# xiexh20/VisTracker

Hardware: AMD Instinct MI355X
Metric: frames/sec joint SMPL+object fit (higher is better)
Workload: dtype f32 (decoder GEMMs: 22-bit split-f16 operands x3 MFMA, fp32 accumulate)

## Files before the change

### include/vistracker.h

```cpp
#ifndef VISTRACKER_H
#define VISTRACKER_H

#include <stddef.h>

#ifdef __cplusplus
extern "C" {
#endif

#define VT_OK 0
#define VT_ERR_ARG -1
#define VT_ERR_HIP -2
#define VT_ERR_BUSY -3

#define VT_SMPL_V 6890
#define VT_SMPL_J 52
#define VT_SMPL_NB 10
#define VT_SMPL_NP 459
#define VT_FEAT 611
#define VT_HID 128

const char *vt_last_error(void);
int vt_version(void);

typedef struct vt_smplh vt_smplh;

int vt_smplh_create(vt_smplh **out, const float *v_template, const float *shapedirs, const float *posedirs,
                    const float *J_regressor, const float *weights, const int *parents, void *stream);
void vt_smplh_destroy(vt_smplh *h);

long vt_smplh_workspace_floats(int B);

int vt_smplh_forward(const vt_smplh *h, const float *pose, const float *betas, const float *trans, int B,
                     float *verts, float *jtr, float *v_posed, float *ws, void *stream);

long vt_smplh_bwd_scratch_floats(int B);
int vt_smplh_backward(const vt_smplh *h, const float *pose, const float *betas, int B, const float *dverts,
                      const float *djtr, const float *v_posed, const float *ws, float *scratch,
                      float *dpose, float *dbetas, float *dtrans, void *stream);

long vt_smplh_prefix_floats(int B);
int vt_smplh_prefix(const vt_smplh *h, const float *pose, int B, float *ws, float *prefix, void *stream);
int vt_smplh_forward_prefixed(const vt_smplh *h, const float *pose, const float *betas, const float *trans, int B, const float *prefix,
                              float *verts, float *jtr, float *v_posed, float *ws, void *stream);
int vt_smplh_backward_free(const vt_smplh *h, const float *pose, int B, const float *dverts, const float *djtr, const float *v_posed,
                           const float *ws, float *scratch, int n_free_pose_cols, float *dpose, float *dbetas, float *dtrans, void *stream);

int vt_rodrigues_forward(const float *aa, int n, float *R, void *stream);
int vt_rodrigues_backward(const float *aa, int n, const float *dR, float *daa, void *stream);

typedef struct vt_landmarks vt_landmarks;
int vt_landmarks_create(vt_landmarks **out, const int *indptr, const int *indices, const float *data, int K, int V,
                        void *stream);
void vt_landmarks_destroy(vt_landmarks *h);
int vt_landmarks_forward(const vt_landmarks *h, const float *verts, int B, float *out, void *stream);
int vt_landmarks_backward(const vt_landmarks *h, const float *dout, int B, float *dverts, int accumulate, void *stream);

int vt_mahalanobis(const float *x, int B, int stride, int off, int n, const float *mean, const float *prec,
                   float *value, float *dx, float gscale, void *stream);

int vt_fill_f64(double *p, long n, double value, void *stream);
int vt_sum_to_term(const float *value, int n, float scale, double *term, void *stream);

typedef struct vt_sifnet vt_sifnet;
int vt_sifnet_create(vt_sifnet **out, const float *const *w, const float *const *b, const float *cam, void *stream);
void vt_sifnet_destroy(vt_sifnet *h);

int vt_nchw_to_nhwc(const float *src, int B, int C, int H, int W, float *dst, void *stream);

typedef struct {
    const float *maps[8];
    int res[8];
    const float *proj;
    int proj_cols;
    int act_level;
    int proj_level;
    int force_fp32;
} vt_maps;

int vt_query_forward(const vt_sifnet *h, const vt_maps *maps, const float *pts, const float *crop_center,
                     const float *body_center, int B, int N,
                     float *df, float *pca, float *parts, float *centers, float *vis, void *stream);
int vt_query_backward(const vt_sifnet *h, const vt_maps *maps, const float *pts, const float *crop_center,
                      const float *body_center, int B, int N,
                      const float *d_df, const float *d_pca, const float *d_parts, const float *d_centers,
                      const float *d_vis, float *dpts, void *stream);

long vt_query_projection_floats(const vt_maps *maps, int B);
int vt_query_build_projection(const vt_sifnet *h, const vt_maps *maps, int B, float *proj, void *stream);

int vt_query_human_loss(const vt_sifnet *h, const vt_maps *maps, const float *pts, const float *crop_center,
                        const float *body_center, int B, int N, const int *labels, const int *order, float w_dfh, float w_part,
                        float *dpts, double *terms, void *stream);
int vt_query_object_loss(const vt_sifnet *h, const vt_maps *maps, const float *pts, const float *crop_center,
                         const float *body_center, int B, int N, const float *occ, float w_obj,
                         float *dpts, double *terms, void *stream);

typedef struct vt_conv3x3 vt_conv3x3;
int vt_conv3x3_create(vt_conv3x3 **out, const float *weight, int cout, int cin, void *stream);
void vt_conv3x3_destroy(vt_conv3x3 *h);
int vt_conv3x3_forward(const vt_conv3x3 *h, const float *in, int B, int H, int W, float *out, int out_cstride, int out_coff, void *stream);
int vt_conv3x3_forward_gn(const vt_conv3x3 *h, const float *in, int in_cstride, int in_coff, const float *gn_stats, const float *gamma,
                          const float *beta, int groups, int B, int H, int W, float *out, int out_cstride, int out_coff, void *stream);
int vt_conv3x3_forward_gn_stats(const vt_conv3x3 *h, const float *in, int in_cstride, int in_coff, const float *gn_stats, const float *gamma,
                                const float *beta, int groups, int B, int H, int W, float *out, int out_cstride, int out_coff, double *stats_ws,
                                int stats_groups, void *stream);
int vt_conv3x3_forward_block(const vt_conv3x3 *h, const float *in, int in_cstride, int in_coff, const float *gn_stats, const float *gamma,
                             const float *beta, int groups, int B, int H, int W, float *out, int out_cstride, int out_coff,
                             const float *res, int res_cstride, int res_coff, float *fin, int fin_cstride, int fin_coff,
                             double *stats_ws, int stats_groups, void *stream);
int vt_conv3x3_tiles(int H, int W);
typedef struct vt_stem7x7 vt_stem7x7;
int vt_stem7x7_create(vt_stem7x7 **out, const float *weight, const float *bias, int cout, int cin, void *stream);
void vt_stem7x7_destroy(vt_stem7x7 *h);
int vt_stem7x7_forward(const vt_stem7x7 *h, const float *in, int in_cstride, int in_coff, int B, int H, int W, float *out, int out_cstride, int out_coff, void *stream);
typedef struct vt_conv1x1 vt_conv1x1;
int vt_conv1x1_create(vt_conv1x1 **out, const float *weight, const float *bias, int cout, int cin, void *stream);
void vt_conv1x1_destroy(vt_conv1x1 *h);
int vt_conv1x1_forward(const vt_conv1x1 *h, const float *in, int in_cstride, int in_coff, const float *gn_stats, const float *gamma, const float *beta, int groups,
                       int B, int H, int W, float *out, int out_cstride, int out_coff, const float *res, int res_cstride, int res_coff,
                       double *stats_ws, int stats_groups, void *stream);
int vt_groupnorm_finalize(double *ws, int nblk, int B, int HW, int C, int groups, float eps, void *stream);
int vt_conv3x3_forward_block_stats(const vt_conv3x3 *h, const float *in, int in_cstride, int in_coff, const float *gn_stats, const float *gamma,
                                   const float *beta, int groups, int B, int H, int W, float *out, int out_cstride, int out_coff,
                                   const float *res, int res_cstride, int res_coff, float *fin, int fin_cstride, int fin_coff,
                                   double *stats_ws, int stats_groups, double *fin_stats_ws, int fin_stats_groups, void *stream);
int vt_avgpool2x2_stats(const float *x, int B, int H, int W, int C, float *out, double *stats_ws, int stats_groups, void *stream);
int vt_sweep_blocks(int HW);
int vt_groupnorm_stats(const float *x, int cstride, int coff, int B, int HW, int C, int groups, float eps, double *ws, void *stream);

#define VT_PRECISION_SPLIT_F16 0
#define VT_PRECISION_FP32 1
int vt_sifnet_set_precision(vt_sifnet *h, int mode);
int vt_sifnet_get_precision(const vt_sifnet *h);

int vt_query_set_human_kernel(int threads);

int vt_query_project_step(const vt_sifnet *h, const vt_maps *maps, const float *pts, const float *crop_center,
                          const float *body_center, int B, int N, int df_idx, float threshold, float *pts_out,
                          float *df_target, void *stream);

int vt_kpts_step(const vt_landmarks *h, const float *verts, const float *kpts, const float *crop_center, int B, int mode, const float *cam, float net_size,
                 float gscale, double *term, float *J, float *dverts, int accumulate, void *stream);
int vt_query_human_step(const vt_sifnet *h, const vt_maps *maps, const float *pts, const float *crop_center, const float *body_center,
                        int B, int N, const int *labels, const int *order, float w_dfh, float w_part, int accumulate, float w_accel,
                        double *term_accel, float *dpts, double *terms, void *stream);
int vt_objstep_head(const float *M0, const float *noise, const float *t, const float *s, int B, const float *X0_points, int N, float *X_points,
                    const float *X0_verts, int NV, float *X_verts, float *R, double *terms, int nzero, float *svd_ws, void *stream);
int vt_temporal_loss2(const float *v, int B, int D, float gscale_accel, double *term_accel, float gscale_velocity, double *term_velocity, float *dv,
                      int init_zero, void *stream);
int vt_objstep_tail(const float *X0_verts, int NV, const float *dX_verts, const float *X0_points, int N, const float *dX_points, const float *s, int B,
                    const float *M0, const float *noise, const float *t, const float *t_init, float w_trans, double *term_trans,
                    float *dR, float *dt, float *dM,
                    float *pR, float *mR, float *vR, float lrR, float *pT, float *mT, float *vT, float lrT, int adam_step, float beta1, float beta2, float eps,
                    double *terms, const float *w, int nterms, float tol, int armed, float *state, int *stop_flag, float *history, int slot, int *ticket, int nzero,
                    float *svd_ws, void *stream);
int vt_objstep_tail_temporal(const float *X_points, float gscale_accel, double *term_accel, float gscale_velocity, double *term_velocity, int init_zero,
                             const float *X0_verts, int NV, const float *dX_verts, const float *X0_points, int N, const float *dX_points, const float *s, int B,
                             const float *M0, const float *noise, const float *t, const float *t_init, float w_trans, double *term_trans,
                             float *dR, float *dt, float *dM,
                             float *pR, float *mR, float *vR, float lrR, float *pT, float *mT, float *vT, float lrT, int adam_step, float beta1, float beta2, float eps,
                             double *terms, const float *w, int nterms, float tol, int armed, float *state, int *stop_flag, float *history, int slot, int *ticket, int nzero,
                             float *svd_ws, void *stream);
int vt_smplstep_tail(float *pose, const float *pose_init, float *dpose, int B, const float *prior_mean, const float *prior_prec, float gscale_prior,
                     double *term_prior, float w_pinit, double *term_pinit,
                     float *p0, int ps0, const float *g0, int gs0, float *m0, float *v0, int n0, float lr0,
                     float *p1, int ps1, const float *g1, int gs1, float *m1, float *v1, int n1, float lr1,
                     float *p2, int ps2, const float *g2, int gs2, float *m2, float *v2, int n2, float lr2,
                     int adam_step, float beta1, float beta2, float eps,
                     double *terms, const float *w, int nterms, float tol, int armed, float *state, int *stop_flag, float *history, int slot, int *ticket, int nzero,
                     void *stream);

int vt_so3_project_forward(const float *M0, const float *noise, int B, float *R, void *stream);
int vt_so3_project_backward(const float *M0, const float *noise, int B, const float *dR, float *dM, void *stream);

int vt_rigid_forward(const float *X0, int shared_x0, const float *R, const float *t, const float *s, int B, int N,
                     float *X, void *stream);
int vt_rigid_backward(const float *X0, int shared_x0, const float *s, int B, int N, const float *dX,
                      float *dR, float *dt, int accumulate, void *stream);

int vt_accel_loss(const float *v, int B, int D, const float *elem_w, float gscale, double *term, float *dv, void *stream);
int vt_accel_loss_strided(const float *v, int B, int D, int stride, const float *elem_w, float gscale, double *term,
                          float *dv, void *stream);
int vt_velocity_loss(const float *v, int B, int D, float gscale, double *term, float *dv, void *stream);

int vt_kpts_loss(const float *J, const float *kpts, const float *crop_center, int B, int K, int mode,
                 const float *cam, float net_size, float gscale, double *term, float *dJ, void *stream);

int vt_sqdiff_loss(const float *a, int a_stride, const float *b, int b_stride, int rows, int cols, float denom,
                   float gscale, double *term, float *da, void *stream);

long vt_collision_workspace_bytes(int B, int n_smpl_faces);
int vt_collision_loss(const float *smpl_verts, int n_smpl_verts, const int *smpl_faces, int n_smpl_faces, const float *obj_verts, int n_obj_verts,
                      const int *obj_faces, int n_obj_faces, int B, float sigma, int max_collisions, float gscale, double *term,
                      float *d_obj_t, int *pairs_per_frame, void *workspace, void *stream);

int vt_chamfer_ragged(const float *x, const int *offx, const float *y, const int *offy, int P, float gscale,
                      double *term, float *dx, float *dy, void *stream);
long vt_chamfer_ws_bytes(long total_x, long total_y, int P);
int vt_chamfer_ragged_ws(const float *x, const int *offx, long total_x, const float *y, const int *offy, long total_y, int P, float gscale,
                         double *term, float *dx, float *dy, void *ws, void *stream);

int vt_chamfer_ragged_idx(const float *x, const int *offx, long total_x, const float *y_base, const int *idx_y, const int *offy, long total_y, int P,
                          float gscale, double *term, float *dy_base, void *ws, int run_plan, void *stream);

int vt_nn_distance(const float *query, int nq, const float *search, int ns, int P, float *dist, void *stream);

long vt_sil_workspace_floats(int B, int NV, int NF, int size);
int vt_sil_forward(const float *verts, int B, int NV, const int *faces, int NF, const float *K, int size,
                   float *image, int *face_index, float *ws, void *stream);
int vt_sil_backward(const float *verts, int B, int NV, const int *faces, int NF, const float *K, int size,
                    const int *face_index, const float *d_image, float eps, float *ws, float *dverts, void *stream);
int vt_sil_setup(const float *mask_h, const float *mask_o, int B, int H, int W, const float *crop_centers, double expansion, int out, double crop_size,
                 double net_size, const double *cam_norm, double image_width, float *image_ref, float *keep_mask, float *K, double *boxes_ws, void *stream);

int vt_sil_mask_loss(const float *image, const float *keep, const float *ref, const float *occ, int B, int size,
                     float gscale, double *term, float *per_frame, float *d_image, void *stream);

int vt_sil_step(const float *verts, int B, int NV, const int *faces, int NF, const float *K, int size, const float *keep, const float *ref,
                const float *occ, float gscale, float eps, double *term, int *face_index, float *d_image, float *ws, float *dverts, void *stream);

int vt_triplane_render(const float *verts, const float *center, int B, int NV, const int *faces, int NF, int size,
                       float *masks, int *face_index, float *ws, void *stream);

int vt_upsample2x_bicubic_add(const float *low, const float *skip, int B, int h, int w, int C, float *out, void *stream);
int vt_upsample2x_bicubic_add_stats(const float *low, const float *skip, int B, int h, int w, int C, float *out, double *stats_ws, int stats_groups,
                                    void *stream);

long vt_groupnorm_workspace_doubles(int B, int HW, int C, int groups);
int vt_groupnorm_nhwc(const float *x, const float *gamma, const float *beta, int B, int HW, int C, int groups, float eps,
                      int relu, double *ws, float *y, void *stream);

int vt_adam_step(float *p, const float *g, float *m, float *v, long n, int step, float lr, float beta1, float beta2,
                 float eps, const int *stop_flag, void *stream);

int vt_adam_step_2d(float *p, long p_stride, const float *g, long g_stride, float *m, float *v, int rows, int cols,
                    int step, float lr, float beta1, float beta2, float eps, const int *stop_flag, void *stream);

int vt_loss_reduce_and_stop(const double *terms, const float *w, int nterms, float tol, int armed, float *state,
                            int *stop_flag, float *history, int slot, void *stream);

int vt_fill(float *p, long n, float value, void *stream);

int vt_stream_set_skip_flag(void *stream, const int *flag);

int vt_gen_round_compact(const float *surface, const float *df_target, const float *pre, const unsigned char *active, int B, int S, float filter_val,
                         float zmin, const long long *fill, int cap, int write, float *buf_points, int *order, float *kept_pre, long long *cnt,
                         long long *fill_out, void *stream);
int vt_gen_scatter_heads(const float *pred, int B, int C, int kmax, const long long *fill_old, const long long *cnt, int cap, float *buf, void *stream);
int vt_gen_resample(const float *samples, const int *order, const long long *cnt, const float *init, int B, int S, int S0, const float *u,
                    const float *pert, int M, float near_scale, float *out, void *stream);

long vt_render_workspace_bytes(int B, int NF, int size, int anti_aliasing, long list_entries);
int vt_render_static_create(void **layer, const float *verts, int NV, const int *faces, int NS, const float *face_colors, const float *K, float orig_size,
                            const float *light, int size, int anti_aliasing, void *stream);
void vt_render_static_destroy(void *layer);
int vt_render_rgb(const float *verts, int B, int NV, const int *faces, int NF, const float *face_colors, const float *K, int k_per_view, float orig_size,
                  const float *light, const float *background, const void *static_layer, int size, int anti_aliasing, float *rgb, float *alpha, float *depth,
                  int *face_index, void *ws, long ws_bytes, long *list_entries, void *stream);
int vt_render_panel_u8(const float *rgb, int B, int size, int row0, int nrows, int col0, int ncols, unsigned char *out, const long long *view_off,
                       long long out_row_stride, void *stream);
int vt_render_rgb_pv(const float *verts, int B, int NV, const int *faces, int NF, const float *face_colors, int colors_per_view, const float *K, int k_per_view,
                     float orig_size, const float *light, const float *background, const void *static_layer, int size, int anti_aliasing, float *rgb,
                     float *alpha, float *depth, int *face_index, void *ws, long ws_bytes, long *list_entries, void *stream);

int vt_contact_regions(const float *smpl_verts, const int *labels, const float *obj_verts, int B, int NVs, int NVo, int P, float thres, int *nn_idx,
                       float *nn_dist, int *part, int *count, float *centre, void *stream);
int vt_contact_spheres(const float *centre, const int *count, int B, int P, const float *unit_verts, int NSV, float radius, float *out, void *stream);
int vt_contact_face_colors(const int *part, int B, int NVo, const int *obj_faces, int NFo, int face_off, const float *base_colors, int NF, const float *palette,
                           int P, float *out, void *stream);

long vt_jpeg_workspace_bytes(int n, int H, int W, int subsampling, long long *max_out_bytes);
int vt_jpeg_encode(const unsigned char *rgb, int n, int H, int W, long long frame_stride, long long row_stride, int quality, int subsampling, void *ws,
                   long ws_bytes, unsigned char *out, long long out_cap, long long *offsets, void *stream);

int vt_mask_bbox(const unsigned char *pm, const unsigned char *om, int B, int H, int W, int thres, int *box, void *stream);
int vt_crop_resize_compose(const unsigned char *rgb, const unsigned char *pm, const unsigned char *om, int B, int H, int W, const int *corners, int crop_size,
                           int out_size, const float *table, float *out, long long frame_stride, void *stream);
int vt_resize_panel_u8(const unsigned char *src, long long src_bytes, const long long *frames, int n, int H, int size, int col0, int pw, unsigned char *out,
                       const long long *out_off, long long out_row_stride, void *stream);

int vt_overlay_panel_u8(const float *rgb, const float *alpha, int B, int size, int row0, int nrows, int col0, int ncols, unsigned char *out,
                        const long long *src_off, const long long *dst_off, long long out_row_stride, float opacity, void *stream);
int vt_mask_score(const int *fidx, int B, int is, int rows, int F, int nf_body, int nf_obj, const unsigned char *pm, long long pm_bytes, const unsigned char *om,
                  long long om_bytes, const long long *frames, int thres, int *count, void *stream);

long vt_point_mesh_workspace_bytes(int B, int n_faces);
int vt_point_mesh_distance(const float *points, int n_points, const float *verts, int n_verts, const int *faces, int n_faces, int B, float *dist, float *closest,
                           int *face_id, void *workspace, void *stream);
int vt_point_mesh_distance_ex(const float *points, int n_points, const float *verts, int n_verts, const int *faces, int n_faces, int B, float *dist,
                              float *closest, int *face_id, void *workspace, int flags, unsigned long long *n_tests, void *stream);
int vt_nearest_vertex(const float *points, int n_points, const float *verts, int n_verts, int B, int *vert_id, float *vert_dist, void *stream);

long vt_sifnet_loss_head_ws_bytes(int B, int n_points);
int vt_sifnet_loss_head(const float *df, const float *pca, const float *parts, const float *centers, const float *vis, int S, int B, int n_points,
                        const float *df_h, const float *df_o, const int *parts_gt, const float *pca_gt, const float *obj_center, const float *visibility,
                        int per_frame, float max_dist, const double *weights, int vis_loss, float gscale, double *terms, float *d_df, float *d_pca,
                        float *d_parts, float *d_centers, float *d_vis, void *workspace, void *stream);

long vt_decoder_param_floats(void);
long vt_decoder_param_offset(int head, int layer, int is_bias);
int vt_decoder_train_forward(const float *params, const float *cam, const vt_maps *maps, const float *pts, const float *crop_center, const float *body_center,
                             int B, int N, float *df, float *pca, float *parts, float *centers, float *vis, void *stream);
long vt_decoder_weight_grads_ws_bytes(int B, int N, int chunk_points);
int vt_decoder_weight_grads(const float *params, const float *cam, const vt_maps *maps, const float *pts, const float *crop_center, const float *body_center,
                            int B, int N, const float *d_df, const float *d_pca, const float *d_parts, const float *d_centers, const float *d_vis,
                            float *dparams, int accumulate, int chunk_points, void *workspace, void *stream);

long vt_decoder_grads_ws_bytes(int B, int N, int chunk_points, int want_maps);
int vt_decoder_grads(const float *params, const float *cam, const vt_maps *maps, const float *pts, const float *crop_center, const float *body_center,
                     int B, int N, const float *d_df, const float *d_pca, const float *d_parts, const float *d_centers, const float *d_vis,
                     float *dparams, int accumulate, const vt_maps *d_maps, int accumulate_maps, int chunk_points, void *workspace, void *stream);

long vt_conv_dgrad_workspace_bytes(int cout, int cin, int taps);
long vt_conv_wgrad_workspace_bytes(int B, int H, int W, int cout, int cin, int taps);
long vt_gn_relu_backward_workspace_bytes(int B, int HW, int C, int groups);
int vt_conv3x3_dgrad(const float *weight, int cout, int cin, const float *d_out, int do_cstride, int do_coff, int B, int H, int W,
                     float *d_in, int di_cstride, int di_coff, void *workspace, void *stream);
int vt_conv1x1_dgrad(const float *weight, int cout, int cin, const float *d_out, int do_cstride, int do_coff, int B, int H, int W,
                     float *d_in, int di_cstride, int di_coff, void *workspace, void *stream);
int vt_conv3x3_wgrad(const float *d_out, int do_cstride, int do_coff, const float *x_in, int xi_cstride, int xi_coff, const float *gn_stats, const float *gamma,
                     const float *beta, int groups, int B, int H, int W, int cin, int cout, float *dW, int accumulate, void *workspace, void *stream);
int vt_conv1x1_wgrad(const float *d_out, int do_cstride, int do_coff, const float *x_in, int xi_cstride, int xi_coff, const float *gn_stats, const float *gamma,
                     const float *beta, int groups, int B, int H, int W, int cin, int cout, float *dW, int accumulate, void *workspace, void *stream);
int vt_gn_relu_backward(const float *g, int g_cstride, int g_coff, const float *x_in, int x_cstride, int x_coff, const float *gn_stats, const float *gamma,
                        const float *beta, int groups, int B, int HW, int C, const float *base, int base_cstride, int base_coff,
                        float *d_x, int dx_cstride, int dx_coff, float *dgamma, float *dbeta, int accumulate, void *workspace, void *stream);
long vt_conv_block_backward_workspace(int B, int H, int W, int cin, int c1, int c2, int c3);
int vt_conv_block_backward(const float *dy, const float *x, const float *raw, const float *stats1, const float *stats2, const float *stats3,
                           const float *w1, const float *w2, const float *w3, const float *gamma1, const float *gamma2, const float *gamma3,
                           const float *beta1, const float *beta2, const float *beta3, const float *wproj, const float *gamma4, const float *beta4,
                           int B, int H, int W, int cin, int c1, int c2, int c3,
                           float *d_x, float *dW1, float *dW2, float *dW3, float *dgamma1, float *dbeta1, float *dgamma2, float *dbeta2, float *dgamma3, float *dbeta3,
                           float *dgamma4, float *dbeta4, float *dWproj, void *workspace, int accumulate, void *stream);

int vt_avgpool2x2_backward(const float *d_out, int B, int H, int W, int C, float *d_x, void *stream);
int vt_upsample2x_bicubic_backward(const float *d_out, int B, int h, int w, int C, float *d_low, void *stream);

long vt_bias_grad_workspace_bytes(int B, int HW, int C);
int vt_bias_grad(const float *d_out, int do_cstride, int do_coff, int B, int HW, int C, float *db, int accumulate, void *workspace, void *stream);
long vt_stem7x7_wgrad_workspace_bytes(int B, int H, int W, int cin, int cout);
int vt_stem7x7_wgrad(const float *d_y, int dy_cstride, int dy_coff, const float *x, int x_cstride, int x_coff, int B, int H, int W, int cin, int cout,
                     float *dW, int accumulate, void *workspace, void *stream);
int vt_gn_relu_backward_y(const float *g, int g_cstride, int g_coff, const float *x_in, int x_cstride, int x_coff, const float *y, int y_cstride, int y_coff,
                          const float *gn_stats, const float *gamma, int groups, int B, int HW, int C, const float *base, int base_cstride, int base_coff,
                          float *d_x, int dx_cstride, int dx_coff, float *dgamma, float *dbeta, int accumulate, void *workspace, void *stream);
long vt_stack_tail_backward_workspace(int B, int H, int W, int C, int Co);
int vt_stack_tail_backward(const float *d_out, const float *d_prev, const float *ll, const float *raw, const float *out, const float *stats,
                           const float *wcl, const float *gamma, const float *beta, const float *wl, const float *wbl, const float *wal,
                           int B, int H, int W, int C, int Co,
                           float *d_ll, float *dWcl, float *dbcl, float *dgamma, float *dbeta, float *dWl, float *dbl, float *dWbl, float *dbbl, float *dWal, float *dbal,
                           void *workspace, int accumulate, void *stream);

#define VT_REPACK_CONV3X3 0
#define VT_REPACK_CONV1X1 1
#define VT_REPACK_STEM7X7 2
typedef struct vt_repack_plan vt_repack_plan;
long vt_conv3x3_packed_bytes(int cout, int cin);
long vt_conv1x1_packed_bytes(int cout, int cin);
int vt_conv1x1_parts(int cout);
long vt_stem7x7_packed_bytes(int cout, int cin);
long vt_repack_workspace_bytes(void);
int vt_conv3x3_pack(const float *w_dev, int cout, int cin, void *packed_dev, float *scale_dev, void *ws_dev, void *stream);
int vt_conv1x1_pack(const float *w_dev, const float *bias_dev, int cout, int cin, void *packed_dev, float *bias_out_dev, float *scale_dev, void *ws_dev,
                    void *stream);
int vt_stem7x7_pack(const float *w_dev, const float *bias_dev, int cout, int cin, void *packed_dev, void *stream);
int vt_conv3x3_create_device(vt_conv3x3 **out, const float *w_dev, int cout, int cin, void *stream);
int vt_conv1x1_create_device(vt_conv1x1 **out, const float *w_dev, const float *bias_dev, int cout, int cin, void *stream);
int vt_stem7x7_create_device(vt_stem7x7 **out, const float *w_dev, const float *bias_dev, int cout, int cin, void *stream);
int vt_conv3x3_repack(vt_conv3x3 *h, const float *w_dev, void *stream);
int vt_conv1x1_repack(vt_conv1x1 *h, const float *w_dev, const float *bias_dev, void *stream);
int vt_stem7x7_repack(vt_stem7x7 *h, const float *w_dev, const float *bias_dev, void *stream);
int vt_repack_plan_create(vt_repack_plan **out, int n, const int *kinds, void *const *handles, const float *const *weights, const float *const *biases);
int vt_repack_plan_run(const vt_repack_plan *plan, void *stream);
void vt_repack_plan_destroy(vt_repack_plan *plan);
int vt_repack_plan_launches(const vt_repack_plan *plan);
int vt_repack_handle_snapshot(int kind, const void *handle, void *packed_out_dev, float *scale_out_dev, void *stream);

int vt_grad_rank_mean(const float *parts, int W, size_t n, size_t stride, float *out, void *stream);

#define VT_GRAD_STATS_CHUNK 4096
#define VT_GUARD_HEAD 16
#define VT_GUARD_SLOT_HEAD 32
#define VT_GUARD_NORM 0
#define VT_GUARD_ERROR 8
#define VT_GUARD_COEF 16
#define VT_GUARD_SKIP 20
#define VT_GUARD_STEP 24
long vt_grad_stats_workspace_bytes(long n, int n_seg);
int vt_grad_stats(const float *g, long n, const long *seg_off, int n_seg, double *sumsq, float *maxabs, int *nonfinite, void *ws, void *stream);
long vt_grad_guard_record_bytes(int n_seg_total, int ring);
int vt_grad_guard_close(const double *sumsq0, const float *maxabs0, const int *nonfinite0, int n_seg0,
                        const double *sumsq1, const float *maxabs1, const int *nonfinite1, int n_seg1,
                        const double *sumsq2, const float *maxabs2, const int *nonfinite2, int n_seg2,
                        const double *error, double max_norm, void *record, int ring, void *stream);
int vt_grad_scale(float *g, long n, const float *coef, const int *skip, void *stream);

long vt_former_layer_tape_floats(int B, int T, int D, int H, int F);
long vt_former_layer_workspace_floats(int B, int T, int D, int H, int F);
int vt_former_layer_forward(const float *x, const float *pos, const unsigned char *key_padding_mask, const float *const *params, int B, int T, int D, int H,
                            int F, int activation, float p, unsigned long long seed, float *y, float *tape, float *workspace, void *stream);
int vt_former_layer_backward(const float *d_y, const float *tape, const float *x, const float *pos, const unsigned char *key_padding_mask,
                             const float *const *params, int B, int T, int D, int H, int F, int activation, float p, unsigned long long seed,
                             float *d_x, float *const *d_params, int accumulate, float *workspace, void *stream);
long vt_layernorm_backward_workspace_floats(long M, int D);
int vt_layernorm_forward(const float *x, const float *weight, const float *bias, long M, int D, float *y, double *stats, void *stream);
int vt_layernorm_backward(const float *d_y, const float *x, const double *stats, const float *weight, long M, int D, float *d_x, float *d_weight,
                          float *d_bias, int accumulate, float *workspace, void *stream);

int vt_query_set_clock_probe(unsigned long long *counters);
long vt_calibrate_workspace_bytes(void);
int vt_calibrate(void *work, double *out, void *stream);

#ifdef __cplusplus
}
#endif
#endif
```

### vistracker_amd/_lib.py

```python
from __future__ import annotations

import ctypes as C
import os

_HERE = os.path.dirname(os.path.abspath(__file__))
LIB_PATH = os.environ.get("VT_LIB_PATH", os.path.join(_HERE, "libvistracker_hip.so"))

vp = C.c_void_p
fp = C.c_void_p
ci = C.c_int
cl = C.c_long
cf = C.c_float
cd = C.c_double


class VtMaps(C.Structure):
    _fields_ = [("maps", C.c_void_p * 8), ("res", C.c_int * 8), ("proj", C.c_void_p), ("proj_cols", C.c_int),
                ("act_level", C.c_int), ("proj_level", C.c_int), ("force_fp32", C.c_int)]


SIGNATURES = {
    "vt_last_error": (C.c_char_p, []),
    "vt_version": (ci, []),
    "vt_smplh_create": (ci, [C.POINTER(vp), vp, vp, vp, vp, vp, vp, vp]),
    "vt_smplh_destroy": (None, [vp]),
    "vt_smplh_workspace_floats": (cl, [ci]),
    "vt_smplh_bwd_scratch_floats": (cl, [ci]),
    "vt_smplh_forward": (ci, [vp, fp, fp, fp, ci, fp, fp, fp, fp, vp]),
    "vt_smplh_backward": (ci, [vp, fp, fp, ci, fp, fp, fp, fp, fp, fp, fp, fp, vp]),
    "vt_smplh_prefix_floats": (cl, [ci]),
    "vt_smplh_prefix": (ci, [vp, fp, ci, fp, fp, vp]),
    "vt_smplh_forward_prefixed": (ci, [vp, fp, fp, fp, ci, fp, fp, fp, fp, fp, vp]),
    "vt_smplh_backward_free": (ci, [vp, fp, ci, fp, fp, fp, fp, fp, ci, fp, fp, fp, vp]),
    "vt_rodrigues_forward": (ci, [fp, ci, fp, vp]),
    "vt_rodrigues_backward": (ci, [fp, ci, fp, fp, vp]),
    "vt_landmarks_create": (ci, [C.POINTER(vp), vp, vp, vp, ci, ci, vp]),
    "vt_landmarks_destroy": (None, [vp]),
    "vt_landmarks_forward": (ci, [vp, fp, ci, fp, vp]),
    "vt_landmarks_backward": (ci, [vp, fp, ci, fp, ci, vp]),
    "vt_mahalanobis": (ci, [fp, ci, ci, ci, ci, fp, fp, fp, fp, cf, vp]),
    "vt_fill_f64": (ci, [fp, cl, cd, vp]),
    "vt_sum_to_term": (ci, [fp, ci, cf, fp, vp]),
    "vt_sifnet_create": (ci, [C.POINTER(vp), C.POINTER(vp), C.POINTER(vp), vp, vp]),
    "vt_sifnet_destroy": (None, [vp]),
    "vt_nchw_to_nhwc": (ci, [fp, ci, ci, ci, ci, fp, vp]),
    "vt_query_forward": (ci, [vp, C.POINTER(VtMaps), fp, fp, fp, ci, ci, fp, fp, fp, fp, fp, vp]),
    "vt_query_backward": (ci, [vp, C.POINTER(VtMaps), fp, fp, fp, ci, ci, fp, fp, fp, fp, fp, fp, vp]),
    "vt_query_human_loss": (ci, [vp, C.POINTER(VtMaps), fp, fp, fp, ci, ci, fp, fp, cf, cf, fp, fp, vp]),
    "vt_query_object_loss": (ci, [vp, C.POINTER(VtMaps), fp, fp, fp, ci, ci, fp, cf, fp, fp, vp]),
    "vt_query_set_human_kernel": (ci, [ci]),
    "vt_sifnet_set_precision": (ci, [vp, ci]),
    "vt_sifnet_get_precision": (ci, [vp]),
    "vt_groupnorm_nhwc": (ci, [fp, fp, fp, ci, ci, ci, ci, cf, ci, fp, fp, vp]),
    "vt_upsample2x_bicubic_add": (ci, [fp, fp, ci, ci, ci, ci, fp, vp]),
    "vt_conv3x3_create": (ci, [C.POINTER(vp), vp, ci, ci, vp]),
    "vt_conv3x3_destroy": (None, [vp]),
    "vt_conv3x3_forward": (ci, [vp, fp, ci, ci, ci, fp, ci, ci, vp]),
    "vt_conv3x3_forward_gn": (ci, [vp, fp, ci, ci, fp, fp, fp, ci, ci, ci, ci, fp, ci, ci, vp]),
    "vt_groupnorm_stats": (ci, [fp, ci, ci, ci, ci, ci, ci, cf, fp, vp]),
    "vt_groupnorm_workspace_doubles": (C.c_long, [ci, ci, ci, ci]),
    "vt_groupnorm_finalize": (ci, [fp, ci, ci, ci, ci, ci, cf, vp]),
    "vt_conv3x3_tiles": (ci, [ci, ci]),
    "vt_kpts_step": (ci, [vp, fp, fp, fp, ci, ci, vp, cf, cf, fp, fp, fp, ci, vp]),
    "vt_query_human_step": (ci, [vp, C.POINTER(VtMaps), fp, fp, fp, ci, ci, fp, fp, cf, cf, ci, cf, fp, fp, fp, vp]),
    "vt_objstep_head": (ci, [fp, fp, fp, fp, ci, fp, ci, fp, fp, ci, fp, fp, fp, ci, fp, vp]),
    "vt_temporal_loss2": (ci, [fp, ci, ci, cf, fp, cf, fp, fp, ci, vp]),
    "vt_objstep_tail": (ci, [fp, ci, fp, fp, ci, fp, fp, ci, fp, fp, fp, fp, cf, fp, fp, fp, fp,
                             fp, fp, fp, cf, fp, fp, fp, cf, ci, cf, cf, cf,
                             fp, vp, ci, cf, ci, fp, fp, fp, ci, fp, ci, fp, vp]),
    "vt_objstep_tail_temporal": (ci, [fp, cf, fp, cf, fp, ci,
                                      fp, ci, fp, fp, ci, fp, fp, ci, fp, fp, fp, fp, cf, fp, fp, fp, fp,
                                      fp, fp, fp, cf, fp, fp, fp, cf, ci, cf, cf, cf,
                                      fp, vp, ci, cf, ci, fp, fp, fp, ci, fp, ci, fp, vp]),
    "vt_smplstep_tail": (ci, [fp, fp, fp, ci, fp, fp, cf, fp, cf, fp,
                              fp, ci, fp, ci, fp, fp, ci, cf, fp, ci, fp, ci, fp, fp, ci, cf, fp, ci, fp, ci, fp, fp, ci, cf, ci, cf, cf, cf,
                              fp, vp, ci, cf, ci, fp, fp, fp, ci, fp, ci, vp]),
    "vt_stream_set_skip_flag": (ci, [vp, vp]),
    "vt_conv1x1_create": (ci, [C.POINTER(vp), vp, vp, ci, ci, vp]),
    "vt_stem7x7_create": (ci, [C.POINTER(vp), vp, vp, ci, ci, vp]),
    "vt_stem7x7_destroy": (None, [vp]),
    "vt_stem7x7_forward": (ci, [vp, fp, ci, ci, ci, ci, ci, fp, ci, ci, vp]),
    "vt_conv1x1_destroy": (None, [vp]),
    "vt_conv1x1_forward": (ci, [vp, fp, ci, ci, fp, fp, fp, ci, ci, ci, ci, fp, ci, ci, fp, ci, ci, fp, ci, vp]),
    "vt_conv3x3_forward_block": (ci, [vp, fp, ci, ci, fp, fp, fp, ci, ci, ci, ci, fp, ci, ci, fp, ci, ci, fp, ci, ci, fp, ci, vp]),
    "vt_conv3x3_forward_block_stats": (ci, [vp, fp, ci, ci, fp, fp, fp, ci, ci, ci, ci, fp, ci, ci, fp, ci, ci, fp, ci, ci, fp, ci, fp, ci, vp]),
    "vt_avgpool2x2_stats": (ci, [fp, ci, ci, ci, ci, fp, fp, ci, vp]),
    "vt_sweep_blocks": (ci, [ci]),
    "vt_upsample2x_bicubic_add_stats": (ci, [fp, fp, ci, ci, ci, ci, fp, fp, ci, vp]),
    "vt_conv3x3_forward_gn_stats": (ci, [vp, fp, ci, ci, fp, fp, fp, ci, ci, ci, ci, fp, ci, ci, fp, ci, vp]),
    "vt_triplane_render": (ci, [fp, fp, ci, ci, fp, ci, ci, fp, fp, fp, vp]),
    "vt_query_project_step": (ci, [vp, C.POINTER(VtMaps), fp, fp, fp, ci, ci, ci, cf, fp, fp, vp]),
    "vt_query_projection_floats": (C.c_long, [C.POINTER(VtMaps), ci]),
    "vt_query_build_projection": (ci, [vp, C.POINTER(VtMaps), ci, fp, vp]),
    "vt_so3_project_forward": (ci, [fp, fp, ci, fp, vp]),
    "vt_so3_project_backward": (ci, [fp, fp, ci, fp, fp, vp]),
    "vt_rigid_forward": (ci, [fp, ci, fp, fp, fp, ci, ci, fp, vp]),
    "vt_rigid_backward": (ci, [fp, ci, fp, ci, ci, fp, fp, fp, ci, vp]),
    "vt_accel_loss": (ci, [fp, ci, ci, fp, cf, fp, fp, vp]),
    "vt_accel_loss_strided": (ci, [fp, ci, ci, ci, fp, cf, fp, fp, vp]),
    "vt_velocity_loss": (ci, [fp, ci, ci, cf, fp, fp, vp]),
    "vt_kpts_loss": (ci, [fp, fp, fp, ci, ci, ci, vp, cf, cf, fp, fp, vp]),
    "vt_sqdiff_loss": (ci, [fp, ci, fp, ci, ci, ci, cf, cf, fp, fp, vp]),
    "vt_chamfer_ragged": (ci, [fp, fp, fp, fp, ci, cf, fp, fp, fp, vp]),
    "vt_chamfer_ws_bytes": (C.c_long, [C.c_long, C.c_long, ci]),
    "vt_chamfer_ragged_ws": (ci, [fp, fp, C.c_long, fp, fp, C.c_long, ci, cf, fp, fp, fp, fp, vp]),
    "vt_chamfer_ragged_idx": (ci, [fp, fp, C.c_long, fp, fp, fp, C.c_long, ci, cf, fp, fp, fp, ci, vp]),
    "vt_collision_workspace_bytes": (cl, [ci, ci]),
    "vt_collision_loss": (ci, [fp, ci, fp, ci, fp, ci, fp, ci, ci, cf, ci, cf, fp, fp, fp, fp, vp]),
    "vt_nn_distance": (ci, [fp, ci, fp, ci, ci, fp, vp]),
    "vt_sil_workspace_floats": (cl, [ci, ci, ci, ci]),
    "vt_sil_forward": (ci, [fp, ci, ci, fp, ci, fp, ci, fp, fp, fp, vp]),
    "vt_sil_backward": (ci, [fp, ci, ci, fp, ci, fp, ci, fp, fp, cf, fp, fp, vp]),
    "vt_sil_mask_loss": (ci, [fp, fp, fp, fp, ci, ci, cf, fp, fp, fp, vp]),
    "vt_sil_step": (ci, [fp, ci, ci, fp, ci, fp, ci, fp, fp, fp, cf, cf, fp, fp, fp, fp, fp, vp]),
    "vt_gen_round_compact": (ci, [fp, fp, fp, vp, ci, ci, cf, cf, vp, ci, ci, fp, vp, fp, vp, vp, vp]),
    "vt_gen_scatter_heads": (ci, [fp, ci, ci, ci, vp, vp, ci, fp, vp]),
    "vt_gen_resample": (ci, [fp, vp, vp, fp, ci, ci, ci, fp, fp, ci, cf, fp, vp]),
    "vt_sil_setup": (ci, [fp, fp, ci, ci, ci, fp, C.c_double, ci, C.c_double, C.c_double, C.POINTER(C.c_double), C.c_double, fp, fp, fp, fp, vp]),
    "vt_adam_step": (ci, [fp, fp, fp, fp, cl, ci, cf, cf, cf, cf, fp, vp]),
    "vt_adam_step_2d": (ci, [fp, cl, fp, cl, fp, fp, ci, ci, ci, cf, cf, cf, cf, fp, vp]),
    "vt_loss_reduce_and_stop": (ci, [fp, vp, ci, cf, ci, fp, fp, fp, ci, vp]),
    "vt_fill": (ci, [fp, cl, cf, vp]),
    "vt_selftest_mfma": (ci, [fp, fp, fp, vp]),
    "vt_query_set_clock_probe": (ci, [vp]),
    "vt_render_workspace_bytes": (cl, [ci, ci, ci, ci, cl]),
    "vt_render_static_create": (ci, [C.POINTER(vp), fp, ci, fp, ci, fp, fp, cf, C.POINTER(cf), ci, ci, vp]),
    "vt_render_static_destroy": (None, [vp]),
    "vt_render_rgb": (ci, [fp, ci, ci, fp, ci, fp, fp, ci, cf, C.POINTER(cf), C.POINTER(cf), vp, ci, ci, fp, fp, fp, fp, fp, cl,
                           C.POINTER(cl), vp]),
    "vt_render_panel_u8": (ci, [fp, ci, ci, ci, ci, ci, ci, fp, fp, C.c_longlong, vp]),
    "vt_render_rgb_pv": (ci, [fp, ci, ci, fp, ci, fp, ci, fp, ci, cf, C.POINTER(cf), C.POINTER(cf), vp, ci, ci, fp, fp, fp, fp, fp, cl,
                              C.POINTER(cl), vp]),
    "vt_contact_regions": (ci, [fp, fp, fp, ci, ci, ci, ci, cf, fp, fp, fp, fp, fp, vp]),
    "vt_contact_spheres": (ci, [fp, fp, ci, ci, fp, ci, cf, fp, vp]),
    "vt_contact_face_colors": (ci, [fp, ci, ci, fp, ci, ci, fp, ci, fp, ci, fp, vp]),
    "vt_jpeg_workspace_bytes": (cl, [ci, ci, ci, ci, C.POINTER(C.c_longlong)]),
    "vt_jpeg_encode": (ci, [fp, ci, ci, ci, C.c_longlong, C.c_longlong, ci, ci, vp, cl, vp, C.c_longlong,
                            C.POINTER(C.c_longlong), vp]),
    "vt_mask_bbox": (ci, [fp, fp, ci, ci, ci, ci, fp, vp]),
    "vt_crop_resize_compose": (ci, [fp, fp, fp, ci, ci, ci, fp, ci, ci, fp, fp, C.c_longlong, vp]),
    "vt_resize_panel_u8": (ci, [fp, C.c_longlong, vp, ci, ci, ci, ci, ci, fp, fp, C.c_longlong, vp]),
    "vt_overlay_panel_u8": (ci, [fp, fp, ci, ci, ci, ci, ci, ci, fp, fp, fp, C.c_longlong, cf, vp]),
    "vt_mask_score": (ci, [fp, ci, ci, ci, ci, ci, ci, fp, C.c_longlong, fp, C.c_longlong, vp, ci, fp, vp]),
    "vt_point_mesh_workspace_bytes": (cl, [ci, ci]),
    "vt_point_mesh_distance": (ci, [fp, ci, fp, ci, fp, ci, ci, fp, fp, fp, vp, vp]),
    "vt_point_mesh_distance_ex": (ci, [fp, ci, fp, ci, fp, ci, ci, fp, fp, fp, vp, ci, fp, vp]),
    "vt_nearest_vertex": (ci, [fp, ci, fp, ci, ci, fp, fp, vp]),
    "vt_sifnet_loss_head_ws_bytes": (cl, [ci, ci]),
    "vt_sifnet_loss_head": (ci, [fp, fp, fp, fp, fp, ci, ci, ci, fp, fp, fp, fp, fp, fp, ci, cf, C.POINTER(cd), ci, cf, fp, fp, fp, fp, fp, fp, vp, vp]),
    "vt_decoder_param_floats": (cl, []),
    "vt_decoder_param_offset": (cl, [ci, ci, ci]),
    "vt_decoder_train_forward": (ci, [fp, vp, C.POINTER(VtMaps), fp, fp, fp, ci, ci, fp, fp, fp, fp, fp, vp]),
    "vt_decoder_weight_grads_ws_bytes": (cl, [ci, ci, ci]),
    "vt_decoder_weight_grads": (ci, [fp, vp, C.POINTER(VtMaps), fp, fp, fp, ci, ci, fp, fp, fp, fp, fp, fp, ci, ci, vp, vp]),
    "vt_decoder_grads_ws_bytes": (cl, [ci, ci, ci, ci]),
    "vt_decoder_grads": (ci, [fp, vp, C.POINTER(VtMaps), fp, fp, fp, ci, ci, fp, fp, fp, fp, fp, fp, ci, C.POINTER(VtMaps), ci, ci, vp, vp]),
    "vt_conv_dgrad_workspace_bytes": (cl, [ci, ci, ci]),
    "vt_conv_wgrad_workspace_bytes": (cl, [ci, ci, ci, ci, ci, ci]),
    "vt_gn_relu_backward_workspace_bytes": (cl, [ci, ci, ci, ci]),
    "vt_conv3x3_dgrad": (ci, [fp, ci, ci, fp, ci, ci, ci, ci, ci, fp, ci, ci, vp, vp]),
    "vt_conv1x1_dgrad": (ci, [fp, ci, ci, fp, ci, ci, ci, ci, ci, fp, ci, ci, vp, vp]),
    "vt_conv3x3_wgrad": (ci, [fp, ci, ci, fp, ci, ci, fp, fp, fp, ci, ci, ci, ci, ci, ci, fp, ci, vp, vp]),
    "vt_conv1x1_wgrad": (ci, [fp, ci, ci, fp, ci, ci, fp, fp, fp, ci, ci, ci, ci, ci, ci, fp, ci, vp, vp]),
    "vt_gn_relu_backward": (ci, [fp, ci, ci, fp, ci, ci, fp, fp, fp, ci, ci, ci, ci, fp, ci, ci, fp, ci, ci, fp, fp, ci, vp, vp]),
    "vt_conv_block_backward_workspace": (cl, [ci, ci, ci, ci, ci, ci, ci]),
    "vt_conv_block_backward": (ci, [fp] * 6 + [fp] * 9 + [fp] * 3 + [ci] * 7 + [fp] * 13 + [vp, ci, vp]),
    "vt_avgpool2x2_backward": (ci, [fp, ci, ci, ci, ci, fp, vp]),
    "vt_upsample2x_bicubic_backward": (ci, [fp, ci, ci, ci, ci, fp, vp]),
    "vt_bias_grad_workspace_bytes": (cl, [ci, ci, ci]),
    "vt_bias_grad": (ci, [fp, ci, ci, ci, ci, ci, fp, ci, vp, vp]),
    "vt_stem7x7_wgrad_workspace_bytes": (cl, [ci, ci, ci, ci, ci]),
    "vt_stem7x7_wgrad": (ci, [fp, ci, ci, fp, ci, ci, ci, ci, ci, ci, ci, fp, ci, vp, vp]),
    "vt_gn_relu_backward_y": (ci, [fp, ci, ci, fp, ci, ci, fp, ci, ci, fp, fp, ci, ci, ci, ci, fp, ci, ci, fp, ci, ci, fp, fp, ci, vp, vp]),
    "vt_stack_tail_backward_workspace": (cl, [ci, ci, ci, ci, ci]),
    "vt_stack_tail_backward": (ci, [fp] * 6 + [fp] * 6 + [ci] * 5 + [fp] * 11 + [vp, ci, vp]),
    "vt_conv3x3_packed_bytes": (cl, [ci, ci]),
    "vt_conv1x1_packed_bytes": (cl, [ci, ci]),
    "vt_conv1x1_parts": (ci, [ci]),
    "vt_stem7x7_packed_bytes": (cl, [ci, ci]),
    "vt_repack_workspace_bytes": (cl, []),
    "vt_conv3x3_pack": (ci, [fp, ci, ci, fp, fp, fp, vp]),
    "vt_conv1x1_pack": (ci, [fp, fp, ci, ci, fp, fp, fp, fp, vp]),
    "vt_stem7x7_pack": (ci, [fp, fp, ci, ci, fp, vp]),
    "vt_conv3x3_create_device": (ci, [C.POINTER(vp), fp, ci, ci, vp]),
    "vt_conv1x1_create_device": (ci, [C.POINTER(vp), fp, fp, ci, ci, vp]),
    "vt_stem7x7_create_device": (ci, [C.POINTER(vp), fp, fp, ci, ci, vp]),
    "vt_conv3x3_repack": (ci, [vp, fp, vp]),
    "vt_conv1x1_repack": (ci, [vp, fp, fp, vp]),
    "vt_stem7x7_repack": (ci, [vp, fp, fp, vp]),
    "vt_repack_plan_create": (ci, [C.POINTER(vp), ci, C.POINTER(ci), C.POINTER(vp), C.POINTER(vp), C.POINTER(vp)]),
    "vt_repack_plan_launches": (ci, [vp]),
    "vt_repack_plan_run": (ci, [vp, vp]),
    "vt_repack_plan_destroy": (None, [vp]),
    "vt_repack_handle_snapshot": (ci, [ci, vp, fp, fp, vp]),
    "vt_grad_rank_mean": (ci, [fp, ci, C.c_size_t, C.c_size_t, fp, vp]),
    "vt_grad_stats_workspace_bytes": (cl, [cl, ci]),
    "vt_grad_stats": (ci, [fp, cl, fp, ci, fp, fp, fp, fp, vp]),
    "vt_grad_guard_record_bytes": (cl, [ci, ci]),
    "vt_grad_guard_close": (ci, [fp, fp, fp, ci] * 3 + [fp, cd, fp, ci, vp]),
    "vt_grad_scale": (ci, [fp, cl, fp, fp, vp]),
    "vt_calibrate_workspace_bytes": (cl, []),
    "vt_calibrate": (ci, [vp, C.POINTER(C.c_double), vp]),
    "vt_former_layer_tape_floats": (cl, [ci, ci, ci, ci, ci]),
    "vt_former_layer_workspace_floats": (cl, [ci, ci, ci, ci, ci]),
    "vt_former_layer_forward": (ci, [fp, fp, fp, vp, ci, ci, ci, ci, ci, ci, cf, C.c_ulonglong, fp, fp, fp, vp]),
    "vt_former_layer_backward": (ci, [fp, fp, fp, fp, fp, vp, ci, ci, ci, ci, ci, ci, cf, C.c_ulonglong, fp, vp, ci, fp, vp]),
    "vt_layernorm_backward_workspace_floats": (cl, [cl, ci]),
    "vt_layernorm_forward": (ci, [fp, fp, fp, cl, ci, fp, fp, vp]),
    "vt_layernorm_backward": (ci, [fp, fp, fp, fp, cl, ci, fp, fp, fp, ci, fp, vp]),
}

_lib = None


class VtError(RuntimeError):
    pass


def lib():
    global _lib
    if _lib is None:
        if not os.path.exists(LIB_PATH):
            raise VtError(f"{LIB_PATH} is missing: build it with `make -C vistracker_amd/csrc` "
                          f"(or `python -c 'import __graft_entry__ as g; g.build()'`); there is no CPU fallback")
        import torch
        l = C.CDLL(LIB_PATH)
        for name, (res, args) in SIGNATURES.items():
            fn = getattr(l, name)
            fn.restype = res
            fn.argtypes = args
        _lib = l
        _host_tuning()
    return _lib


def _host_tuning():
    if os.environ.get("VT_HOST_THP", "keep") != "off":
        return
    try:
        C.CDLL(None, use_errno=True).prctl(41, 1, 0, 0, 0)
    except Exception:
        pass


VT_OK, VT_ERR_ARG, VT_ERR_HIP, VT_ERR_BUSY = 0, -1, -2, -3


def check(rc: int):
    if rc != 0:
        raise VtError(f"libvistracker_hip error {rc}: {lib().vt_last_error().decode()}")


def stream_ptr():
    import torch
    return torch.cuda.current_stream().cuda_stream


def dptr(t):
    if t is None:
        return None
    if not t.is_cuda:
        raise VtError("libvistracker_hip ops need CUDA (HIP) tensors; there is no CPU fallback in the product path")
    if not t.is_contiguous():
        raise VtError("libvistracker_hip ops need contiguous tensors")
    import torch
    if t.device.index != torch.cuda.current_device():
        raise VtError(f"tensor on cuda:{t.device.index} but the current device is cuda:{torch.cuda.current_device()}: "
                      "wrap the call in `with torch.cuda.device(tensor.device):`")
    return t.data_ptr()
```

### vistracker_amd/csrc/smplh.hip

```cpp
#include "common.h"
#include <cstring>

#define V_ VT_SMPL_V
#define J_ VT_SMPL_J
#define NB_ VT_SMPL_NB
#define NP_ VT_SMPL_NP
#define VP_ 6912
#define NVT_ 27
#define KQ_ 472
#define NQ_ 480
#define J_LIVE_ 22
#define NP_LIVE_ ((J_LIVE_ - 1) * 9)
#define KF_ 272
#define NT_LIVE_ 13
#define NQ_HAND_ (NT_LIVE_ * 16)
#define NP_NUM_ (J_ * 3)
__host__ __device__ constexpr int kq_of_posemap(int p) { return p < NP_LIVE_ ? KF_ + p : p - NP_LIVE_; }
__host__ __device__ constexpr int nq_of_posemap(int p) { return p < NP_LIVE_ ? p : NQ_HAND_ + (p - NP_LIVE_); }
#define KQ_BETA0 (KF_ + NP_LIVE_)
#define KQ_TEMPLATE (KQ_ - 1)
#define NQ_BETA0 NP_LIVE_
static_assert(KF_ % 8 == 0 && KF_ >= NP_ - NP_LIVE_ && KQ_BETA0 + NB_ <= KQ_TEMPLATE && (KQ_ - KF_) % 8 == 0, "K order of Q_kcv");
static_assert(NQ_BETA0 + NB_ <= NQ_HAND_ && NQ_HAND_ + (NP_ - NP_LIVE_) <= NQ_, "N order of Q_t");
typedef float f32x4 __attribute__((ext_vector_type(4)));
#define MFMA16(a, b, c) __builtin_amdgcn_mfma_f32_16x16x4f32((a), (b), (c), 0, 0, 0)

#define WS_R 0
#define WS_J (52 * 9)
#define WS_G (WS_J + 52 * 3)
#define WS_A (WS_G + 52 * 12)
#define WS_FRAME (WS_A + 52 * 12)
#define PT_DA 0
#define PT_DTR 624
#define PT_N 627
#define KTOT_ (VP_ * 3)
#define KG_SLAB 24
#define NKS_ (KTOT_ / 16 / KG_SLAB)

#define SCHED_STEPS 32
#define SCHED_WIDTH 10
struct SmplParents { int p[J_]; int nsteps; short sched[SCHED_STEPS][SCHED_WIDTH]; };

#define SP_K 8
struct vt_smplh {
    float *Q_kcv, *Q_t, *W_jv, *W_v64, *J_t, *J_s;
    float *W_sp;
    int nnz;
    SmplParents par;
};

struct RodCtx { float n, ax, ay, az, c, s, qn, w, x, y, z; };

__device__ __forceinline__ void rodrigues_fwd(const float *t, float *R, RodCtx *k)
{
    const float xe = t[0] + 1e-8f, ye = t[1] + 1e-8f, ze = t[2] + 1e-8f;
    const float n = sqrtf(xe * xe + ye * ye + ze * ze);
    const float ax = t[0] / n, ay = t[1] / n, az = t[2] / n;
    const float h = n * 0.5f;
    const float c = cosf(h), s = sinf(h);
    const float q0 = c, q1 = s * ax, q2 = s * ay, q3 = s * az;
    const float qn = sqrtf(q0 * q0 + q1 * q1 + q2 * q2 + q3 * q3);
    const float w = q0 / qn, x = q1 / qn, y = q2 / qn, z = q3 / qn;
    const float w2 = w * w, x2 = x * x, y2 = y * y, z2 = z * z;
    const float wx = w * x, wy = w * y, wz = w * z, xy = x * y, xz = x * z, yz = y * z;
    R[0] = w2 + x2 - y2 - z2; R[1] = 2 * xy - 2 * wz;   R[2] = 2 * wy + 2 * xz;
    R[3] = 2 * wz + 2 * xy;   R[4] = w2 - x2 + y2 - z2; R[5] = 2 * yz - 2 * wx;
    R[6] = 2 * xz - 2 * wy;   R[7] = 2 * wx + 2 * yz;   R[8] = w2 - x2 - y2 + z2;
    if (k) { k->n = n; k->ax = ax; k->ay = ay; k->az = az; k->c = c; k->s = s; k->qn = qn; k->w = w; k->x = x; k->y = y; k->z = z; }
}

__device__ __forceinline__ void rodrigues_bwd(const float *t, const float *dR, float *dt)
{
    float R[9]; RodCtx k; rodrigues_fwd(t, R, &k);
    const float w = k.w, x = k.x, y = k.y, z = k.z;
    const float dw = 2 * w * (dR[0] + dR[4] + dR[8]) + 2 * (-z * dR[1] + y * dR[2] + z * dR[3] - x * dR[5] - y * dR[6] + x * dR[7]);
    const float dx = 2 * x * (dR[0] - dR[4] - dR[8]) + 2 * (y * dR[1] + z * dR[2] + y * dR[3] - w * dR[5] + z * dR[6] + w * dR[7]);
    const float dy = 2 * y * (-dR[0] + dR[4] - dR[8]) + 2 * (x * dR[1] + w * dR[2] + x * dR[3] + z * dR[5] - w * dR[6] + z * dR[7]);
    const float dz = 2 * z * (-dR[0] - dR[4] + dR[8]) + 2 * (-w * dR[1] + x * dR[2] + w * dR[3] + y * dR[5] + x * dR[6] + y * dR[7]);
    const float dot = w * dw + x * dx + y * dy + z * dz;
    const float dq0 = (dw - w * dot) / k.qn, dq1 = (dx - x * dot) / k.qn, dq2 = (dy - y * dot) / k.qn, dq3 = (dz - z * dot) / k.qn;
    const float dh = -k.s * dq0 + k.c * (k.ax * dq1 + k.ay * dq2 + k.az * dq3);
    const float dax = k.s * dq1, day = k.s * dq2, daz = k.s * dq3;
    const float dn = 0.5f * dh - (t[0] * dax + t[1] * day + t[2] * daz) / (k.n * k.n);
    dt[0] = dax / k.n + dn * (t[0] + 1e-8f) / k.n;
    dt[1] = day / k.n + dn * (t[1] + 1e-8f) / k.n;
    dt[2] = daz / k.n + dn * (t[2] + 1e-8f) / k.n;
}

__global__ void rodrigues_fwd_kernel(const float *aa, int n, float *R)
{
    const int i = blockIdx.x * blockDim.x + threadIdx.x;
    if (i >= n) return;
    float t[3] = {aa[3 * i], aa[3 * i + 1], aa[3 * i + 2]}, r[9];
    rodrigues_fwd(t, r, nullptr);
#pragma unroll
    for (int e = 0; e < 9; e++) R[9 * i + e] = r[e];
}

__global__ void rodrigues_bwd_kernel(const float *aa, int n, const float *dR, float *daa)
{
    const int i = blockIdx.x * blockDim.x + threadIdx.x;
    if (i >= n) return;
    float t[3] = {aa[3 * i], aa[3 * i + 1], aa[3 * i + 2]}, g[9], d[3];
#pragma unroll
    for (int e = 0; e < 9; e++) g[e] = dR[9 * i + e];
    rodrigues_bwd(t, g, d);
    daa[3 * i] = d[0]; daa[3 * i + 1] = d[1]; daa[3 * i + 2] = d[2];
}

__global__ __launch_bounds__(64) void smplh_pose_kernel(const float *__restrict__ pose, const float *__restrict__ betas,
                                                        const float *__restrict__ trans, const float *__restrict__ J_t,
                                                        const float *__restrict__ J_s, SmplParents par,
                                                        float *__restrict__ ws, float *__restrict__ jtr, int rod_lo, int rod_hi, int chain,
                                                        const int *skip)
{
    VT_SKIP_RETURN(skip);
    __shared__ float sR[J_ * 9], sJ[J_ * 3], sG[J_ * 12];
    const int b = blockIdx.x, j = threadIdx.x;
    float *w = ws + (size_t)b * WS_FRAME;
    if (j < J_) {
        float R[9];
        if (j >= rod_lo && j < rod_hi) {
            float t[3] = {pose[(b * J_ + j) * 3], pose[(b * J_ + j) * 3 + 1], pose[(b * J_ + j) * 3 + 2]};
            rodrigues_fwd(t, R, nullptr);
#pragma unroll
            for (int e = 0; e < 9; e++) w[WS_R + j * 9 + e] = R[e];
        } else if (chain) {
#pragma unroll
            for (int e = 0; e < 9; e++) R[e] = w[WS_R + j * 9 + e];
        }
        if (chain) {
#pragma unroll
            for (int e = 0; e < 9; e++) sR[j * 9 + e] = R[e];
        }
    }
    if (!chain) return;
    if (j < J_) {
#pragma unroll
        for (int c = 0; c < 3; c++) {
            float a = J_t[j * 3 + c];
#pragma unroll
            for (int l = 0; l < NB_; l++) a += J_s[(j * 3 + c) * NB_ + l] * betas[b * NB_ + l];
            sJ[j * 3 + c] = a; w[WS_J + j * 3 + c] = a;
        }
    }
    __shared__ int sPar[J_];
    if (j < J_) sPar[j] = par.p[j];
    __syncthreads();
    int lvl = 0, maxl = 0;
    if (j < J_) { for (int q = j; q != 0; q = sPar[q]) lvl++; }
    maxl = lvl;
    for (int o = 32; o > 0; o >>= 1) maxl = max(maxl, __shfl_xor(maxl, o, 64));
    maxl = __builtin_amdgcn_readfirstlane(maxl);
    if (j == 0) { for (int r = 0; r < 3; r++) { for (int c = 0; c < 3; c++) sG[r * 4 + c] = sR[r * 3 + c]; sG[r * 4 + 3] = sJ[r]; } }
    __syncthreads();
    for (int l = 1; l <= maxl; l++) {
        if (j < J_ && lvl == l) {
            const int i = j, p = sPar[i];
            const float *Gp = sG + 12 * p, *Ri = sR + 9 * i;
            const float d0 = sJ[3 * i] - sJ[3 * p], d1 = sJ[3 * i + 1] - sJ[3 * p + 1], d2 = sJ[3 * i + 2] - sJ[3 * p + 2];
            float *Gi = sG + 12 * i;
            for (int r = 0; r < 3; r++) {
                const float g0 = Gp[r * 4], g1 = Gp[r * 4 + 1], g2 = Gp[r * 4 + 2];
                Gi[r * 4 + 0] = g0 * Ri[0] + g1 * Ri[3] + g2 * Ri[6];
                Gi[r * 4 + 1] = g0 * Ri[1] + g1 * Ri[4] + g2 * Ri[7];
                Gi[r * 4 + 2] = g0 * Ri[2] + g1 * Ri[5] + g2 * Ri[8];
                Gi[r * 4 + 3] = g0 * d0 + g1 * d1 + g2 * d2 + Gp[r * 4 + 3];
            }
        }
        __syncthreads();
    }
    if (j < J_) {
        const float *G = sG + 12 * j;
#pragma unroll
        for (int r = 0; r < 3; r++) {
            const float gt = G[r * 4 + 3];
            w[WS_G + j * 12 + r * 4 + 0] = G[r * 4]; w[WS_G + j * 12 + r * 4 + 1] = G[r * 4 + 1];
            w[WS_G + j * 12 + r * 4 + 2] = G[r * 4 + 2]; w[WS_G + j * 12 + r * 4 + 3] = gt;
            w[WS_A + j * 12 + r * 4 + 0] = G[r * 4]; w[WS_A + j * 12 + r * 4 + 1] = G[r * 4 + 1]; w[WS_A + j * 12 + r * 4 + 2] = G[r * 4 + 2];
            w[WS_A + j * 12 + r * 4 + 3] = gt - (G[r * 4] * sJ[3 * j] + G[r * 4 + 1] * sJ[3 * j + 1] + G[r * 4 + 2] * sJ[3 * j + 2]);
            if (jtr) jtr[(b * J_ + j) * 3 + r] = gt + trans[3 * b + r];
        }
    }
}

#define FWD_FB 16
#ifndef FWD_PF
#define FWD_PF 6
#endif
#define AXS 516
#define SAS 628
#define FWD_R0 (FWD_FB * AXS > 8 * SAS ? FWD_FB * AXS : 8 * SAS)
template <int MODE>
__global__ __launch_bounds__(256) void smplh_verts_kernel(const float *__restrict__ Q_kcv, const float *__restrict__ W_jv,
                                                          const float *__restrict__ betas, const float *__restrict__ trans,
                                                          const float *__restrict__ ws, int B,
                                                          float *__restrict__ verts, float *__restrict__ v_posed, const float *__restrict__ W_sp, int nnz,
                                                          float *prefix, const int *skip)
{
    VT_SKIP_RETURN(skip);
    constexpr int K0 = MODE == 2 ? KF_ : 0, K1 = MODE == 1 ? KF_ : KQ_;
    extern __shared__ __attribute__((aligned(16))) float lds[];
    float *sAx = lds;
    float *sA = lds;
    float *sVp = lds + FWD_R0;
    float *sW = sVp + FWD_FB * 64 * 3;
    float *sTr = sW + (nnz > 0 ? 2 * SP_K * 64 : J_ * 64);
    const int tid = threadIdx.x, wave = tid >> 6, lane = tid & 63, q = lane >> 4, j = lane & 15;
    const int b0 = blockIdx.y * FWD_FB, v = blockIdx.x * 64 + wave * 16 + j;
    for (int k = K0 + tid; k < K1; k += 256) {
        int p = -1, l = -1;
        if (k < NP_ - NP_LIVE_) p = NP_LIVE_ + k;
        else if (k >= KF_ && k < KQ_BETA0) p = k - KF_;
        else if (k >= KQ_BETA0 && k < KQ_BETA0 + NB_) l = k - KQ_BETA0;
        const int e9 = p % 9;
        const float sub = (p >= 0 && (e9 == 0 || e9 == 4 || e9 == 8)) ? 1.f : 0.f;
        float val[FWD_FB];
#pragma unroll
        for (int f = 0; f < FWD_FB; f++) {
            const int b = min(b0 + f, B - 1);
            if (p >= 0) val[f] = ws[(size_t)b * WS_FRAME + WS_R + 9 + p];
            else if (l >= 0) val[f] = betas[b * NB_ + l];
            else val[f] = (k == KQ_TEMPLATE) ? 1.f : 0.f;
        }
#pragma unroll
        for (int f = 0; f < FWD_FB; f++) sAx[f * AXS + k] = val[f] - sub;
    }
    if (MODE == 1) {
    } else if (nnz > 0) {
        for (int i = tid; i < nnz * 64; i += 256) {
            sW[i] = W_sp[(size_t)(i >> 6) * VP_ + blockIdx.x * 64 + (i & 63)];
            sW[SP_K * 64 + i] = W_sp[(size_t)(SP_K + (i >> 6)) * VP_ + blockIdx.x * 64 + (i & 63)];
        }
    } else
        for (int i = tid; i < J_ * 64; i += 256) sW[i] = W_jv[(i >> 6) * VP_ + blockIdx.x * 64 + (i & 63)];
    if (MODE != 1 && tid < FWD_FB * 3) { const int f = tid / 3, b = min(b0 + f, B - 1); sTr[tid] = trans[b * 3 + tid % 3]; }
    __syncthreads();

    f32x4 acc[3];
    f32x4 *pre4 = reinterpret_cast<f32x4 *>(prefix) + ((size_t)blockIdx.y * gridDim.x + blockIdx.x) * 3 * 256 + tid;
#pragma unroll
    for (int c = 0; c < 3; c++) acc[c] = MODE == 2 ? pre4[c * 256] : (f32x4){0.f, 0.f, 0.f, 0.f};
    constexpr int S0 = K0 / 8, NS = K1 / 8;
    float bq[FWD_PF][2][3];
#define FWD_LOADQ(slot_, s_)                                                                     \
    {                                                                                            \
        const float *qk = Q_kcv + (size_t)(8 * (s_) + 2 * q) * 3 * VP_ + v;                      \
        _Pragma("unroll") for (int e = 0; e < 2; e++)                                            \
            _Pragma("unroll") for (int c = 0; c < 3; c++) bq[slot_][e][c] = qk[(size_t)(e * 3 + c) * VP_]; \
    }
#pragma unroll
    for (int s = 0; s < FWD_PF; s++) FWD_LOADQ(s, S0 + s)
#pragma unroll
    for (int s = S0; s < NS; s++) {
        const float2 av = *reinterpret_cast<const float2 *>(sAx + j * AXS + 8 * s + 2 * q);
#pragma unroll
        for (int c = 0; c < 3; c++) acc[c] = MFMA16(av.x, bq[(s - S0) % FWD_PF][0][c], acc[c]);
#pragma unroll
        for (int c = 0; c < 3; c++) acc[c] = MFMA16(av.y, bq[(s - S0) % FWD_PF][1][c], acc[c]);
        if (s + FWD_PF < NS) FWD_LOADQ((s - S0) % FWD_PF, s + FWD_PF)
        __builtin_amdgcn_sched_barrier(0);
    }
#undef FWD_LOADQ
    if (MODE == 1) {
#pragma unroll
        for (int c = 0; c < 3; c++) pre4[c * 256] = acc[c];
        return;
    }
    __syncthreads();
#pragma unroll
    for (int r = 0; r < 4; r++)
#pragma unroll
        for (int c = 0; c < 3; c++) sVp[((4 * q + r) * 64 + wave * 16 + j) * 3 + c] = acc[c][r];
    const int vv = tid & 63, vg = blockIdx.x * 64 + vv;
#pragma unroll 1
    for (int r = 0; r < 4; r++) {
        if ((r & 1) == 0) {
            if (r) __syncthreads();
            for (int i = tid; i < 8 * 624; i += 256) {
                const int sl = i / 624, f = 4 * (sl >> 1) + r + (sl & 1), b = min(b0 + f, B - 1);
                sA[sl * SAS + (i % 624)] = ws[(size_t)b * WS_FRAME + WS_A + (i % 624)];
            }
            __syncthreads();
        }
        const int f = 4 * wave + r, b = b0 + f;
        float T[12];
#pragma unroll
        for (int e = 0; e < 12; e++) T[e] = 0.f;
        const float4 *Af = reinterpret_cast<const float4 *>(sA + (2 * wave + (r & 1)) * SAS);
        if (nnz > 0) {
            for (int k = 0; k < nnz; k++) {
                const int jj = __float_as_int(sW[k * 64 + vv]);
                const float wj = sW[(SP_K + k) * 64 + vv];
                const float4 a0 = Af[jj * 3], a1 = Af[jj * 3 + 1], a2 = Af[jj * 3 + 2];
                T[0] += wj * a0.x; T[1] += wj * a0.y; T[2] += wj * a0.z; T[3] += wj * a0.w;
                T[4] += wj * a1.x; T[5] += wj * a1.y; T[6] += wj * a1.z; T[7] += wj * a1.w;
                T[8] += wj * a2.x; T[9] += wj * a2.y; T[10] += wj * a2.z; T[11] += wj * a2.w;
            }
        } else {
#pragma unroll 4
            for (int jj = 0; jj < J_; jj++) {
                const float wj = sW[jj * 64 + vv];
                const float4 a0 = Af[jj * 3], a1 = Af[jj * 3 + 1], a2 = Af[jj * 3 + 2];
                T[0] += wj * a0.x; T[1] += wj * a0.y; T[2] += wj * a0.z; T[3] += wj * a0.w;
                T[4] += wj * a1.x; T[5] += wj * a1.y; T[6] += wj * a1.z; T[7] += wj * a1.w;
                T[8] += wj * a2.x; T[9] += wj * a2.y; T[10] += wj * a2.z; T[11] += wj * a2.w;
            }
        }
        if (b < B && vg < V_) {
            const float p0 = sVp[(f * 64 + vv) * 3], p1 = sVp[(f * 64 + vv) * 3 + 1], p2 = sVp[(f * 64 + vv) * 3 + 2];
            const size_t o = ((size_t)b * V_ + vg) * 3;
#pragma unroll
            for (int rr = 0; rr < 3; rr++) verts[o + rr] = T[rr * 4] * p0 + T[rr * 4 + 1] * p1 + T[rr * 4 + 2] * p2 + T[rr * 4 + 3] + sTr[f * 3 + rr];
            v_posed[o] = p0; v_posed[o + 1] = p1; v_posed[o + 2] = p2;
        }
    }
}

template <int FB>
__global__ __launch_bounds__(256) void smplh_bwd_tile_kernel(const float *__restrict__ W_v64, const float *__restrict__ ws,
                                                             const float *__restrict__ v_posed, const float *__restrict__ dverts,
                                                             int B, float *__restrict__ part, float *__restrict__ dvp_g, const int *skip)
{
    VT_SKIP_RETURN(skip);
    extern __shared__ __attribute__((aligned(16))) float lds[];
    float *sdT = lds;
    float *sA = sdT + 256 * 13;
    const int tid = threadIdx.x, tile = blockIdx.x, b0 = blockIdx.y * FB, v0 = tile * 256, v = v0 + tid;
    const int wave = tid >> 6, lane = tid & 63, q = lane >> 4, j = lane & 15;
    for (int i = tid; i < FB * 624; i += 256) { const int f = i / 624, b = min(b0 + f, B - 1); sA[i] = ws[(size_t)b * WS_FRAME + WS_A + (i % 624)]; }
    float w1[4][13], w2[64];
#pragma unroll
    for (int mt = 0; mt < 4; mt++)
#pragma unroll
        for (int ks = 0; ks < 13; ks++) w1[mt][ks] = W_v64[(size_t)(v0 + 64 * wave + 16 * mt + j) * 64 + 4 * ks + q];
#pragma unroll
    for (int ks = 0; ks < 64; ks++) w2[ks] = W_v64[(size_t)(v0 + 4 * ks + q) * 64 + wave * 16 + j];
    __syncthreads();
    float dvn[3] = {0.f, 0.f, 0.f}, vpn[3] = {0.f, 0.f, 0.f};
    auto fetch = [&](int b) {
#pragma unroll
        for (int r = 0; r < 3; r++) { dvn[r] = 0.f; vpn[r] = 0.f; }
        if (b < B && v < V_) {
            const size_t o = ((size_t)b * V_ + v) * 3;
            dvn[0] = dverts[o]; dvn[1] = dverts[o + 1]; dvn[2] = dverts[o + 2];
            vpn[0] = v_posed[o]; vpn[1] = v_posed[o + 1]; vpn[2] = v_posed[o + 2];
        }
    };
    fetch(b0);
#pragma unroll 1
    for (int f = 0; f < FB; f++) {
        const int b = b0 + f;
        const float dv[3] = {dvn[0], dvn[1], dvn[2]}, vp[3] = {vpn[0], vpn[1], vpn[2]};
        if (f + 1 < FB) fetch(b + 1);
#pragma unroll
        for (int r = 0; r < 3; r++) {
            sdT[tid * 13 + r * 4 + 0] = dv[r] * vp[0]; sdT[tid * 13 + r * 4 + 1] = dv[r] * vp[1];
            sdT[tid * 13 + r * 4 + 2] = dv[r] * vp[2]; sdT[tid * 13 + r * 4 + 3] = dv[r];
        }
        __syncthreads();
        {
            f32x4 t[4];
#pragma unroll
            for (int mt = 0; mt < 4; mt++) t[mt] = (f32x4){0.f, 0.f, 0.f, 0.f};
#pragma unroll
            for (int ks = 0; ks < 13; ks++) {
                const float bv = j < 12 ? sA[f * 624 + (4 * ks + q) * 12 + j] : 0.f;
#pragma unroll
                for (int mt = 0; mt < 4; mt++) t[mt] = MFMA16(w1[mt][ks], bv, t[mt]);
            }
            const int r4 = (j < 12 ? (j >> 2) : 0) * 4 + 3;
#pragma unroll
            for (int mt = 0; mt < 4; mt++) {
#pragma unroll
                for (int r = 0; r < 4; r++) {
                    const int vl = 64 * wave + 16 * mt + 4 * q + r;
                    float x = t[mt][r] * sdT[vl * 13 + r4];
                    x += __shfl_down(x, 4, 16) + __shfl_down(x, 8, 16);
                    if (j < 3 && b < B) dvp_g[(size_t)b * KTOT_ + (size_t)(v0 + vl) * 3 + j] = x;
                }
            }
        }
        {
            f32x4 acc = (f32x4){0.f, 0.f, 0.f, 0.f}, acc2 = (f32x4){0.f, 0.f, 0.f, 0.f};
#pragma unroll
            for (int ks = 0; ks < 64; ks += 2) {
                const int va = 4 * ks + q, vb = va + 4;
                const float a0 = j < 12 ? sdT[va * 13 + j] : 0.f, a1 = j < 12 ? sdT[vb * 13 + j] : 0.f;
                acc = MFMA16(a0, w2[ks], acc);
                acc2 = MFMA16(a1, w2[ks + 1], acc2);
            }
            acc += acc2;
            if (b < B) {
                float *dst = part + ((size_t)tile * B + b) * PT_N;
                const int jn = wave * 16 + j;
#pragma unroll
                for (int r = 0; r < 4; r++) {
                    const int e = 4 * q + r;
                    if (e < 12) {
                        if (jn < J_) dst[PT_DA + jn * 12 + e] = acc[r];
                        else if (jn == J_ && (e & 3) == 3) dst[PT_DTR + (e >> 2)] = acc[r];
                    }
                }
            }
        }
        __syncthreads();
    }
}

#define BL_M 96
#ifndef BL_NW
#define BL_NW 1
#endif
#define BL_AS 132
__global__ __launch_bounds__(256) void smplh_bwd_blend_kernel(const float *__restrict__ Q_p, const float *__restrict__ dvp_g, int B, int ntiles,
                                                              float *__restrict__ part3, const int *skip)
{
    VT_SKIP_RETURN(skip);
    __shared__ __attribute__((aligned(16))) float sA[BL_M * BL_AS];
    const int tid = threadIdx.x, wave = tid >> 6, lane = tid & 63, q = lane >> 4, j = lane & 15;
    const int ks = blockIdx.x, m0 = blockIdx.z * BL_M, nt0 = blockIdx.y * (4 * BL_NW) + wave * BL_NW;
    const bool has_tile = nt0 < ntiles;
    f32x4 acc[6][BL_NW];
#pragma unroll
    for (int mt = 0; mt < 6; mt++)
#pragma unroll
        for (int n = 0; n < BL_NW; n++) acc[mt][n] = (f32x4){0.f, 0.f, 0.f, 0.f};
    const float4 *Q4 = reinterpret_cast<const float4 *>(Q_p);
#pragma unroll 1
    for (int c = 0; c < KG_SLAB / 8; c++) {
        __syncthreads();
        for (int i = tid; i < BL_M * 32; i += 256) {
            const int row = i >> 5, c4 = i & 31, b = m0 + row;
            float4 v = make_float4(0.f, 0.f, 0.f, 0.f);
            if (b < B) v = *reinterpret_cast<const float4 *>(dvp_g + (size_t)b * KTOT_ + (size_t)(ks * KG_SLAB + c * 8) * 16 + c4 * 4);
            *reinterpret_cast<float4 *>(sA + row * BL_AS + c4 * 4) = v;
        }
        __syncthreads();
        if (!has_tile) continue;
#pragma unroll
        for (int g = 0; g < 8; g++) {
            const size_t kg = (size_t)ks * KG_SLAB + c * 8 + g;
            float bq[BL_NW][4];
#pragma unroll
            for (int n = 0; n < BL_NW; n++) {
                const float4 fq = Q4[(kg * (NQ_ / 16) + min(nt0 + n, ntiles - 1)) * 64 + lane];
                bq[n][0] = fq.x; bq[n][1] = fq.y; bq[n][2] = fq.z; bq[n][3] = fq.w;
            }
#pragma unroll
            for (int mt = 0; mt < 6; mt++) {
                const float4 a4 = *reinterpret_cast<const float4 *>(sA + (mt * 16 + j) * BL_AS + g * 16 + q * 4);
                const float av[4] = {a4.x, a4.y, a4.z, a4.w};
#pragma unroll
                for (int s = 0; s < 4; s++)
#pragma unroll
                    for (int n = 0; n < BL_NW; n++) acc[mt][n] = MFMA16(av[s], bq[n][s], acc[mt][n]);
            }
        }
    }
#pragma unroll
    for (int mt = 0; mt < 6; mt++) {
#pragma unroll
        for (int r = 0; r < 4; r++) {
            const int b = m0 + mt * 16 + 4 * q + r;
            if (b < B) {
                float *dst = part3 + ((size_t)ks * B + b) * NQ_;
#pragma unroll
                for (int n = 0; n < BL_NW; n++)
                    if (nt0 + n < ntiles) dst[(nt0 + n) * 16 + j] = acc[mt][n][r];
            }
        }
    }
}

__global__ __launch_bounds__(256) void smplh_bwd_frame_kernel(const float *__restrict__ pose, const float *__restrict__ J_s,
                                                              SmplParents par, const float *__restrict__ ws,
                                                              const float *__restrict__ part, const float *__restrict__ part3,
                                                              const float *__restrict__ djtr, int B, int n_free, float *__restrict__ dpose,
                                                              float *__restrict__ dbetas, float *__restrict__ dtrans, const int *skip)
{
    VT_SKIP_RETURN(skip);
    __shared__ float red[PT_N], red3[NQ_];
    __shared__ float sdG[J_ * 12], sdJ[J_ * 3], sdR[J_ * 9];
    __shared__ float sG[J_ * 12], sRm[J_ * 9], sJr[J_ * 3];
    const int b = blockIdx.x, tid = threadIdx.x;
    const float *w = ws + (size_t)b * WS_FRAME;
    for (int i = tid; i < J_ * 12; i += 256) sG[i] = w[WS_G + i];
    for (int i = tid; i < J_ * 9; i += 256) sRm[i] = w[WS_R + i];
    for (int i = tid; i < J_ * 3; i += 256) sJr[i] = w[WS_J + i];
    for (int i = tid; i < PT_N; i += 256) {
        float s = 0.f;
#pragma unroll 9
        for (int t = 0; t < NVT_; t++) s += part[((size_t)t * B + b) * PT_N + i];
        red[i] = s;
    }
    const int ncol = n_free < NP_NUM_ ? NQ_HAND_ : NQ_, jfree = n_free / 3;
    for (int i = tid; i < ncol; i += 256) {
        float s = 0.f;
#pragma unroll 9
        for (int t = 0; t < NKS_; t++) s += part3[((size_t)t * B + b) * NQ_ + i];
        red3[i] = s;
    }
    __syncthreads();
    if (tid < J_) {
        const int j = tid;
        const float *G = sG + 12 * j; const float *Jr = sJr;
        float dj[3] = {0.f, 0.f, 0.f};
#pragma unroll
        for (int r = 0; r < 3; r++) {
            const float dat = red[PT_DA + 12 * j + r * 4 + 3];
#pragma unroll
            for (int c = 0; c < 3; c++) { sdG[12 * j + r * 4 + c] = red[PT_DA + 12 * j + r * 4 + c] - dat * Jr[3 * j + c]; dj[c] -= G[r * 4 + c] * dat; }
            sdG[12 * j + r * 4 + 3] = dat + (djtr ? djtr[(b * J_ + j) * 3 + r] : 0.f);
        }
        sdJ[3 * j] = dj[0]; sdJ[3 * j + 1] = dj[1]; sdJ[3 * j + 2] = dj[2];
#pragma unroll
        for (int e = 0; e < 9; e++) sdR[9 * j + e] = 0.f;
    }
    __syncthreads();
    const int jloc = tid / 24, el = tid - 24 * jloc;
    const int nsteps = par.nsteps > 0 ? par.nsteps : J_ - 1;
    for (int step = 0; step < nsteps; step++) {
        const int j = par.nsteps > 0 ? (jloc < SCHED_WIDTH ? (int)par.sched[step][jloc < SCHED_WIDTH ? jloc : 0] : -1) : (jloc == 0 ? J_ - 1 - step : -1);
        if (j >= 1) {
            const int p = par.p[j];
            const float *Gp = sG + 12 * p, *Rj = sRm + 9 * j, *dGj = sdG + 12 * j;
            float upd = 0.f; float *dst = nullptr; float upd2 = 0.f; float *dst2 = nullptr;
            if (el < 12) {
                const int r = el >> 2, c = el & 3;
                dst = sdG + 12 * p + el;
                if (c < 3) upd = dGj[r * 4] * Rj[3 * c] + dGj[r * 4 + 1] * Rj[3 * c + 1] + dGj[r * 4 + 2] * Rj[3 * c + 2] + dGj[r * 4 + 3] * (sJr[3 * j + c] - sJr[3 * p + c]);
                else upd = dGj[r * 4 + 3];
            } else if (el < 21) {
                const int e = el - 12, r = e / 3, c = e - 3 * r;
                dst = sdR + 9 * j + e;
                upd = Gp[r] * dGj[c] + Gp[4 + r] * dGj[4 + c] + Gp[8 + r] * dGj[8 + c];
            } else {
                const int c = el - 21;
                upd = Gp[c] * dGj[3] + Gp[4 + c] * dGj[7] + Gp[8 + c] * dGj[11];
                dst = sdJ + 3 * j + c; dst2 = sdJ + 3 * p + c; upd2 = -upd;
            }
            if (dst) *dst += upd;
            if (dst2) *dst2 += upd2;
        }
        __syncthreads();
    }
    if (tid < 3) { for (int c = 0; c < 3; c++) sdR[3 * tid + c] += sdG[tid * 4 + c]; sdJ[tid] += sdG[tid * 4 + 3]; }
    __syncthreads();
    if (tid < jfree) {
        const int j = tid;
        float g[9], t[3] = {pose[(b * J_ + j) * 3], pose[(b * J_ + j) * 3 + 1], pose[(b * J_ + j) * 3 + 2]}, d[3];
#pragma unroll
        for (int e = 0; e < 9; e++) g[e] = sdR[9 * j + e] + (j >= 1 ? red3[nq_of_posemap((j - 1) * 9 + e)] : 0.f);
        rodrigues_bwd(t, g, d);
        dpose[(b * J_ + j) * 3] = d[0]; dpose[(b * J_ + j) * 3 + 1] = d[1]; dpose[(b * J_ + j) * 3 + 2] = d[2];
    } else if (tid >= 64 && tid < 64 + NB_) {
        const int l = tid - 64;
        float s = red3[NQ_BETA0 + l];
        for (int i = 0; i < J_ * 3; i++) s += J_s[i * NB_ + l] * sdJ[i];
        dbetas[b * NB_ + l] = s;
    } else if (tid >= 128 && tid < 131) {
        const int c = tid - 128;
        float s = red[PT_DTR + c];
        if (djtr) for (int j = 0; j < J_; j++) s += djtr[(b * J_ + j) * 3 + c];
        dtrans[b * 3 + c] = s;
    }
}

extern "C" int vt_smplh_create(vt_smplh **out, const float *v_template, const float *shapedirs, const float *posedirs,
                               const float *J_regressor, const float *weights, const int *parents, void *stream)
{
    VT_REQUIRE(out && v_template && shapedirs && posedirs && J_regressor && weights && parents, "vt_smplh_create: null argument");
    hipStream_t st = vt_stream(stream);
    vt_smplh *h = new vt_smplh();
    for (int j = 0; j < J_; j++) h->par.p[j] = (j == 0) ? 0 : parents[j];
    for (int j = 1; j < J_; j++) VT_REQUIRE(h->par.p[j] >= 0 && h->par.p[j] < j, "vt_smplh_create: parents[%d]=%d must be in [0,%d)", j, parents[j], j);
    {
        int lvl[J_], rank[J_], maxl = 0;
        lvl[0] = 0; rank[0] = 0;
        for (int j = 1; j < J_; j++) { lvl[j] = lvl[h->par.p[j]] + 1; maxl = std::max(maxl, lvl[j]); rank[j] = 0; for (int k = j + 1; k < J_; k++) rank[j] += (h->par.p[k] == h->par.p[j]); }
        int n = 0; bool ok = true;
        for (int t = 0; t < SCHED_STEPS; t++) for (int i = 0; i < SCHED_WIDTH; i++) h->par.sched[t][i] = -1;
        for (int l = maxl; l >= 1 && ok; l--)
            for (int r = 0; r < J_ && ok; r++) {
                int cnt = 0;
                for (int j = J_ - 1; j >= 1; j--) if (lvl[j] == l && rank[j] == r) { if (n >= SCHED_STEPS || cnt >= SCHED_WIDTH) { ok = false; break; } h->par.sched[n][cnt++] = (short)j; }
                if (cnt) n++;
            }
        h->par.nsteps = ok ? n : 0;
    }
    float *Q_kcv = new float[(size_t)KQ_ * 3 * VP_](), *Q_t = new float[(size_t)VP_ * 3 * NQ_](), *W_jv = new float[(size_t)J_ * VP_](),
          *J_t = new float[J_ * 3], *J_s = new float[J_ * 3 * NB_];
    for (int v = 0; v < V_; v++) for (int c = 0; c < 3; c++) {
        for (int k = 0; k < NP_ + NB_ + 1; k++) {
            const float val = k < NP_ ? posedirs[((size_t)v * 3 + c) * NP_ + k]
                            : (k < NP_ + NB_ ? shapedirs[((size_t)v * 3 + c) * NB_ + (k - NP_)] : v_template[v * 3 + c]);
            const int kq = k < NP_ ? kq_of_posemap(k) : (k < NP_ + NB_ ? KQ_BETA0 + (k - NP_) : KQ_TEMPLATE);
            Q_kcv[(size_t)(kq * 3 + c) * VP_ + v] = val;
            if (k < NP_ + NB_) {
                const int nq = k < NP_ ? nq_of_posemap(k) : NQ_BETA0 + (k - NP_);
                const size_t kr = (size_t)v * 3 + c, g = kr >> 4, qq = (kr & 15) >> 2, ss = kr & 3;
                Q_t[((g * (NQ_ / 16) + (nq >> 4)) * 64 + qq * 16 + (nq & 15)) * 4 + ss] = val;
            }
        }
    }
    float *W_v64 = new float[(size_t)VP_ * 64]();
    for (int v = 0; v < V_; v++) { for (int j = 0; j < J_; j++) { W_jv[(size_t)j * VP_ + v] = weights[(size_t)v * J_ + j]; W_v64[(size_t)v * 64 + j] = weights[(size_t)v * J_ + j]; } W_v64[(size_t)v * 64 + J_] = 1.0f; }
    float *W_sp = new float[(size_t)2 * SP_K * VP_]();
    int nnz = 0;
    for (int v = 0; v < V_; v++) {
        int k = 0;
        for (int j = 0; j < J_; j++) {
            const float w = weights[(size_t)v * J_ + j];
            if (w == 0.0f) continue;
            if (k < SP_K) { const int jj = j; memcpy(&W_sp[(size_t)k * VP_ + v], &jj, 4); W_sp[(size_t)(SP_K + k) * VP_ + v] = w; }
            k++;
        }
        nnz = k > nnz ? k : nnz;
    }
    h->nnz = nnz <= SP_K ? (nnz > 0 ? nnz : 1) : 0;
    for (int j = 0; j < J_; j++) for (int c = 0; c < 3; c++) {
        double a = 0; double sb[NB_] = {0};
        for (int v = 0; v < V_; v++) {
            const double r = J_regressor[(size_t)j * V_ + v];
            if (r == 0.0) continue;
            a += r * v_template[v * 3 + c];
            for (int l = 0; l < NB_; l++) sb[l] += r * shapedirs[((size_t)v * 3 + c) * NB_ + l];
        }
        J_t[j * 3 + c] = (float)a;
        for (int l = 0; l < NB_; l++) J_s[(j * 3 + c) * NB_ + l] = (float)sb[l];
    }
    int rc = VT_OK;
    if ((rc = vt_upload(&h->Q_kcv, Q_kcv, (size_t)KQ_ * 3 * VP_, st)) || (rc = vt_upload(&h->Q_t, Q_t, (size_t)VP_ * 3 * NQ_, st)) ||
        (rc = vt_upload(&h->W_jv, W_jv, (size_t)J_ * VP_, st)) || (rc = vt_upload(&h->W_v64, W_v64, (size_t)VP_ * 64, st)) ||
        (rc = vt_upload(&h->J_t, J_t, (size_t)J_ * 3, st)) || (rc = vt_upload(&h->J_s, J_s, (size_t)J_ * 3 * NB_, st)) ||
        (rc = vt_upload(&h->W_sp, W_sp, (size_t)2 * SP_K * VP_, st))) {
        return rc;
    }
    VT_HIP(hipStreamSynchronize(st));
    delete[] Q_kcv; delete[] Q_t; delete[] W_jv; delete[] W_v64; delete[] J_t; delete[] J_s; delete[] W_sp;
    *out = h;
    return VT_OK;
}

extern "C" void vt_smplh_destroy(vt_smplh *h)
{
    if (!h) return;
    hipFree(h->Q_kcv); hipFree(h->Q_t); hipFree(h->W_jv); hipFree(h->W_v64); hipFree(h->J_t); hipFree(h->J_s); hipFree(h->W_sp);
    delete h;
}

extern "C" long vt_smplh_workspace_floats(int B) { return (long)B * WS_FRAME; }
extern "C" long vt_smplh_bwd_scratch_floats(int B) { return (long)NVT_ * B * PT_N + (long)B * KTOT_ + (long)NKS_ * B * NQ_; }

#define BWD_FB 6

extern "C" long vt_smplh_prefix_floats(int B) { return (long)((B + FWD_FB - 1) / FWD_FB) * (VP_ / 64) * 3 * 256 * 4; }

#define FWD_LDS_FLOATS(w_) (FWD_R0 + FWD_FB * 64 * 3 + (w_) + FWD_FB * 3)
static int smplh_forward_launch(int mode, const vt_smplh *h, const float *pose, const float *betas, const float *trans, int B, float *verts, float *jtr,
                                float *v_posed, float *ws, float *prefix, hipStream_t st)
{
    const int *skip = mode == 1 ? nullptr : vt_skip_flag_of(st);
    hipLaunchKernelGGL(smplh_pose_kernel, dim3(B), dim3(64), 0, st, pose, betas, trans, h->J_t, h->J_s, h->par, ws, jtr, mode == 1 ? J_LIVE_ : 0,
                       mode == 2 ? J_LIVE_ : J_, mode == 1 ? 0 : 1, skip);
    VT_LAUNCH_CHECK();
    const size_t lds_f = sizeof(float) * FWD_LDS_FLOATS(h->nnz > 0 ? 2 * SP_K * 64 : J_ * 64), lds_max = sizeof(float) * FWD_LDS_FLOATS(J_ * 64);
    const dim3 grid(VP_ / 64, (B + FWD_FB - 1) / FWD_FB);
    if (mode == 0) {
        VT_LDS_LIMIT(smplh_verts_kernel<0>, lds_max);
        hipLaunchKernelGGL(smplh_verts_kernel<0>, grid, dim3(256), lds_f, st, h->Q_kcv, h->W_jv, betas, trans, ws, B, verts, v_posed, h->W_sp, h->nnz, prefix, skip);
    } else if (mode == 1) {
        VT_LDS_LIMIT(smplh_verts_kernel<1>, sizeof(float) * FWD_R0);
        hipLaunchKernelGGL(smplh_verts_kernel<1>, grid, dim3(256), sizeof(float) * FWD_R0, st, h->Q_kcv, h->W_jv, betas, trans, ws, B, verts, v_posed, h->W_sp,
                           h->nnz, prefix, skip);
    } else {
        VT_LDS_LIMIT(smplh_verts_kernel<2>, lds_max);
        hipLaunchKernelGGL(smplh_verts_kernel<2>, grid, dim3(256), lds_f, st, h->Q_kcv, h->W_jv, betas, trans, ws, B, verts, v_posed, h->W_sp, h->nnz, prefix, skip);
    }
    VT_LAUNCH_CHECK();
    return VT_OK;
}

extern "C" int vt_smplh_forward(const vt_smplh *h, const float *pose, const float *betas, const float *trans, int B,
                                float *verts, float *jtr, float *v_posed, float *ws, void *stream)
{
    VT_REQUIRE(h && pose && betas && trans && verts && v_posed && ws && B > 0, "vt_smplh_forward: null argument or B <= 0");
    return smplh_forward_launch(0, h, pose, betas, trans, B, verts, jtr, v_posed, ws, nullptr, vt_stream(stream));
}

extern "C" int vt_smplh_prefix(const vt_smplh *h, const float *pose, int B, float *ws, float *prefix, void *stream)
{
    VT_REQUIRE(h && pose && ws && prefix && B > 0, "vt_smplh_prefix: null argument or B <= 0");
    return smplh_forward_launch(1, h, pose, nullptr, nullptr, B, nullptr, nullptr, nullptr, ws, prefix, vt_stream(stream));
}

extern "C" int vt_smplh_forward_prefixed(const vt_smplh *h, const float *pose, const float *betas, const float *trans, int B, const float *prefix,
                                         float *verts, float *jtr, float *v_posed, float *ws, void *stream)
{
    VT_REQUIRE(h && pose && betas && trans && prefix && verts && v_posed && ws && B > 0, "vt_smplh_forward_prefixed: null argument or B <= 0");
    return smplh_forward_launch(2, h, pose, betas, trans, B, verts, jtr, v_posed, ws, const_cast<float *>(prefix), vt_stream(stream));
}

static int smplh_backward_launch(const vt_smplh *h, const float *pose, int B, const float *dverts, const float *djtr, const float *v_posed, const float *ws,
                                 float *scratch, int n_free, float *dpose, float *dbetas, float *dtrans, hipStream_t st)
{
    const int *skip = vt_skip_flag_of(st);
    const size_t lds = sizeof(float) * (256 * 13 + BWD_FB * 624);
    float *dvp_g = scratch + (size_t)NVT_ * B * PT_N, *part3 = dvp_g + (size_t)B * KTOT_;
    const int ntiles = n_free < NP_NUM_ ? NT_LIVE_ : NQ_ / 16;
    VT_LDS_LIMIT(smplh_bwd_tile_kernel<BWD_FB>, lds);
    hipLaunchKernelGGL(smplh_bwd_tile_kernel<BWD_FB>, dim3(NVT_, (B + BWD_FB - 1) / BWD_FB), dim3(256), lds, st, h->W_v64, ws, v_posed, dverts, B, scratch, dvp_g, skip);
    VT_LAUNCH_CHECK();
    hipLaunchKernelGGL(smplh_bwd_blend_kernel, dim3(NKS_, (ntiles + 4 * BL_NW - 1) / (4 * BL_NW), (B + BL_M - 1) / BL_M), dim3(256), 0, st, h->Q_t, dvp_g, B, ntiles,
                       part3, skip);
    VT_LAUNCH_CHECK();
    hipLaunchKernelGGL(smplh_bwd_frame_kernel, dim3(B), dim3(256), 0, st, pose, h->J_s, h->par, ws, scratch, part3, djtr, B, n_free, dpose, dbetas, dtrans, skip);
    VT_LAUNCH_CHECK();
    return VT_OK;
}

extern "C" int vt_smplh_backward(const vt_smplh *h, const float *pose, const float *betas, int B, const float *dverts,
                                 const float *djtr, const float *v_posed, const float *ws, float *scratch,
                                 float *dpose, float *dbetas, float *dtrans, void *stream)
{
    (void)betas;
    VT_REQUIRE(h && pose && dverts && v_posed && ws && scratch && dpose && dbetas && dtrans && B > 0, "vt_smplh_backward: null argument or B <= 0");
    return smplh_backward_launch(h, pose, B, dverts, djtr, v_posed, ws, scratch, NP_NUM_, dpose, dbetas, dtrans, vt_stream(stream));
}

extern "C" int vt_smplh_backward_free(const vt_smplh *h, const float *pose, int B, const float *dverts, const float *djtr, const float *v_posed,
                                      const float *ws, float *scratch, int n_free_pose_cols, float *dpose, float *dbetas, float *dtrans, void *stream)
{
    VT_REQUIRE(h && pose && dverts && v_posed && ws && scratch && dpose && dbetas && dtrans && B > 0, "vt_smplh_backward_free: null argument or B <= 0");
    VT_REQUIRE(n_free_pose_cols > 0 && n_free_pose_cols <= 3 * J_LIVE_ && n_free_pose_cols % 3 == 0,
               "vt_smplh_backward_free: n_free_pose_cols=%d must be a multiple of 3 in (0, %d] (the joints from %d on are the frozen ones of the layout)",
               n_free_pose_cols, 3 * J_LIVE_, J_LIVE_);
    return smplh_backward_launch(h, pose, B, dverts, djtr, v_posed, ws, scratch, n_free_pose_cols, dpose, dbetas, dtrans, vt_stream(stream));
}

extern "C" int vt_rodrigues_forward(const float *aa, int n, float *R, void *stream)
{
    VT_REQUIRE(aa && R && n > 0, "vt_rodrigues_forward: bad argument");
    hipLaunchKernelGGL(rodrigues_fwd_kernel, dim3((n + 255) / 256), dim3(256), 0, vt_stream(stream), aa, n, R);
    VT_LAUNCH_CHECK();
    return VT_OK;
}

extern "C" int vt_rodrigues_backward(const float *aa, int n, const float *dR, float *daa, void *stream)
{
    VT_REQUIRE(aa && dR && daa && n > 0, "vt_rodrigues_backward: bad argument");
    hipLaunchKernelGGL(rodrigues_bwd_kernel, dim3((n + 255) / 256), dim3(256), 0, vt_stream(stream), aa, n, dR, daa);
    VT_LAUNCH_CHECK();
    return VT_OK;
}
```

### vistracker_amd/csrc/step.hip

```cpp
#include "step_ops.h"
#include <vector>

__global__ __launch_bounds__(1024) void objstep_head_kernel(const float *__restrict__ M0, const float *__restrict__ noise, const float *__restrict__ t,
                                                           const float *__restrict__ s, const float *__restrict__ X0p, int N, float *__restrict__ Xp,
                                                           const float *__restrict__ X0v, int NV, float *__restrict__ Xv, float *__restrict__ Rout,
                                                           double *terms, int nzero, float *__restrict__ svd_ws)
{
    __shared__ float sR[9];
    const int b = blockIdx.y;
    if (threadIdx.x == 0) {
        float M[9]; Svd3 sv;
        so3_input(M0, noise, b, M);
        svd3(M, sv);
        so3_rotation(sv, sR);
        if (blockIdx.x == 0) {
#pragma unroll
            for (int e = 0; e < 9; e++) Rout[9 * b + e] = sR[e];
            if (svd_ws) svd_ws_store(sv, svd_ws + SVD_WS * b);
        }
    }
    if (blockIdx.x == 0 && b == 0 && terms && (int)threadIdx.x < nzero) terms[threadIdx.x] = 0.0;
    __syncthreads();
    const float sc = s[b], t0 = t[3 * b], t1 = t[3 * b + 1], t2 = t[3 * b + 2];
    const float tt[3] = {t0, t1, t2};
    float r[9];
#pragma unroll
    for (int e = 0; e < 9; e++) r[e] = sR[e];
    for (int n = blockIdx.x * blockDim.x + threadIdx.x; n < N; n += gridDim.x * blockDim.x) rigid_point(X0p + (size_t)n * 3, r, tt, sc, Xp + ((size_t)b * N + n) * 3);
    if (Xv)
        for (int n = blockIdx.x * blockDim.x + threadIdx.x; n < NV; n += gridDim.x * blockDim.x) rigid_point(X0v + (size_t)n * 3, r, tt, sc, Xv + ((size_t)b * NV + n) * 3);
}
extern "C" int vt_objstep_head(const float *M0, const float *noise, const float *t, const float *s, int B, const float *X0_points, int N, float *X_points,
                               const float *X0_verts, int NV, float *X_verts, float *R, double *terms, int nzero, float *svd_ws, void *stream)
{
    VT_REQUIRE(M0 && t && s && X0_points && X_points && R && B > 0 && N > 0 && (!X_verts || (X0_verts && NV > 0)) && nzero >= 0 && nzero <= 16, "vt_objstep_head: bad argument");
    hipLaunchKernelGGL(objstep_head_kernel, dim3(1, B), dim3(1024), 0, vt_stream(stream), M0, noise, t, s, X0_points, N, X_points, X0_verts, NV, X_verts,
                       R, terms, nzero, svd_ws);
    VT_LAUNCH_CHECK();
    return VT_OK;
}

__device__ __forceinline__ float temporal2_elem(const float *v, int f, int B, int D, int i, float gs_a, float gs_v, float g, double &acc_a, double &acc_v)
{
    float taps[5], ga, gv;
    stencil_taps(v, f, B, D, i, taps);
    acc_a += (double)accel_stencil(taps, f, B, 1.f, gs_a, ga);
    g += ga;
    acc_v += (double)velocity_stencil(taps[1], taps[2], taps[3], f, B, gs_v, gv);
    return g + gv;
}
__global__ __launch_bounds__(256) void temporal2_kernel(const float *__restrict__ v, int B, int D, float gs_a, double *term_a, float gs_v, double *term_v,
                                                        float *__restrict__ dv, int init_zero)
{
    __shared__ double red[4];
    double acc_a = 0, acc_v = 0;
    for (int t = blockIdx.x * 256 + threadIdx.x; t < B * D; t += gridDim.x * 256) {
        const int f = t / D, i = t - f * D;
        dv[(size_t)f * D + i] = temporal2_elem(v, f, B, D, i, gs_a, gs_v, init_zero ? 0.f : dv[(size_t)f * D + i], acc_a, acc_v);
    }
    term_add(acc_a / ((double)(B - 2) * D), term_a, red);
    term_add(acc_v / ((double)(B - 1) * D), term_v, red);
}
extern "C" int vt_temporal_loss2(const float *v, int B, int D, float gscale_accel, double *term_accel, float gscale_velocity, double *term_velocity, float *dv,
                                 int init_zero, void *stream)
{
    VT_REQUIRE(v && dv && B >= 3 && D > 0, "vt_temporal_loss2: bad argument (B >= 3)");
    const float gs_a = 2.f * gscale_accel / ((float)(B - 2) * (float)D), gs_v = 2.f * gscale_velocity / ((float)(B - 1) * (float)D);
    hipLaunchKernelGGL(temporal2_kernel, dim3(min((B * D + 255) / 256, 512)), dim3(256), 0, vt_stream(stream), v, B, D, gs_a, term_accel, gs_v, term_velocity, dv, init_zero);
    VT_LAUNCH_CHECK();
    return VT_OK;
}

struct StepEnd {
    const double *terms_r; double *terms_w; TermW tw; int nterms; float tol; int armed; float *state; int *stop_flag; float *history; int slot;
    int *ticket; int nzero;
};
#ifndef STEP_END_FENCE
#if defined(__HIP_DEVICE_COMPILE__) && !defined(__gfx942__) && !defined(__gfx950__)
#define STEP_END_FENCE 1
#else
#define STEP_END_FENCE 0
#endif
#endif
__device__ __forceinline__ void step_end(const StepEnd &e, int nblocks, bool stopped)
{
    __shared__ int last;
#if STEP_END_FENCE
    __threadfence();
#else
    asm volatile("s_waitcnt vmcnt(0) lgkmcnt(0)" ::: "memory");
#endif
    __syncthreads();
    if (threadIdx.x == 0) last = (atomicAdd(e.ticket, 1) == nblocks - 1);
    __syncthreads();
    if (!last) return;
#if STEP_END_FENCE
    __threadfence();
#endif
    if (threadIdx.x == 0) {
        *e.ticket = 0;
        close_loss<true>(e.terms_r, e.tw, e.nterms, e.tol, e.armed, e.state, e.stop_flag, e.history, e.slot, stopped);
        for (int k = 0; k < e.nzero; k++) e.terms_w[k] = 0.0;
    }
}

struct TemporalIn { const float *X; float gs_a, gs_v; double *term_a, *term_v; int mode; };
__global__ __launch_bounds__(256) void objstep_tail_kernel(TemporalIn tin, const float *__restrict__ X0v, int NV, const float *__restrict__ dXv, const float *__restrict__ X0p, int N,
                                                           const float *__restrict__ dXp, const float *__restrict__ s, const float *__restrict__ M0,
                                                           const float *__restrict__ noise, const float *__restrict__ tpar, const float *__restrict__ t_init,
                                                           float w_trans, double *term_trans, float *__restrict__ dR, float *__restrict__ dt, float *__restrict__ dM,
                                                           AdamSlice aR, AdamSlice aT, float bc2s, float beta1, float beta2, float eps, StepEnd end,
                                                           const float *__restrict__ svd_ws)
{
    __shared__ float red12[4][12];
    __shared__ double redt[4];
    const int b = blockIdx.x, B = gridDim.x;
    const bool stopped = end.stop_flag && *end.stop_flag;
    double acc_a = 0, acc_v = 0;
    const bool rot = aR.p != nullptr;
    const float sc = s[b];
    float svw[SVD_WS];
    if (svd_ws && rot && threadIdx.x == 0) {
#pragma unroll
        for (int e = 0; e < SVD_WS; e++) svw[e] = svd_ws[SVD_WS * b + e];
    }
    const float inv_denom = 1.f / (float)(3 * B);
    float tot[12];
#pragma unroll
    for (int e = 0; e < 12; e++) tot[e] = 0.f;
#pragma unroll
    for (int pass = 0; pass < 2; pass++) {
        const float *X0 = pass == 0 ? X0v : X0p; const float *dX = pass == 0 ? dXv : dXp; const int n_ = pass == 0 ? NV : N;
        if (!dX) continue;
        float a[12];
#pragma unroll
        for (int e = 0; e < 12; e++) a[e] = 0.f;
        for (int n = threadIdx.x; n < n_; n += 256) {
            const float *x = X0 + (size_t)n * 3; const float *g = dX + ((size_t)b * n_ + n) * 3;
            float gt[3];
            if (pass == 1 && tin.mode) {
#pragma unroll
                for (int c = 0; c < 3; c++) gt[c] = temporal2_elem(tin.X, b, B, N * 3, n * 3 + c, tin.gs_a, tin.gs_v, tin.mode == 2 ? 0.f : g[c], acc_a, acc_v);
                g = gt;
            }
            if (rot) rigid_vjp_point<true>(x, g, sc, a); else rigid_vjp_point<false>(x, g, sc, a);
        }
#pragma unroll
        for (int e = 0; e < 12; e++) a[e] = wave_sum(a[e]);
        __syncthreads();
        if ((threadIdx.x & 63) == 0) {
#pragma unroll
            for (int e = 0; e < 12; e++) red12[threadIdx.x >> 6][e] = a[e];
        }
        __syncthreads();
#pragma unroll
        for (int e = 0; e < 12; e++) {
            float v = 0.f;
#pragma unroll
            for (int i = 0; i < 4; i++) v += red12[i][e];
            tot[e] = (pass == 0 || !dXv) ? v : tot[e] + v;
        }
        if (pass == 0 && t_init) {
#pragma unroll
            for (int c = 0; c < 3; c++) { float gr; sqdiff_elem(tpar[3 * b + c], t_init[3 * b + c], inv_denom, w_trans, gr); tot[9 + c] += gr; }
        }
    }
    if (tin.mode) {
        term_add(acc_a / ((double)(B - 2) * (N * 3)), tin.term_a, redt);
        term_add(acc_v / ((double)(B - 1) * (N * 3)), tin.term_v, redt);
    }
    if (threadIdx.x == 0) {
        float g[12];
#pragma unroll
        for (int e = 0; e < 12; e++) g[e] = tot[e];
        if (t_init) {
            double acc = 0;
#pragma unroll
            for (int c = 0; c < 3; c++) { float gr; acc += (double)sqdiff_elem(tpar[3 * b + c], t_init[3 * b + c], inv_denom, w_trans, gr); }
            atomicAdd(term_trans, acc * (double)inv_denom);
        }
#pragma unroll
        for (int c = 0; c < 3; c++) dt[3 * b + c] = g[9 + c];
        if (rot) {
            float M[9]; Svd3 sv;
            if (svd_ws) svd_ws_load(svw, sv);
            else { so3_input(M0, noise, b, M); svd3(M, sv); }
            so3_vjp(sv, g, dM + 9 * b);
#pragma unroll
            for (int e = 0; e < 9; e++) dR[9 * b + e] = g[e];
        }
    }
    __syncthreads();
    if (!stopped) {
        if (aR.p && threadIdx.x < 9) adam_one(aR, b, threadIdx.x, bc2s, beta1, beta2, eps);
        if (aT.p && threadIdx.x >= 64 && threadIdx.x < 67) adam_one(aT, b, threadIdx.x - 64, bc2s, beta1, beta2, eps);
    }
    step_end(end, B, stopped);
}
static StepEnd make_end(double *terms, const float *w, int nterms, float tol, int armed, float *state, int *stop_flag, float *history, int slot, int *ticket, int nzero)
{
    StepEnd e; e.terms_r = terms; e.terms_w = terms; e.nterms = nterms; e.tol = tol; e.armed = armed; e.state = state; e.stop_flag = stop_flag; e.history = history; e.slot = slot;
    e.ticket = ticket; e.nzero = nzero;
    for (int k = 0; k < 16; k++) e.tw.w[k] = k < nterms ? w[k] : 0.f;
    return e;
}
static int objstep_tail_launch(const char *who, const TemporalIn &tin, const float *X0_verts, int NV, const float *dX_verts, const float *X0_points, int N, const float *dX_points,
                               const float *s, int B, const float *M0, const float *noise, const float *t, const float *t_init, float w_trans, double *term_trans,
                               float *dR, float *dt, float *dM,
                               float *pR, float *mR, float *vR, float lrR, float *pT, float *mT, float *vT, float lrT, int adam_step, float beta1, float beta2, float eps,
                               double *terms, const float *w, int nterms, float tol, int armed, float *state, int *stop_flag, float *history, int slot, int *ticket, int nzero,
                               const float *svd_ws, void *stream)
{
    VT_REQUIRE(X0_points && dX_points && s && M0 && t && dR && dt && dM && B > 0 && N > 0 && (!dX_verts || (X0_verts && NV > 0)) && (!t_init || term_trans), "%s: bad argument", who);
    VT_REQUIRE(terms && w && state && ticket && nterms > 0 && nterms <= 16 && nzero >= 0 && nzero <= nterms && adam_step >= 1 && (!pR || (mR && vR)) && (!pT || (mT && vT)),
               "%s: bad optimiser / loss arguments", who);
    double bc1; const float bc2s = adam_bias(beta1, beta2, adam_step, &bc1);
    AdamSlice aR = {pR, 9, dM, 9, mR, vR, 9, (float)(lrR / bc1)}, aT = {pT, 3, dt, 3, mT, vT, 3, (float)(lrT / bc1)};
    hipLaunchKernelGGL(objstep_tail_kernel, dim3(B), dim3(256), 0, vt_stream(stream), tin, X0_verts, NV, dX_verts, X0_points, N, dX_points, s, M0, noise, t, t_init, w_trans, term_trans,
                       dR, dt, dM, aR, aT, bc2s, beta1, beta2, eps, make_end(terms, w, nterms, tol, armed, state, stop_flag, history, slot, ticket, nzero), svd_ws);
    VT_LAUNCH_CHECK();
    return VT_OK;
}
extern "C" int vt_objstep_tail(const float *X0_verts, int NV, const float *dX_verts, const float *X0_points, int N, const float *dX_points, const float *s, int B,
                               const float *M0, const float *noise, const float *t, const float *t_init, float w_trans, double *term_trans,
                               float *dR, float *dt, float *dM,
                               float *pR, float *mR, float *vR, float lrR, float *pT, float *mT, float *vT, float lrT, int adam_step, float beta1, float beta2, float eps,
                               double *terms, const float *w, int nterms, float tol, int armed, float *state, int *stop_flag, float *history, int slot, int *ticket, int nzero,
                               float *svd_ws, void *stream)
{
    return objstep_tail_launch("vt_objstep_tail", TemporalIn{nullptr, 0.f, 0.f, nullptr, nullptr, 0}, X0_verts, NV, dX_verts, X0_points, N, dX_points, s, B, M0, noise, t, t_init, w_trans,
                               term_trans, dR, dt, dM, pR, mR, vR, lrR, pT, mT, vT, lrT, adam_step, beta1, beta2, eps, terms, w, nterms, tol, armed, state, stop_flag, history, slot,
                               ticket, nzero, svd_ws, stream);
}
extern "C" int vt_objstep_tail_temporal(const float *X_points, float gscale_accel, double *term_accel, float gscale_velocity, double *term_velocity, int init_zero,
                                        const float *X0_verts, int NV, const float *dX_verts, const float *X0_points, int N, const float *dX_points, const float *s, int B,
                                        const float *M0, const float *noise, const float *t, const float *t_init, float w_trans, double *term_trans,
                                        float *dR, float *dt, float *dM,
                                        float *pR, float *mR, float *vR, float lrR, float *pT, float *mT, float *vT, float lrT, int adam_step, float beta1, float beta2, float eps,
                                        double *terms, const float *w, int nterms, float tol, int armed, float *state, int *stop_flag, float *history, int slot, int *ticket, int nzero,
                                        float *svd_ws, void *stream)
{
    VT_REQUIRE(X_points && term_accel && term_velocity && B >= 3, "vt_objstep_tail_temporal: bad argument (B >= 3)");
    const int D = N * 3;
    const TemporalIn tin = {X_points, 2.f * gscale_accel / ((float)(B - 2) * (float)D), 2.f * gscale_velocity / ((float)(B - 1) * (float)D), term_accel, term_velocity, init_zero ? 2 : 1};
    return objstep_tail_launch("vt_objstep_tail_temporal", tin, X0_verts, NV, dX_verts, X0_points, N, dX_points, s, B, M0, noise, t, t_init, w_trans, term_trans, dR, dt, dM,
                               pR, mR, vR, lrR, pT, mT, vT, lrT, adam_step, beta1, beta2, eps, terms, w, nterms, tol, armed, state, stop_flag, history, slot, ticket, nzero, svd_ws, stream);
}

__global__ __launch_bounds__(64) void smplstep_tail_kernel(float *__restrict__ pose, const float *__restrict__ pose_init, float *__restrict__ dpose,
                                                           const float *__restrict__ mean, const float *__restrict__ prec, float gscale, double *term_prior,
                                                           float w_pinit, double *term_pinit, AdamSlice a0, AdamSlice a1, AdamSlice a2, float bc2s, float beta1,
                                                           float beta2, float eps, StepEnd end)
{
    __shared__ float d[64], t2[64];
    const int b = blockIdx.x, B = gridDim.x, j = threadIdx.x, n = 63, off = 3, stride = 156;
    const bool stopped = end.stop_flag && *end.stop_flag;
    const float val = mahalanobis_value(pose + (size_t)b * stride + off, n, mean, prec, d, t2);
    __syncthreads();
    mahalanobis_grad(t2, n, prec, dpose + (size_t)b * stride + off, gscale);
    double acc = 0;
    const float inv_denom = 1.f / (float)B;
    for (int c = j; c < 69; c += 64) {
        float g;
        acc += (double)sqdiff_elem(pose[(size_t)b * stride + 3 + c], pose_init[(size_t)b * stride + 3 + c], inv_denom, w_pinit, g);
        dpose[(size_t)b * stride + 3 + c] += g;
    }
    for (int o = 32; o > 0; o >>= 1) acc += __shfl_xor(acc, o, 64);
    if (j == 0) { atomicAdd(term_pinit, acc * (double)inv_denom); atomicAdd(term_prior, (double)val / (double)B); }
    __syncthreads();
    if (!stopped) {
        const AdamSlice *sl[3] = {&a0, &a1, &a2};
#pragma unroll
        for (int k = 0; k < 3; k++)
            if (sl[k]->p) for (int c = j; c < sl[k]->ncols; c += 64) adam_one(*sl[k], b, c, bc2s, beta1, beta2, eps);
    }
    step_end(end, B, stopped);
}
extern "C" int vt_smplstep_tail(float *pose, const float *pose_init, float *dpose, int B, const float *prior_mean, const float *prior_prec, float gscale_prior,
                                double *term_prior, float w_pinit, double *term_pinit,
                                float *p0, int ps0, const float *g0, int gs0, float *m0, float *v0, int n0, float lr0,
                                float *p1, int ps1, const float *g1, int gs1, float *m1, float *v1, int n1, float lr1,
                                float *p2, int ps2, const float *g2, int gs2, float *m2, float *v2, int n2, float lr2,
                                int adam_step, float beta1, float beta2, float eps,
                                double *terms, const float *w, int nterms, float tol, int armed, float *state, int *stop_flag, float *history, int slot, int *ticket, int nzero,
                                void *stream)
{
    VT_REQUIRE(pose && pose_init && dpose && prior_mean && prior_prec && term_prior && term_pinit && B > 0 && adam_step >= 1, "vt_smplstep_tail: bad argument");
    VT_REQUIRE(terms && w && state && ticket && nterms > 0 && nterms <= 16 && nzero >= 0 && nzero <= nterms, "vt_smplstep_tail: bad loss arguments");
    VT_REQUIRE((!p0 || (g0 && m0 && v0 && n0 > 0 && ps0 >= n0 && gs0 >= n0)) && (!p1 || (g1 && m1 && v1 && n1 > 0 && ps1 >= n1 && gs1 >= n1)) &&
               (!p2 || (g2 && m2 && v2 && n2 > 0 && ps2 >= n2 && gs2 >= n2)), "vt_smplstep_tail: a parameter group without its gradient / moments, or a stride below its column count");
    double bc1; const float bc2s = adam_bias(beta1, beta2, adam_step, &bc1);
    AdamSlice a0 = {p0, ps0, g0, gs0, m0, v0, n0, (float)(lr0 / bc1)}, a1 = {p1, ps1, g1, gs1, m1, v1, n1, (float)(lr1 / bc1)}, a2 = {p2, ps2, g2, gs2, m2, v2, n2, (float)(lr2 / bc1)};
    hipLaunchKernelGGL(smplstep_tail_kernel, dim3(B), dim3(64), 0, vt_stream(stream), pose, pose_init, dpose, prior_mean, prior_prec, gscale_prior, term_prior, w_pinit, term_pinit,
                       a0, a1, a2, bc2s, beta1, beta2, eps, make_end(terms, w, nterms, tol, armed, state, stop_flag, history, slot, ticket, nzero));
    VT_LAUNCH_CHECK();
    return VT_OK;
}

__global__ __launch_bounds__(1024) void kpts_step_kernel(const int *__restrict__ indptr, const int *__restrict__ indices, const float *__restrict__ data,
                                                        const int *__restrict__ colptr, const int *__restrict__ rowidx, const float *__restrict__ cdata,
                                                        const float *__restrict__ verts, int V, int K, const float *__restrict__ kpts, const float *__restrict__ cc,
                                                        int mode, Cam5 cam, float net_size, float gscale, float inv_cnt, double *term, float *__restrict__ Jout,
                                                        float *__restrict__ dverts, int accumulate)
{
    __shared__ float sJ[64 * 3], sdJ[64 * 3];
    __shared__ double red[16];
    const int b = blockIdx.x, wave = threadIdx.x >> 6, lane = threadIdx.x & 63, nw = blockDim.x >> 6;
    for (int k = wave; k < K; k += nw) {
        float a[3];
        landmark_row(indptr, indices, data, verts, b, V, k, lane, a);
        if (lane == 0) {
            sJ[3 * k] = a[0]; sJ[3 * k + 1] = a[1]; sJ[3 * k + 2] = a[2];
            if (Jout) { float *o = Jout + ((size_t)b * K + k) * 3; o[0] = a[0]; o[1] = a[1]; o[2] = a[2]; }
        }
    }
    __syncthreads();
    double acc = 0;
    if ((int)threadIdx.x < K) {
        const int k = threadIdx.x;
        acc = (double)kpts_term(sJ + 3 * k, kpts + 3 * (b * K + k), cc, b, mode, cam, net_size, gscale, inv_cnt, sdJ + 3 * k);
    }
    term_add(acc * (double)inv_cnt, term, red);
    for (int v = threadIdx.x; v < V; v += blockDim.x) landmark_col(colptr, rowidx, cdata, sdJ, 0, v, accumulate, dverts + ((size_t)b * V + v) * 3);
}
extern "C" int vt_kpts_step(const vt_landmarks *h, const float *verts, const float *kpts, const float *crop_center, int B, int mode, const float *cam, float net_size,
                            float gscale, double *term, float *J, float *dverts, int accumulate, void *stream)
{
    VT_REQUIRE(h && verts && kpts && cam && dverts && B > 0 && h->K <= 64 && (mode == 0 || (mode == 1 && crop_center)), "vt_kpts_step: bad argument (at most 64 landmarks)");
    Cam5 c{cam[0], cam[1], cam[2], cam[3], cam[4]};
    const float inv_cnt = 1.f / (mode == 0 ? (float)(B * h->K * 2) : (float)(B * h->K));
    hipLaunchKernelGGL(kpts_step_kernel, dim3(B), dim3(1024), 0, vt_stream(stream), h->indptr, h->indices, h->data, h->colptr, h->rowidx, h->cdata, verts, h->V, h->K,
                       kpts, crop_center, mode, c, net_size, gscale, inv_cnt, term, J, dverts, accumulate);
    VT_LAUNCH_CHECK();
    return VT_OK;
}

struct SkipEntry { int dev; hipStream_t st; const int *flag; };
static thread_local std::vector<SkipEntry> t_skip_tab;
static int skip_device() { int d = 0; (void)hipGetDevice(&d); return d; }
const int *vt_skip_flag_of(hipStream_t st)
{
    if (t_skip_tab.empty()) return nullptr;
    const int dev = skip_device();
    for (const auto &e : t_skip_tab) if (e.st == st && e.dev == dev) return e.flag;
    return nullptr;
}
extern "C" int vt_stream_set_skip_flag(void *stream, const int *flag)
{
    const hipStream_t st = vt_stream(stream); const int dev = skip_device();
    for (size_t i = 0; i < t_skip_tab.size(); i++)
        if (t_skip_tab[i].st == st && t_skip_tab[i].dev == dev) {
            if (flag && t_skip_tab[i].flag != flag) VT_FAIL(VT_ERR_BUSY, "vt_stream_set_skip_flag: another stop flag is already registered for this stream by this thread");
            if (!flag) { t_skip_tab[i] = t_skip_tab.back(); t_skip_tab.pop_back(); }
            return VT_OK;
        }
    if (flag) t_skip_tab.push_back({dev, st, flag});
    return VT_OK;
}
```

### vistracker_amd/csrc/step_ops.h

```cpp
#pragma once
#include "common.h"

__device__ __forceinline__ void term_add(double s, double *term, double *red )
{
    for (int o = 32; o > 0; o >>= 1) s += __shfl_xor(s, o, 64);
    const int nw = (blockDim.x + 63) >> 6;
    __syncthreads();
    if ((threadIdx.x & 63) == 0) red[threadIdx.x >> 6] = s;
    __syncthreads();
    if (threadIdx.x == 0) { double t = 0; for (int i = 0; i < nw; i++) t += red[i]; if (term) atomicAdd(term, t); }
}

__device__ __forceinline__ void landmark_row(const int *indptr, const int *indices, const float *data, const float *verts, int b, int V, int k, int lane, float *a)
{
    float a0 = 0.f, a1 = 0.f, a2 = 0.f;
    for (int e = indptr[k] + lane; e < indptr[k + 1]; e += 64) {
        const float w = data[e]; const float *v = verts + ((size_t)b * V + indices[e]) * 3;
        a0 += w * v[0]; a1 += w * v[1]; a2 += w * v[2];
    }
    a[0] = wave_sum(a0); a[1] = wave_sum(a1); a[2] = wave_sum(a2);
}

__device__ __forceinline__ void landmark_col(const int *colptr, const int *rowidx, const float *cdata, const float *dJ, size_t row0, int v, int accumulate, float *o)
{
    const int s = colptr[v], e = colptr[v + 1];
    if (s == e && accumulate) return;
    float a0 = 0.f, a1 = 0.f, a2 = 0.f;
    for (int i = s; i < e; i++) { const float w = cdata[i]; const float *g = dJ + (row0 + rowidx[i]) * 3; a0 += w * g[0]; a1 += w * g[1]; a2 += w * g[2]; }
    if (accumulate) { o[0] += a0; o[1] += a1; o[2] += a2; } else { o[0] = a0; o[1] = a1; o[2] = a2; }
}

__device__ __forceinline__ float mahalanobis_value(const float *x, int n, const float *mean, const float *prec, float *d, float *t2)
{
    const int j = threadIdx.x;
    d[j] = (j < n) ? x[j] - mean[j] : 0.f;
    __syncthreads();
    float a = 0.f;
    if (j < n) for (int i = 0; i < n; i++) a += d[i] * prec[i * n + j];
    t2[j] = a;
    return wave_sum(a * a);
}
__device__ __forceinline__ void mahalanobis_grad(const float *t2, int n, const float *prec, float *dx, float gscale)
{
    const int j = threadIdx.x;
    if (j >= n) return;
    float g = 0.f;
    for (int k = 0; k < n; k++) g += t2[k] * prec[j * n + k];
    dx[j] += 2.f * g * gscale;
}

struct Svd3 { float U[9], V[9], s[3], d; };
#define SVD_WS 22

__device__ __forceinline__ void jacobi_pair(float *A, float *V, const int p, const int q)
{
    float a = 0.f, b = 0.f, g = 0.f;
#pragma unroll
    for (int r = 0; r < 3; r++) { a += A[3 * r + p] * A[3 * r + p]; b += A[3 * r + q] * A[3 * r + q]; g += A[3 * r + p] * A[3 * r + q]; }
    if (fabsf(g) <= 1e-30f) return;
    const float zeta = (b - a) / (2.f * g);
    const float t = (zeta >= 0.f ? 1.f : -1.f) / (fabsf(zeta) + sqrtf(1.f + zeta * zeta));
    const float c = 1.f / sqrtf(1.f + t * t), sn = c * t;
#pragma unroll
    for (int r = 0; r < 3; r++) {
        float x = A[3 * r + p], y = A[3 * r + q]; A[3 * r + p] = c * x - sn * y; A[3 * r + q] = sn * x + c * y;
        x = V[3 * r + p]; y = V[3 * r + q]; V[3 * r + p] = c * x - sn * y; V[3 * r + q] = sn * x + c * y;
    }
}

__device__ __forceinline__ void svd3(const float *M, Svd3 &o)
{
    float A[9], V[9] = {1, 0, 0, 0, 1, 0, 0, 0, 1};
#pragma unroll
    for (int e = 0; e < 9; e++) A[e] = M[e];
    for (int sweep = 0; sweep < 8; sweep++) { jacobi_pair(A, V, 0, 1); jacobi_pair(A, V, 0, 2); jacobi_pair(A, V, 1, 2); }
    float sv[3];
#pragma unroll
    for (int c = 0; c < 3; c++) sv[c] = sqrtf(A[c] * A[c] + A[3 + c] * A[3 + c] + A[6 + c] * A[6 + c]);
#define SWAPC(i, j)                                                                                          \
    if (sv[j] > sv[i]) {                                                                                     \
        float t_ = sv[i]; sv[i] = sv[j]; sv[j] = t_;                                                         \
        for (int r = 0; r < 3; r++) { t_ = A[3 * r + i]; A[3 * r + i] = A[3 * r + j]; A[3 * r + j] = t_;     \
                                      t_ = V[3 * r + i]; V[3 * r + i] = V[3 * r + j]; V[3 * r + j] = t_; }   \
    }
    SWAPC(0, 1) SWAPC(0, 2) SWAPC(1, 2)
#undef SWAPC
#pragma unroll
    for (int c = 0; c < 3; c++) {
        o.s[c] = sv[c];
        const float inv = sv[c] > 0.f ? 1.f / sv[c] : 0.f;
#pragma unroll
        for (int r = 0; r < 3; r++) { o.U[3 * r + c] = A[3 * r + c] * inv; o.V[3 * r + c] = V[3 * r + c]; }
    }
    const float *U = o.U, *W = o.V;
    const float dU = U[0] * (U[4] * U[8] - U[5] * U[7]) - U[1] * (U[3] * U[8] - U[5] * U[6]) + U[2] * (U[3] * U[7] - U[4] * U[6]);
    const float dV = W[0] * (W[4] * W[8] - W[5] * W[7]) - W[1] * (W[3] * W[8] - W[5] * W[6]) + W[2] * (W[3] * W[7] - W[4] * W[6]);
    o.d = dU * dV;
}

__device__ __forceinline__ void so3_input(const float *M0, const float *noise, int b, float *M)
{
#pragma unroll
    for (int e = 0; e < 9; e++) M[e] = M0[9 * b + e] + (noise ? 1e-4f * noise[9 * b + e] : 0.f);
}

__device__ __forceinline__ void so3_rotation(const Svd3 &s, float *R)
{
#pragma unroll
    for (int r = 0; r < 3; r++)
#pragma unroll
        for (int c = 0; c < 3; c++) R[3 * r + c] = s.U[3 * r] * s.V[3 * c] + s.U[3 * r + 1] * s.V[3 * c + 1] + s.d * s.U[3 * r + 2] * s.V[3 * c + 2];
}

__device__ __forceinline__ void so3_vjp(const Svd3 &s, const float *G, float *dM)
{
    const float D[3] = {1.f, 1.f, s.d}, h[3] = {s.s[0], s.s[1], s.d * s.s[2]};
    float UtG[9], Q[9], Z[9], UDZ[9];
#pragma unroll
    for (int r = 0; r < 3; r++)
#pragma unroll
        for (int c = 0; c < 3; c++) UtG[3 * r + c] = s.U[r] * G[c] + s.U[3 + r] * G[3 + c] + s.U[6 + r] * G[6 + c];
#pragma unroll
    for (int r = 0; r < 3; r++)
#pragma unroll
        for (int c = 0; c < 3; c++) Q[3 * r + c] = D[r] * (UtG[3 * r] * s.V[c] + UtG[3 * r + 1] * s.V[3 + c] + UtG[3 * r + 2] * s.V[6 + c]);
#pragma unroll
    for (int r = 0; r < 3; r++)
#pragma unroll
        for (int c = 0; c < 3; c++) Z[3 * r + c] = (r == c) ? 0.f : (Q[3 * r + c] - Q[3 * c + r]) / (h[r] + h[c]);
#pragma unroll
    for (int r = 0; r < 3; r++)
#pragma unroll
        for (int c = 0; c < 3; c++) UDZ[3 * r + c] = s.U[3 * r] * D[0] * Z[c] + s.U[3 * r + 1] * D[1] * Z[3 + c] + s.U[3 * r + 2] * D[2] * Z[6 + c];
#pragma unroll
    for (int r = 0; r < 3; r++)
#pragma unroll
        for (int c = 0; c < 3; c++) dM[3 * r + c] = UDZ[3 * r] * s.V[3 * c] + UDZ[3 * r + 1] * s.V[3 * c + 1] + UDZ[3 * r + 2] * s.V[3 * c + 2];
}

__device__ __forceinline__ void svd_ws_store(const Svd3 &s, float *o)
{
#pragma unroll
    for (int e = 0; e < 9; e++) { o[e] = s.U[e]; o[9 + e] = s.V[e]; }
    o[18] = s.s[0]; o[19] = s.s[1]; o[20] = s.s[2]; o[21] = s.d;
}
__device__ __forceinline__ void svd_ws_load(const float *w, Svd3 &s)
{
#pragma unroll
    for (int e = 0; e < 9; e++) { s.U[e] = w[e]; s.V[e] = w[9 + e]; }
    s.s[0] = w[18]; s.s[1] = w[19]; s.s[2] = w[20]; s.d = w[21];
}

__device__ __forceinline__ void rigid_point(const float *x, const float *r, const float *t, float sc, float *o)
{
    const float x0 = x[0], x1 = x[1], x2 = x[2];
#pragma unroll
    for (int c = 0; c < 3; c++) o[c] = (x0 * r[c] + x1 * r[3 + c] + x2 * r[6 + c] + t[c]) * sc;
}
template <bool ROT>
__device__ __forceinline__ void rigid_vjp_point(const float *x, const float *g, float sc, float *a)
{
#pragma unroll
    for (int c = 0; c < 3; c++) {
        const float gc = g[c] * sc; a[9 + c] += gc;
        if (ROT) { a[c] += x[0] * gc; a[3 + c] += x[1] * gc; a[6 + c] += x[2] * gc; }
    }
}

__device__ __forceinline__ void stencil_taps(const float *v, int f, int B, int D, int i, float *o)
{
#pragma unroll
    for (int k = 0; k < 5; k++) o[k] = v[(size_t)min(max(f - 2 + k, 0), B - 1) * D + i];
}
__device__ __forceinline__ float accel_stencil(const float *o, int f, int B, float w, float gs, float &grad)
{
    const float vm2 = o[0], vm1 = o[1], v0 = o[2], vp1 = o[3], vp2 = o[4];
    const float a_m = (f - 1 >= 1 && f - 1 <= B - 2) ? 2.f * vm1 - vm2 - v0 : 0.f;
    const float a_0 = (f >= 1 && f <= B - 2) ? 2.f * v0 - vm1 - vp1 : 0.f;
    const float a_p = (f + 1 >= 1 && f + 1 <= B - 2) ? 2.f * vp1 - v0 - vp2 : 0.f;
    grad = gs * w * (2.f * a_0 - a_m - a_p);
    return w * a_0 * a_0;
}
__device__ __forceinline__ float velocity_stencil(float vm1, float v0, float vp1, int f, int B, float gs, float &grad)
{
    const float d0 = f >= 1 ? v0 - vm1 : 0.f;
    const float d1 = f + 1 < B ? vp1 - v0 : 0.f;
    grad = gs * (d0 - d1);
    return d0 * d0;
}

struct Cam5 { float fx, fy, cx, cy, crop; };
__device__ __forceinline__ float kpts_term(const float *J, const float *kp, const float *cc, int b, int mode, const Cam5 &cam, float net_size, float gscale, float inv_cnt, float *dJ)
{
    const float x = J[0], y = J[1], z = J[2];
    float px = cam.fx * x / z + cam.cx, py = cam.fy * y / z + cam.cy, sc = 1.f;
    if (mode == 1) {
        px = cam.crop / 2 + px - cc[2 * b]; py = cam.crop / 2 + py - cc[2 * b + 1];
        sc = net_size / cam.crop; px *= sc; py *= sc;
    }
    const float ex = px - kp[0], ey = py - kp[1], conf = kp[2];
    const float gpx = 2.f * ex * conf * gscale * inv_cnt * sc, gpy = 2.f * ey * conf * gscale * inv_cnt * sc;
    dJ[0] = gpx * cam.fx / z; dJ[1] = gpy * cam.fy / z;
    dJ[2] = -gpx * cam.fx * x / (z * z) - gpy * cam.fy * y / (z * z);
    return (ex * ex + ey * ey) * conf;
}

__device__ __forceinline__ float sqdiff_elem(float a, float b, float inv_denom, float gscale, float &grad)
{
    const float d = a - b;
    grad = 2.f * d * inv_denom * gscale;
    return d * d;
}

__device__ __forceinline__ void adam_update(float &p, float gi, float &m, float &v, float step_size, float bc2s, float beta1, float beta2, float eps)
{
    const float mi = m * beta1 + (1.f - beta1) * gi;
    const float vi = v * beta2 + (1.f - beta2) * gi * gi;
    m = mi; v = vi;
    const float denom = sqrtf(vi) / bc2s + eps;
    p = p - step_size * (mi / denom);
}
struct AdamSlice { float *p; int pstride; const float *g; int gstride; float *m, *v; int ncols; float step_size; };
__device__ __forceinline__ void adam_one(const AdamSlice &a, int b, int c, float bc2s, float beta1, float beta2, float eps)
{
    const int i = b * a.ncols + c;
    adam_update(a.p[(size_t)b * a.pstride + c], a.g[(size_t)b * a.gstride + c], a.m[i], a.v[i], a.step_size, bc2s, beta1, beta2, eps);
}

struct TermW { float w[16]; };
template <bool ATOMIC>
__device__ __forceinline__ void close_loss(const double *terms, const TermW &tw, int nterms, float tol, int armed, float *state, int *stop_flag, float *history, int slot,
                                           bool stopped)
{
    if (stopped) { if (history) history[slot] = nanf(""); return; }
    double l = 0;
    for (int k = 0; k < nterms; k++) l += (double)tw.w[k] * (ATOMIC ? __hip_atomic_load(terms + k, __ATOMIC_RELAXED, __HIP_MEMORY_SCOPE_AGENT) : terms[k]);
    const float loss = (float)l, prev = state[0];
    if (history) history[slot] = loss;
    if (armed && stop_flag && (fabsf(prev - loss) / prev < prev * tol)) *stop_flag = 1;
    state[0] = loss; state[1] = loss;
}

struct vt_landmarks { int K, V; int *indptr, *indices; float *data; int *colptr, *rowidx; float *cdata; };
static inline float adam_bias(float beta1, float beta2, int step, double *bc1)
{
    *bc1 = 1.0 - pow((double)beta1, step);
    return (float)sqrt(1.0 - pow((double)beta2, step));
}
```

### vistracker_amd/fitting.py

```python
from __future__ import annotations

import contextlib
import ctypes as C
import functools
import os
import threading
import time
from dataclasses import dataclass, field

import numpy as np
import torch

from . import _lib as L
from . import ops

FIT_WEIGHTS = {"pose": 1e-5, "hand": 1e-5, "j2d": 0.09, "object": 900.0, "part": 0.0025, "contact": 900.0, "scale": 100.0,
               "df_h": 100.0, "mask": 0.0009, "ocent": 0.0, "pinit": 25.0, "rot": 100.0, "trans": 100.0,
               "stemp": 10000.0, "otemp": 225.0, "ovtemp": 2500.0, "collide": 9.0}
SMPLT_WEIGHTS = {"pose": 1e-5, "hand": 1e-5, "kpts": 0.09, "temp": 900.0, "ptemp": 25.0, "pinit": 900.0}
JOINT_WEIGHTS_66 = np.repeat(np.array([1, 10, 10, 10, 5, 5, 10, 1, 1, 10, 1, 1, 5, 5, 5, 5, 5, 5, 1, 1, 1, 1], np.float32), 3)
JOINT_WEIGHTS_66[37:39] = 10.0


def _lib():
    return L.lib()


def _chk(rc):
    L.check(rc)


def _ev_begin(prof):
    if prof is None:
        return None
    e = torch.cuda.Event(enable_timing=True); e.record()
    return e


def _flush_events(prof, local, executed):
    if prof is None:
        return
    for k, v in local.items():
        prof[k].extend((a, b, n) for a, b, n, step in v if executed is None or step < executed)


def _ev_end(prof, key, e0, frames, step):
    if prof is None:
        return
    e1 = torch.cuda.Event(enable_timing=True); e1.record()
    prof[key].append((e0, e1, frames, step))


class Terms:

    def __init__(self, names, device):
        self.names = list(names)
        self.buf = torch.zeros(len(self.names), dtype=torch.float64, device=device)
        self.idx = {n: i for i, n in enumerate(self.names)}

    def ptr(self, name):
        return self.buf.data_ptr() + 8 * self.idx[name]

    def zero(self, first=0, count=None):
        count = len(self.names) - first if count is None else count
        _chk(_lib().vt_fill_f64(self.buf.data_ptr() + 8 * first, count, 0.0, L.stream_ptr()))

    def weights(self, table, decay, extra=None):
        w = np.zeros(16, np.float32)
        for n, i in self.idx.items():
            w[i] = table[n] / (1.0 + decay) * (1.0 if extra is None else extra.get(n, 1.0))
        return w


class AdamState:

    def __init__(self, slices, stop_flag):
        self.slices = slices
        self.m = [torch.zeros(p.shape[0], n, device=p.device) for p, n, g, lr in slices]
        self.v = [torch.zeros(p.shape[0], n, device=p.device) for p, n, g, lr in slices]
        self.t = 0
        self.stop_flag = stop_flag

    def tick(self):
        self.t += 1
        return self.t

    def step(self):
        t = self.tick()
        for (p, n, g, lr), m, v in zip(self.slices, self.m, self.v):
            _chk(_lib().vt_adam_step_2d(p.data_ptr(), p.shape[1], g.data_ptr(), g.shape[1], m.data_ptr(), v.data_ptr(), p.shape[0], n,
                                        t, lr, 0.9, 0.999, 1e-8, self.stop_flag.data_ptr(), L.stream_ptr()))

    @functools.cached_property
    def smpl_tail_groups(self):
        out = ()
        for (p, n, g, lr), m, v in zip(self.slices, self.m, self.v):
            out += (p.data_ptr(), p.shape[1], g.data_ptr(), g.shape[1], m.data_ptr(), v.data_ptr(), n, lr)
        return out + (None, 0, None, 0, None, None, 0, 0.0) * (3 - len(self.slices))

    @functools.cached_property
    def object_tail_groups(self):
        rot = trans = (None, None, None, 0.0)
        for (p, n, g, lr), m, v in zip(self.slices, self.m, self.v):
            if n == 9:
                rot = (p.data_ptr(), m.data_ptr(), v.data_ptr(), lr)
            else:
                trans = (p.data_ptr(), m.data_ptr(), v.data_ptr(), lr)
        return rot + trans


def _check_finite(res, what):
    executed = res.losses[:res.steps]
    if executed.size and not np.isfinite(executed).all():
        bad = int(np.flatnonzero(~np.isfinite(executed))[0])
        raise FloatingPointError(f"{what}: non-finite loss at Adam step {bad} (non-finite input or decoder activation out of range)")


def _as_input(t, dev):
    if t is None:
        return None
    return torch.as_tensor(t).to(device=dev, dtype=torch.float32).contiguous()


def _require_params(*ts):
    for t in ts:
        if not (torch.is_tensor(t) and t.is_cuda and t.dtype == torch.float32 and t.is_contiguous()):
            raise L.VtError("fit loops update their parameters in place: pass contiguous float32 CUDA tensors "
                            f"(got {type(t).__name__} {getattr(t, 'dtype', None)} on {getattr(t, 'device', None)})")
        if t.device != ts[0].device:
            raise L.VtError("fit loops: all parameters must live on the same device")


@dataclass
class FitResult:
    steps: int = 0
    outer_iters: int = 0
    stopped_early: bool = False
    losses: np.ndarray = field(default_factory=lambda: np.zeros(0, np.float32))


def morton_order(points) -> np.ndarray:
    p = np.asarray(points, np.float64)
    q = ((p - p.min(0)) / (p.max(0) - p.min(0) + 1e-12) * 1023).astype(np.int64)

    def part(x):
        x = (x | (x << 16)) & 0x030000FF; x = (x | (x << 8)) & 0x0300F00F; x = (x | (x << 4)) & 0x030C30C3
        return (x | (x << 2)) & 0x09249249
    return np.argsort(part(q[:, 0]) | (part(q[:, 1]) << 1) | (part(q[:, 2]) << 2), kind="stable")


def morton_order_device(p: torch.Tensor) -> torch.Tensor:
    p = p.double()
    lo = p.min(0).values; hi = p.max(0).values
    q = ((p - lo) / (hi - lo + 1e-12) * 1023).long()

    def part(x):
        x = (x | (x << 16)) & 0x030000FF; x = (x | (x << 8)) & 0x0300F00F; x = (x | (x << 4)) & 0x030C30C3
        return (x | (x << 2)) & 0x09249249
    key = part(q[:, 0]) | (part(q[:, 1]) << 1)
    if p.shape[1] > 2:
        key = key | (part(q[:, 2]) << 2)
    return torch.argsort(key, stable=True).to(torch.int32)


class _StopWatch:
    _tls = threading.local()

    def __init__(self, ctx, stop, lookahead):
        self.ctx, self.stop, self.look = ctx, stop, lookahead
        self.pending = None; self.n = 0
        if lookahead:
            pool = getattr(self._tls, "pool", None)
            if pool is None or pool[0] != stop.device:
                pool = (stop.device, torch.zeros(2, dtype=torch.int32).pin_memory(), [torch.cuda.Event(), torch.cuda.Event()])
                self._tls.pool = pool
            _, self.host, self.ev = pool

    def _wait(self, k):
        t0 = time.perf_counter()
        self.ev[k].synchronize()
        with self.ctx._counter_lock:
            self.ctx.host_wait_s += time.perf_counter() - t0
        return bool(int(self.host[k]))

    def check(self):
        if not self.look:
            return bool(self.ctx._read_stop(self.stop))
        k = self.n & 1; self.n += 1
        self.host[k:k + 1].copy_(self.stop, non_blocking=True); self.ev[k].record()
        prev, self.pending = self.pending, k
        return prev is not None and self._wait(prev)

    def final(self):
        if not self.look or self.pending is None:
            return False
        k, self.pending = self.pending, None
        return self._wait(k)


class _Fit:

    def __init__(self, dev, names, nsteps, prev_loss, prof):
        self.terms = Terms(names, dev)
        self.stop = torch.zeros(1, dtype=torch.int32, device=dev)
        self.loss_state = torch.full((2,), prev_loss, device=dev)
        self.ticket = torch.zeros(1, dtype=torch.int32, device=dev)
        self.hist = torch.full((nsteps,), float("nan"), device=dev)
        self.lp = {"human": [], "object": []} if prof is not None else None
        self.adam = None


class _SmplFit(_Fit):

    def __init__(self, pose, betas, trans, names, nsteps, prev_loss, prof=None, smpl=None):
        dev = pose.device; B = self.B = pose.shape[0]
        super().__init__(dev, names, nsteps, prev_loss, prof)
        self.pose, self.betas, self.trans = pose, betas, trans
        self.verts = torch.empty(B, 6890, 3, device=dev); self.jtr = torch.empty(B, 52, 3, device=dev); self.vposed = torch.empty_like(self.verts)
        self.ws = torch.empty(_lib().vt_smplh_workspace_floats(B), device=dev); self.scratch = torch.empty(_lib().vt_smplh_bwd_scratch_floats(B), device=dev)
        self.dverts = torch.empty_like(self.verts); self.J = torch.empty(B, 25, 3, device=dev); self.dJ = torch.empty_like(self.J)
        self.dpose = torch.empty(B, 156, device=dev); self.dbetas = torch.empty(B, 10, device=dev); self.dtrans = torch.empty(B, 3, device=dev)
        self.vb = torch.empty(B, device=dev)
        self.pose_init = pose.clone()
        self.prefix, self.n_free = None, 156
        if smpl is not None:
            self.prefix = torch.empty(_lib().vt_smplh_prefix_floats(B), device=dev); self.n_free = 66
            _chk(_lib().vt_smplh_prefix(smpl.h, pose.data_ptr(), B, self.ws.data_ptr(), self.prefix.data_ptr(), L.stream_ptr()))
            self.dpose.zero_()

    @property
    def vert_order_ptr(self):
        return self.vert_order.data_ptr() if self.vert_order is not None else None


class _ObjectFit(_Fit):

    def __init__(self, ctx, obj_R, obj_t, sil, nsteps, prof):
        dev = obj_R.device; B = self.B = obj_R.shape[0]; N = self.N = ctx.obj_points.shape[0]; NV = self.NV = ctx.obj_verts.shape[0]
        super().__init__(dev, ["object", "otemp", "ovtemp", "mask", "trans", "contact", "collide", "scale"], nsteps, 300.0, prof)
        self.obj_R, self.obj_t, self.sil = obj_R, obj_t, sil
        self.R = torch.empty(B, 3, 3, device=dev); self.X = torch.empty(B, N, 3, device=dev); self.dX = torch.empty_like(self.X)
        self.svd_ws = torch.empty(B, 22, device=dev)
        self.dR = torch.empty(B, 3, 3, device=dev); self.dM = torch.empty(B, 3, 3, device=dev); self.dt = torch.empty(B, 3, device=dev)
        if sil is not None:
            self.Vt = torch.empty(B, NV, 3, device=dev); self.dVt = torch.empty_like(self.Vt)
            self.fidx = torch.empty(B, sil.size, sil.size, dtype=torch.int32, device=dev); self.dimg = torch.empty(B, sil.size, sil.size, device=dev)
            self.sws = torch.empty(_lib().vt_sil_workspace_floats(B, NV, ctx.obj_faces.shape[0], sil.size), device=dev)
            if not ctx.fused_steps:
                self.img = torch.empty_like(self.dimg); self.per = torch.empty(B, device=dev)
        self.trans_init = None
        self.Vc = self.cws = None
        self.contact = None


class FitContext:
    use_projection = True
    sort_object_points = True
    sort_query_points = True
    collision_loss = False
    fused_steps = os.environ.get("VT_FUSED_STEPS", "1") != "0"
    fused_smpl_query = os.environ.get("VT_FUSED_SMPL_QUERY", "0") != "0"
    device_skip = os.environ.get("VT_DEVICE_SKIP", "1") != "0"
    frozen_hands = True

    def __init__(self, smpl_model, regressors, priors, decoders=None, part_labels=None, obj_verts=None, obj_faces=None, obj_points=None,
                 cam=ops.DEFAULT_CAM, device="cuda:0"):
        self.device = torch.device(device)
        dev = self.device
        self.smpl = ops.SmplhHandle(smpl_model, dev)
        self.b25 = ops.LandmarkHandle(regressors["body25"], dev)
        self.net = ops.SifNetHandle(decoders, cam, dev) if decoders is not None else None
        self.cam = np.ascontiguousarray(cam, np.float32)
        t = lambda a, dt=torch.float32: None if a is None else torch.as_tensor(np.ascontiguousarray(a), dtype=dt, device=dev)
        self.pri = {k: t(v) for k, v in priors.items()}
        self.labels = t(part_labels, torch.int32)
        self.vert_order = t(morton_order(np.asarray(smpl_model["v_template"])), torch.int32) if self.sort_query_points else None
        if obj_points is not None and self.sort_object_points:
            obj_points = np.asarray(obj_points, np.float32)[morton_order(obj_points)]
        self.obj_verts = t(obj_verts); self.obj_faces = t(obj_faces, torch.int32); self.obj_points = t(obj_points)
        self.smpl_faces = t(np.asarray(smpl_model["f"]).astype(np.int32), torch.int32) if "f" in smpl_model else None
        self.jw66 = t(JOINT_WEIGHTS_66)

    range_retries = 0
    fp32_fallbacks = 0
    _counter_lock = threading.Lock()
    host_wait_s = 0.0

    def _with_range_fallback(self, maps, params, run):
        if self.net is None or maps is None or maps.force_fp32 or self.net.precision == "fp32":
            return run()
        saved = [p.clone() for p in params]
        while True:
            try:
                return run()
            except FloatingPointError as e:
                import warnings
                for p, s0 in zip(params, saved):
                    p.copy_(s0)
                if maps.act_level + 1 < maps.ACT_LEVELS:
                    maps.set_act_level(maps.act_level + 1)
                    warnings.warn(f"{e}; repeating the fit at operand-range level {maps.act_level} of the split-f16 decoders", RuntimeWarning)
                    with self._counter_lock:
                        self.range_retries += 1
                    continue
                if maps.force_fp32:
                    raise
                warnings.warn(f"{e}; repeating the fit on the strict-fp32 decoder kernels (5x slower)", RuntimeWarning)
                maps.set_force_fp32(True)
                with self._counter_lock:
                    self.fp32_fallbacks += 1
                return run()

    def smpl_forward(self, pose, betas, trans, verts, jtr, vposed, ws, prefix=None):
        if prefix is not None:
            _chk(_lib().vt_smplh_forward_prefixed(self.smpl.h, pose.data_ptr(), betas.data_ptr(), trans.data_ptr(), pose.shape[0], prefix.data_ptr(),
                                                  verts.data_ptr(), jtr.data_ptr(), vposed.data_ptr(), ws.data_ptr(), L.stream_ptr()))
            return
        _chk(_lib().vt_smplh_forward(self.smpl.h, pose.data_ptr(), betas.data_ptr(), trans.data_ptr(), pose.shape[0], verts.data_ptr(),
                                     jtr.data_ptr(), vposed.data_ptr(), ws.data_ptr(), L.stream_ptr()))

    def smpl_backward(self, pose, betas, dverts, vposed, ws, scratch, dpose, dbetas, dtrans, n_free=156):
        if n_free < 156:
            _chk(_lib().vt_smplh_backward_free(self.smpl.h, pose.data_ptr(), pose.shape[0], dverts.data_ptr(), None, vposed.data_ptr(), ws.data_ptr(),
                                               scratch.data_ptr(), n_free, dpose.data_ptr(), dbetas.data_ptr(), dtrans.data_ptr(), L.stream_ptr()))
            return
        _chk(_lib().vt_smplh_backward(self.smpl.h, pose.data_ptr(), betas.data_ptr(), pose.shape[0], dverts.data_ptr(), None, vposed.data_ptr(),
                                      ws.data_ptr(), scratch.data_ptr(), dpose.data_ptr(), dbetas.data_ptr(), dtrans.data_ptr(), L.stream_ptr()))

    def hand_prior_value(self, pose, terms, name, scratch_b):
        B = pose.shape[0]
        for off, m, p in ((66, "lhand_mean", "lhand_prec"), (111, "rhand_mean", "rhand_prec")):
            _chk(_lib().vt_mahalanobis(pose.data_ptr(), B, 156, off, 45, self.pri[m].data_ptr(), self.pri[p].data_ptr(), scratch_b.data_ptr(), None, 0.0, L.stream_ptr()))
            _chk(_lib().vt_sum_to_term(scratch_b.data_ptr(), B, 1.0 / 45.0, terms.ptr(name), L.stream_ptr()))

    def body_prior(self, pose, dpose, w, terms, name, scratch_b):
        B = pose.shape[0]
        _chk(_lib().vt_mahalanobis(pose.data_ptr(), B, 156, 3, 63, self.pri["body_mean"].data_ptr(), self.pri["body_prec"].data_ptr(),
                                   scratch_b.data_ptr(), dpose.data_ptr(), w / B, L.stream_ptr()))
        _chk(_lib().vt_sum_to_term(scratch_b.data_ptr(), B, 1.0 / B, terms.ptr(name), L.stream_ptr()))

    def _run_fit(self, f, start, end, check_every, outer, prof=None):
        res = FitResult()
        with self._skip_after_stop(f.stop) as skipping:
            watch = _StopWatch(self, f.stop, skipping)
            for it in range(start, end):
                step, phase, w, armed = outer(it)
                for i in range(10):
                    step(f, phase, (it - start) * 10 + i, w, armed)
                res.steps += 10
                res.outer_iters += 1
                if (it - start) % check_every == check_every - 1 and watch.check():
                    res.stopped_early = True
                    break
            res.stopped_early = res.stopped_early or watch.final()
        res.losses = f.hist.cpu().numpy()
        if res.stopped_early:
            res.steps = int(np.isfinite(res.losses).sum())
            res.outer_iters = -(-res.steps // 10)
        _flush_events(prof, f.lp, res.steps if (res.stopped_early and self.device_skip) else None)
        _check_finite(res, "fit")
        return res

    def fit_smplt(self, pose, betas, trans, kpts, max_iter=100, iter_for_global=8, temporal=True, pinit_w=900.0,
                  lr_global=0.01, lr_all=0.001, it_range=None, check_every=1, weights=None, early_stop=True):
        with torch.cuda.device(pose.device):
            return self._fit_smplt(pose, betas, trans, kpts, max_iter, iter_for_global, temporal, pinit_w, lr_global, lr_all, it_range, check_every, weights, early_stop)

    def _fit_smplt(self, pose, betas, trans, kpts, max_iter, iter_for_global, temporal, pinit_w, lr_global, lr_all, it_range, check_every, weights, early_stop=True):
        _require_params(pose, betas, trans)
        table = dict(SMPLT_WEIGHTS); table["pinit"] = pinit_w
        if weights is not None:
            table.update({k: float(v) for k, v in weights.items() if k in table})
        start, end = it_range if it_range is not None else (0, max_iter)
        f = _SmplFit(pose, betas, trans, ["kpts", "temp", "ptemp", "pose", "pinit", "hand"], (end - start) * 10, 0.0,
                     smpl=self.smpl if self.frozen_hands else None)
        f.kpts = _as_input(kpts, pose.device)
        f.temporal = temporal and f.B >= 3
        self.hand_prior_value(pose, f.terms, "hand", f.vb)

        def outer(it):
            if f.adam is None or it == iter_for_global:
                if it < iter_for_global:
                    f.adam = AdamState([(trans, 3, f.dtrans, lr_global), (pose, 3, f.dpose, lr_global), (betas, 2, f.dbetas, lr_global)], f.stop)
                else:
                    f.adam = AdamState([(trans, 3, f.dtrans, lr_all), (pose, 66, f.dpose, lr_all), (betas, 10, f.dbetas, lr_all)], f.stop)
            return self._smplt_step, None, f.terms.weights(table, it // 3), int(early_stop and it > 0.3 * max_iter)
        return self._run_fit(f, start, end, check_every, outer)

    def optimize_smpl(self, maps, pose, betas, trans, crop_center, body_center, body_kpts, max_iter=100, iter_for_betas=1,
                      iter_for_pose=1, iter_for_kpts=1, it_range=None, net_size=512.0, check_every=1, prof=None, early_stop=True):
        with torch.cuda.device(pose.device):
            return self._with_range_fallback(maps, (pose, betas, trans), lambda: self._optimize_smpl(
                maps, pose, betas, trans, crop_center, body_center, body_kpts, max_iter, iter_for_betas, iter_for_pose, iter_for_kpts, it_range, net_size,
                check_every, prof, early_stop))

    def _optimize_smpl(self, maps, pose, betas, trans, crop_center, body_center, body_kpts, max_iter, iter_for_betas, iter_for_pose, iter_for_kpts,
                       it_range, net_size, check_every, prof, early_stop=True):
        dev = pose.device
        _require_params(pose, betas, trans)
        split_route = self.net.precision != "fp32" and not maps.force_fp32
        if self.use_projection and split_route:
            maps.build_projection(self.net)
        total = iter_for_betas + iter_for_kpts + iter_for_pose + max_iter
        start, end = it_range if it_range is not None else (0, total)
        f = _SmplFit(pose, betas, trans, ["df_h", "part", "pose", "pinit", "j2d", "stemp", "hand"], (end - start) * 10, 300.0, prof,
                     smpl=self.smpl if self.frozen_hands else None)
        f.maps, f.net_size = maps, net_size
        f.crop_center, f.body_center, f.body_kpts = _as_input(crop_center, dev), _as_input(body_center, dev), _as_input(body_kpts, dev)
        f.vert_order = self.vert_order
        if self.sort_query_points:
            self.smpl_forward(pose, betas, trans, f.verts, f.jtr, f.vposed, f.ws, f.prefix)
            v0 = f.verts[f.B // 2]
            f.vert_order = morton_order_device(torch.stack([v0[:, 0] / v0[:, 2], v0[:, 1] / v0[:, 2]], 1))
        self.hand_prior_value(pose, f.terms, "hand", f.vb)
        if not self.fused_steps:
            step = self._smpl_step
        elif split_route and self.fused_smpl_query:
            step = self._smpl_step_fused_query
        else:
            step = self._smpl_step_fused
        arm_after = 0.25 * max_iter + iter_for_betas + iter_for_pose

        def outer(it):
            if it < iter_for_betas:
                phase = "global"
                if f.adam is None:
                    f.adam = AdamState([(betas, 2, f.dbetas, 0.02), (trans, 3, f.dtrans, 0.02)], f.stop)
            else:
                phase = "kpts" if it >= iter_for_betas + iter_for_pose else "smpl all pose"
                if f.adam is None or it == iter_for_betas:
                    f.adam = AdamState([(trans, 3, f.dtrans, 0.006), (pose, 66, f.dpose, 0.006), (betas, 10, f.dbetas, 0.006)], f.stop)
            return step, phase, f.terms.weights(FIT_WEIGHTS, 1 if phase != "kpts" else it / 3), int(early_stop and it > arm_after)
        return self._run_fit(f, start, end, check_every, outer, prof)

    def optimize_smpl_object(self, maps, smpl_verts, obj_R, obj_t, obj_s, crop_center, body_center, occ, sil=None, noise=None,
                             iter_for_obj=15, iter_for_sil=30, joint_iter=10, max_iter=100, it_range=None, seed=0, check_every=1, prof=None, early_stop=True):
        with torch.cuda.device(obj_R.device):
            return self._with_range_fallback(maps, (obj_R, obj_t), lambda: self._optimize_smpl_object(
                maps, smpl_verts, obj_R, obj_t, obj_s, crop_center, body_center, occ, sil, noise, iter_for_obj, iter_for_sil, joint_iter, max_iter, it_range,
                seed, check_every, prof, early_stop))

    def _optimize_smpl_object(self, maps, smpl_verts, obj_R, obj_t, obj_s, crop_center, body_center, occ, sil, noise, iter_for_obj, iter_for_sil,
                              joint_iter, max_iter, it_range, seed, check_every, prof, early_stop=True):
        dev = obj_R.device; B = obj_R.shape[0]
        _require_params(obj_R, obj_t)
        if self.use_projection and self.net.precision != "fp32" and not maps.force_fp32:
            maps.build_projection(self.net, reuse=True)
        total = joint_iter + iter_for_obj + max_iter + iter_for_sil
        start, end = it_range if it_range is not None else (0, total)
        f = _ObjectFit(self, obj_R, obj_t, sil, (end - start) * 10, prof)
        f.maps = maps
        f.smpl_verts, f.obj_s, f.crop_center, f.body_center, f.occ = (_as_input(x, dev) for x in (smpl_verts, obj_s, crop_center, body_center, occ))
        f.obj_s = f.obj_s.reshape(-1)
        if noise is not None:
            f.noise = _as_input(noise, dev)
        else:
            gen = torch.Generator(device=dev); gen.manual_seed(seed)
            f.noise = torch.rand((end - start) * 10, B, 3, 3, device=dev, generator=gen)
        ones = torch.ones_like(f.obj_s)
        _chk(_lib().vt_sqdiff_loss(f.obj_s.data_ptr(), 1, ones.data_ptr(), 1, B, 1, float(B), 0.0, f.terms.ptr("scale"), None, L.stream_ptr()))
        Rv, dMv = obj_R.view(B, 9), f.dM.view(B, 9)

        def outer(it):
            if it < iter_for_obj:
                phase = "object only"
                if f.adam is None:
                    f.adam = AdamState([(Rv, 9, dMv, 0.002), (obj_t, 3, f.dt, 0.006)], f.stop)
            elif it < iter_for_obj + iter_for_sil:
                phase = "sil"
                if sil is None:
                    raise L.VtError("phase 'sil' needs a SilSetup")
                if f.adam is None or it == iter_for_obj:
                    f.adam = AdamState([(Rv, 9, dMv, 0.006), (obj_t, 3, f.dt, 0.006)], f.stop)
                    f.trans_init = obj_t.clone()
            else:
                phase = "joint"
                if f.adam is None or it == iter_for_obj + iter_for_sil:
                    f.adam = AdamState([(obj_t, 3, f.dt, 0.002)], f.stop)
            decay = 1 if phase == "object only" else (it - iter_for_obj + 1 if phase == "sil" else (it - iter_for_obj + 1) / 3)
            tw = 10.0 if phase == "joint" else 1.0
            w = f.terms.weights(FIT_WEIGHTS, decay, {"otemp": tw, "ovtemp": tw})
            fused = self.fused_steps and not (phase == "joint" and self.collision_loss)
            return (self._object_step_fused if fused else self._object_step), phase, w, int(early_stop and phase == "joint" and it > 0.25 * max_iter)
        return self._run_fit(f, start, end, check_every, outer, prof)

    def _read_stop(self, stop):
        t0 = time.perf_counter()
        v = int(stop.item())
        with self._counter_lock:
            self.host_wait_s += time.perf_counter() - t0
        return v

    @contextlib.contextmanager
    def _skip_after_stop(self, stop):
        if not self.device_skip:
            yield False
            return
        sp = L.stream_ptr()
        rc = _lib().vt_stream_set_skip_flag(sp, stop.data_ptr())
        if rc == L.VT_ERR_BUSY:
            yield False
            return
        L.check(rc)
        try:
            yield True
        finally:
            _lib().vt_stream_set_skip_flag(sp, None)

    def _smplt_step(self, f, phase, k, w, armed):
        lib = _lib(); st = L.stream_ptr(); B = f.B; pose = f.pose
        f.terms.zero(0, 5)
        self.smpl_forward(pose, f.betas, f.trans, f.verts, f.jtr, f.vposed, f.ws, f.prefix)
        _chk(lib.vt_landmarks_forward(self.b25.h, f.verts.data_ptr(), B, f.J.data_ptr(), st))
        _chk(lib.vt_kpts_loss(f.J.data_ptr(), f.kpts.data_ptr(), None, B, 25, 0, self.cam.ctypes.data, 0.0, float(w[0]), f.terms.ptr("kpts"), f.dJ.data_ptr(), st))
        _chk(lib.vt_landmarks_backward(self.b25.h, f.dJ.data_ptr(), B, f.dverts.data_ptr(), 0, st))
        if f.temporal:
            _chk(lib.vt_accel_loss(f.verts.data_ptr(), B, 6890 * 3, None, float(w[1]), f.terms.ptr("temp"), f.dverts.data_ptr(), st))
        self.smpl_backward(pose, f.betas, f.dverts, f.vposed, f.ws, f.scratch, f.dpose, f.dbetas, f.dtrans, f.n_free)
        if f.temporal:
            _chk(lib.vt_accel_loss_strided(pose.data_ptr(), B, 66, 156, self.jw66.data_ptr(), float(w[2]), f.terms.ptr("ptemp"), f.dpose.data_ptr(), st))
        self.body_prior(pose, f.dpose, float(w[3]), f.terms, "pose", f.vb)
        _chk(lib.vt_sqdiff_loss(pose.data_ptr() + 12, 156, f.pose_init.data_ptr() + 12, 156, B, 63, float(B * 63), float(w[4]),
                                f.terms.ptr("pinit"), f.dpose.data_ptr() + 12, st))
        f.adam.step()
        _chk(lib.vt_loss_reduce_and_stop(f.terms.buf.data_ptr(), w.ctypes.data, len(f.terms.names), 1e-3, armed, f.loss_state.data_ptr(),
                                         f.stop.data_ptr(), f.hist.data_ptr(), k, st))

    def _human_query(self, f, k, w):
        ev = _ev_begin(f.lp)
        _chk(_lib().vt_query_human_loss(self.net.h, C.byref(f.maps.c), f.verts.data_ptr(), f.crop_center.data_ptr(), f.body_center.data_ptr(), f.B, 6890,
                                        self.labels.data_ptr(), f.vert_order_ptr, float(w[0]), float(w[1]), f.dverts.data_ptr(), f.terms.ptr("df_h"),
                                        L.stream_ptr()))
        _ev_end(f.lp, "human", ev, f.B, k)

    def _smpl_step(self, f, phase, k, w, armed):
        lib = _lib(); st = L.stream_ptr(); B = f.B; pose = f.pose
        f.terms.zero(0, 6)
        self.smpl_forward(pose, f.betas, f.trans, f.verts, f.jtr, f.vposed, f.ws, f.prefix)
        self._human_query(f, k, w)
        if phase == "kpts":
            _chk(lib.vt_landmarks_forward(self.b25.h, f.verts.data_ptr(), B, f.J.data_ptr(), st))
            _chk(lib.vt_kpts_loss(f.J.data_ptr(), f.body_kpts.data_ptr(), f.crop_center.data_ptr(), B, 25, 1, self.cam.ctypes.data, f.net_size,
                                  float(w[4]), f.terms.ptr("j2d"), f.dJ.data_ptr(), st))
            _chk(lib.vt_landmarks_backward(self.b25.h, f.dJ.data_ptr(), B, f.dverts.data_ptr(), 1, st))
        if B >= 4:
            _chk(lib.vt_accel_loss(f.verts.data_ptr(), B, 6890 * 3, None, float(w[5]), f.terms.ptr("stemp"), f.dverts.data_ptr(), st))
        self.smpl_backward(pose, f.betas, f.dverts, f.vposed, f.ws, f.scratch, f.dpose, f.dbetas, f.dtrans, f.n_free)
        self.body_prior(pose, f.dpose, float(w[2]), f.terms, "pose", f.vb)
        _chk(lib.vt_sqdiff_loss(pose.data_ptr() + 12, 156, f.pose_init.data_ptr() + 12, 156, B, 69, float(B), float(w[3]),
                                f.terms.ptr("pinit"), f.dpose.data_ptr() + 12, st))
        f.adam.step()
        _chk(lib.vt_loss_reduce_and_stop(f.terms.buf.data_ptr(), w.ctypes.data, len(f.terms.names), 1e-3, armed, f.loss_state.data_ptr(),
                                         f.stop.data_ptr(), f.hist.data_ptr(), k, st))

    def _smpl_step_fused(self, f, phase, k, w, armed):
        lib = _lib(); st = L.stream_ptr(); B = f.B
        self.smpl_forward(f.pose, f.betas, f.trans, f.verts, f.jtr, f.vposed, f.ws, f.prefix)
        self._human_query(f, k, w)
        if phase == "kpts":
            _chk(lib.vt_kpts_step(self.b25.h, f.verts.data_ptr(), f.body_kpts.data_ptr(), f.crop_center.data_ptr(), B, 1, self.cam.ctypes.data, f.net_size,
                                  float(w[4]), f.terms.ptr("j2d"), f.J.data_ptr(), f.dverts.data_ptr(), 1, st))
        if B >= 4:
            _chk(lib.vt_accel_loss(f.verts.data_ptr(), B, 6890 * 3, None, float(w[5]), f.terms.ptr("stemp"), f.dverts.data_ptr(), st))
        self.smpl_backward(f.pose, f.betas, f.dverts, f.vposed, f.ws, f.scratch, f.dpose, f.dbetas, f.dtrans, f.n_free)
        self._smpl_tail(f, k, w, armed)

    def _smpl_step_fused_query(self, f, phase, k, w, armed):
        lib = _lib(); st = L.stream_ptr(); B = f.B
        self.smpl_forward(f.pose, f.betas, f.trans, f.verts, f.jtr, f.vposed, f.ws, f.prefix)
        if phase == "kpts":
            _chk(lib.vt_kpts_step(self.b25.h, f.verts.data_ptr(), f.body_kpts.data_ptr(), f.crop_center.data_ptr(), B, 1, self.cam.ctypes.data, f.net_size,
                                  float(w[4]), f.terms.ptr("j2d"), f.J.data_ptr(), f.dverts.data_ptr(), 0, st))
        ev = _ev_begin(f.lp)
        _chk(lib.vt_query_human_step(self.net.h, C.byref(f.maps.c), f.verts.data_ptr(), f.crop_center.data_ptr(), f.body_center.data_ptr(), B, 6890,
                                     self.labels.data_ptr(), f.vert_order_ptr, float(w[0]), float(w[1]), int(phase == "kpts"), float(w[5]),
                                     f.terms.ptr("stemp") if B >= 4 else None, f.dverts.data_ptr(), f.terms.ptr("df_h"), st))
        _ev_end(f.lp, "human", ev, B, k)
        self.smpl_backward(f.pose, f.betas, f.dverts, f.vposed, f.ws, f.scratch, f.dpose, f.dbetas, f.dtrans, f.n_free)
        self._smpl_tail(f, k, w, armed)

    def _smpl_tail(self, f, k, w, armed):
        _chk(_lib().vt_smplstep_tail(f.pose.data_ptr(), f.pose_init.data_ptr(), f.dpose.data_ptr(), f.B, self.pri["body_mean"].data_ptr(),
                                     self.pri["body_prec"].data_ptr(), float(w[2]) / f.B, f.terms.ptr("pose"), float(w[3]), f.terms.ptr("pinit"),
                                     *f.adam.smpl_tail_groups, f.adam.tick(), 0.9, 0.999, 1e-8,
                                     f.terms.buf.data_ptr(), w.ctypes.data, len(f.terms.names), 1e-3, armed, f.loss_state.data_ptr(), f.stop.data_ptr(),
                                     f.hist.data_ptr(), k, f.ticket.data_ptr(), 6, L.stream_ptr()))

    def _object_query(self, f, k, w):
        ev = _ev_begin(f.lp)
        _chk(_lib().vt_query_object_loss(self.net.h, C.byref(f.maps.c), f.X.data_ptr(), f.crop_center.data_ptr(), f.body_center.data_ptr(), f.B, f.N,
                                         f.occ.data_ptr(), float(w[0]), f.dX.data_ptr(), f.terms.ptr("object"), L.stream_ptr()))
        _ev_end(f.lp, "object", ev, f.B, k)

    def _contacts(self, f, w):
        if f.contact is None:
            f.contact = self._contacts_once(f.maps, f.smpl_verts, f.X, f.crop_center, f.body_center)
        if f.contact["P"] > 0:
            self._contact_term(f.contact, f.X, f.dX, float(w[5]), f.terms)

    def _object_step(self, f, phase, k, w, armed):
        lib = _lib(); st = L.stream_ptr(); B, N, NV, nz = f.B, f.N, f.NV, f.noise[k]
        obj_R, obj_t, obj_s, X, dX, R, dR, dt = f.obj_R, f.obj_t, f.obj_s, f.X, f.dX, f.R, f.dR, f.dt
        nf = self.obj_faces.shape[0]
        f.terms.zero(0, 7)
        _chk(lib.vt_so3_project_forward(obj_R.data_ptr(), nz.data_ptr(), B, R.data_ptr(), st))
        _chk(lib.vt_rigid_forward(self.obj_points.data_ptr(), 1, R.data_ptr(), obj_t.data_ptr(), obj_s.data_ptr(), B, N, X.data_ptr(), st))
        if phase == "sil":
            _chk(lib.vt_fill(dX.data_ptr(), dX.numel(), 0.0, st))
        else:
            self._object_query(f, k, w)
        if B >= 4:
            _chk(lib.vt_accel_loss(X.data_ptr(), B, N * 3, None, float(w[1]), f.terms.ptr("otemp"), dX.data_ptr(), st))
            _chk(lib.vt_velocity_loss(X.data_ptr(), B, N * 3, float(w[2]), f.terms.ptr("ovtemp"), dX.data_ptr(), st))
        acc = 0
        if phase == "sil":
            sil = f.sil
            _chk(lib.vt_rigid_forward(self.obj_verts.data_ptr(), 1, R.data_ptr(), obj_t.data_ptr(), obj_s.data_ptr(), B, NV, f.Vt.data_ptr(), st))
            _chk(lib.vt_sil_forward(f.Vt.data_ptr(), B, NV, self.obj_faces.data_ptr(), nf, sil.K.data_ptr(), sil.size, f.img.data_ptr(), f.fidx.data_ptr(),
                                    f.sws.data_ptr(), st))
            _chk(lib.vt_sil_mask_loss(f.img.data_ptr(), sil.keep.data_ptr(), sil.ref.data_ptr(), f.occ.data_ptr(), B, sil.size, float(w[3]),
                                      f.terms.ptr("mask"), f.per.data_ptr(), f.dimg.data_ptr(), st))
            _chk(lib.vt_sil_backward(f.Vt.data_ptr(), B, NV, self.obj_faces.data_ptr(), nf, sil.K.data_ptr(), sil.size, f.fidx.data_ptr(), f.dimg.data_ptr(),
                                     1e-4, f.sws.data_ptr(), f.dVt.data_ptr(), st))
            _chk(lib.vt_rigid_backward(self.obj_verts.data_ptr(), 1, obj_s.data_ptr(), B, NV, f.dVt.data_ptr(), dR.data_ptr(), dt.data_ptr(), 0, st))
            _chk(lib.vt_sqdiff_loss(obj_t.data_ptr(), 3, f.trans_init.data_ptr(), 3, B, 3, float(B * 3), float(w[4]), f.terms.ptr("trans"), dt.data_ptr(), st))
            acc = 1
        if phase == "joint":
            self._contacts(f, w)
        _chk(lib.vt_rigid_backward(self.obj_points.data_ptr(), 1, obj_s.data_ptr(), B, N, dX.data_ptr(), dR.data_ptr(), dt.data_ptr(), acc, st))
        if phase == "joint" and self.collision_loss:
            if f.cws is None:
                f.Vc = torch.empty(B, NV, 3, device=X.device)
                f.cws = torch.empty((lib.vt_collision_workspace_bytes(B, self.smpl_faces.shape[0]) + 7) // 8, dtype=torch.int64, device=X.device)
            _chk(lib.vt_rigid_forward(self.obj_verts.data_ptr(), 1, R.data_ptr(), obj_t.data_ptr(), obj_s.data_ptr(), B, NV, f.Vc.data_ptr(), st))
            _chk(lib.vt_collision_loss(f.smpl_verts.data_ptr(), f.smpl_verts.shape[1], self.smpl_faces.data_ptr(), self.smpl_faces.shape[0], f.Vc.data_ptr(), NV,
                                       self.obj_faces.data_ptr(), nf, B, 0.5, 8, float(w[6]), f.terms.ptr("collide"), dt.data_ptr(), None, f.cws.data_ptr(), st))
        _chk(lib.vt_so3_project_backward(obj_R.data_ptr(), nz.data_ptr(), B, dR.data_ptr(), f.dM.data_ptr(), st))
        f.adam.step()
        _chk(lib.vt_loss_reduce_and_stop(f.terms.buf.data_ptr(), w.ctypes.data, len(f.terms.names), 1e-4, armed, f.loss_state.data_ptr(), f.stop.data_ptr(),
                                         f.hist.data_ptr(), k, st))

    def _object_step_fused(self, f, phase, k, w, armed):
        lib = _lib(); st = L.stream_ptr(); B, N, NV, nz = f.B, f.N, f.NV, f.noise[k]
        is_sil = phase == "sil"
        X, dX = f.X.data_ptr(), f.dX.data_ptr()
        obj_verts, Vt, dVt = (self.obj_verts.data_ptr(), f.Vt.data_ptr(), f.dVt.data_ptr()) if is_sil else (None, None, None)
        _chk(lib.vt_objstep_head(f.obj_R.data_ptr(), nz.data_ptr(), f.obj_t.data_ptr(), f.obj_s.data_ptr(), B, self.obj_points.data_ptr(), N, X,
                                 obj_verts, NV, Vt, f.R.data_ptr(), f.terms.buf.data_ptr(), 7, f.svd_ws.data_ptr(), st))
        if not is_sil:
            self._object_query(f, k, w)
        tail_temporal = B >= 4 and phase != "joint"
        if B >= 4 and phase == "joint":
            _chk(lib.vt_temporal_loss2(X, B, N * 3, float(w[1]), f.terms.ptr("otemp"), float(w[2]), f.terms.ptr("ovtemp"), dX, 0, st))
        elif is_sil and B < 4:
            _chk(lib.vt_fill(dX, f.dX.numel(), 0.0, st))
        if is_sil:
            sil = f.sil
            _chk(lib.vt_sil_step(Vt, B, NV, self.obj_faces.data_ptr(), self.obj_faces.shape[0], sil.K.data_ptr(), sil.size, sil.keep.data_ptr(),
                                 sil.ref.data_ptr(), f.occ.data_ptr(), float(w[3]), 1e-4, f.terms.ptr("mask"), f.fidx.data_ptr(), f.dimg.data_ptr(),
                                 f.sws.data_ptr(), dVt, st))
        if phase == "joint":
            self._contacts(f, w)
        tail, pre = lib.vt_objstep_tail, ()
        if tail_temporal:
            tail, pre = lib.vt_objstep_tail_temporal, (X, float(w[1]), f.terms.ptr("otemp"), float(w[2]), f.terms.ptr("ovtemp"), int(is_sil))
        _chk(tail(*pre, obj_verts, NV, dVt, self.obj_points.data_ptr(), N, dX, f.obj_s.data_ptr(), B, f.obj_R.data_ptr(), nz.data_ptr(), f.obj_t.data_ptr(),
                  f.trans_init.data_ptr() if is_sil else None, float(w[4]), f.terms.ptr("trans"), f.dR.data_ptr(), f.dt.data_ptr(), f.dM.data_ptr(),
                  *f.adam.object_tail_groups, f.adam.tick(), 0.9, 0.999, 1e-8, f.terms.buf.data_ptr(), w.ctypes.data, len(f.terms.names), 1e-4, armed,
                  f.loss_state.data_ptr(), f.stop.data_ptr(), f.hist.data_ptr(), k, f.ticket.data_ptr(), 0, f.svd_ws.data_ptr(), st))

    def _contact_term(self, contact, X, dX, w, terms):
        _chk(_lib().vt_chamfer_ragged_idx(contact["x"].data_ptr(), contact["offx"].data_ptr(), contact["x"].shape[0], X.data_ptr(), contact["idx_o32"].data_ptr(),
                                          contact["offy"].data_ptr(), contact["idx_o32"].shape[0], contact["P"], w, terms.ptr("contact"), dX.data_ptr(),
                                          contact["ws"].data_ptr(), int(not contact["planned"]), L.stream_ptr()))
        contact["planned"] = True

    def _contacts_once(self, maps, smpl_verts, X, crop_center, body_center, thres=0.08):
        B, N = X.shape[:2]; V = smpl_verts.shape[1]; dev = X.device
        df_o, _, parts_o, _, _ = ops.sifnet_query(self.net, maps, X, crop_center, body_center, head_mask=0b00101)
        df_h, _, _, _, _ = ops.sifnet_query(self.net, maps, smpl_verts, crop_center, body_center, head_mask=0b00001)
        mask_o = df_o[:, 0] < thres
        mask_h = df_h[:, 1] < thres
        lab_o = parts_o.argmax(1)
        lab_h = self.labels.long().unsqueeze(0).expand(B, V)
        oh = torch.zeros(B, 14, device=dev, dtype=torch.long); oo = torch.zeros_like(oh)
        oh.scatter_add_(1, lab_h, mask_h.long()); oo.scatter_add_(1, lab_o, mask_o.long())
        pair = (oh > 0) & (oo > 0)
        P = int(pair.sum().item())
        if P == 0:
            return {"P": 0}
        sel_h = mask_h & pair.gather(1, lab_h); sel_o = mask_o & pair.gather(1, lab_o)
        bh, vh = sel_h.nonzero(as_tuple=True); bo, no = sel_o.nonzero(as_tuple=True)
        cnt_h = (oh * pair).reshape(-1); cnt_o = (oo * pair).reshape(-1)
        keep = pair.reshape(-1)
        ch, co = cnt_h[keep], cnt_o[keep]
        perm = torch.argsort(ch * co, descending=True, stable=True)
        rank_of_key = torch.zeros(B * 14, dtype=torch.long, device=dev)
        rank_of_key[keep.nonzero(as_tuple=True)[0][perm]] = torch.arange(P, device=dev)
        kh = rank_of_key[bh * 14 + lab_h[bh, vh]]; ko = rank_of_key[bo * 14 + lab_o[bo, no]]
        oh_s = torch.sort(kh, stable=True); oo_s = torch.sort(ko, stable=True)
        idx_h = (bh * V + vh)[oh_s.indices]; idx_o = (bo * N + no)[oo_s.indices]
        offx = torch.zeros(P + 1, dtype=torch.int32, device=dev); offy = torch.zeros(P + 1, dtype=torch.int32, device=dev)
        offx[1:] = torch.cumsum(ch[perm], 0).int(); offy[1:] = torch.cumsum(co[perm], 0).int()
        x = smpl_verts.reshape(-1, 3).index_select(0, idx_h).contiguous()
        ws = torch.empty(int(_lib().vt_chamfer_ws_bytes(x.shape[0], idx_o.shape[0], P)), dtype=torch.uint8, device=dev)
        return {"P": P, "x": x, "offx": offx, "offy": offy, "idx_o": idx_o, "idx_o32": idx_o.int().contiguous(), "ws": ws, "planned": False}


class SilSetup:

    def __init__(self, K, keep, ref, size=256):
        self.K, self.keep, self.ref, self.size = K.contiguous(), keep.contiguous(), ref.contiguous(), size
```

Measured before the change: 152.4.

## Fuse SMPL backward frame, step tail and next pose kernel into one close kernel

```diff
diff --git a/include/vistracker.h b/include/vistracker.h
--- a/include/vistracker.h
+++ b/include/vistracker.h
@@ -44,6 +44,11 @@
                               float *verts, float *jtr, float *v_posed, float *ws, void *stream);
 int vt_smplh_backward_free(const vt_smplh *h, const float *pose, int B, const float *dverts, const float *djtr, const float *v_posed,
                            const float *ws, float *scratch, int n_free_pose_cols, float *dpose, float *dbetas, float *dtrans, void *stream);
+
+int vt_smplh_forward_verts(const vt_smplh *h, const float *betas, const float *trans, int B, const float *prefix, float *verts, float *v_posed,
+                           const float *ws, void *stream);
+int vt_smplh_backward_gemms(const vt_smplh *h, int B, const float *dverts, const float *v_posed, const float *ws, float *scratch, int n_free_pose_cols,
+                            void *stream);
 
 int vt_rodrigues_forward(const float *aa, int n, float *R, void *stream);
 int vt_rodrigues_backward(const float *aa, int n, const float *dR, float *daa, void *stream);
@@ -169,6 +174,16 @@
                      int adam_step, float beta1, float beta2, float eps,
                      double *terms, const float *w, int nterms, float tol, int armed, float *state, int *stop_flag, float *history, int slot, int *ticket, int nzero,
                      void *stream);
+int vt_smplstep_close(const vt_smplh *h, float *pose, float *betas, float *trans, int B, const float *djtr, float *ws, const float *scratch,
+                      int n_free_pose_cols, float *dpose, float *dbetas, float *dtrans, int prefixed, float *jtr,
+                      const float *pose_init, const float *prior_mean, const float *prior_prec, float gscale_prior, double *term_prior, float w_pinit,
+                      double *term_pinit,
+                      float *p0, int ps0, const float *g0, int gs0, float *m0, float *v0, int n0, float lr0,
+                      float *p1, int ps1, const float *g1, int gs1, float *m1, float *v1, int n1, float lr1,
+                      float *p2, int ps2, const float *g2, int gs2, float *m2, float *v2, int n2, float lr2,
+                      int adam_step, float beta1, float beta2, float eps,
+                      double *terms, const float *w, int nterms, float tol, int armed, float *state, int *stop_flag, float *history, int slot, int *ticket, int nzero,
+                      void *stream);
 
 int vt_so3_project_forward(const float *M0, const float *noise, int B, float *R, void *stream);
 int vt_so3_project_backward(const float *M0, const float *noise, int B, const float *dR, float *dM, void *stream);
diff --git a/vistracker_amd/_lib.py b/vistracker_amd/_lib.py
--- a/vistracker_amd/_lib.py
+++ b/vistracker_amd/_lib.py
@@ -32,6 +32,12 @@
     "vt_smplh_prefix": (ci, [vp, fp, ci, fp, fp, vp]),
     "vt_smplh_forward_prefixed": (ci, [vp, fp, fp, fp, ci, fp, fp, fp, fp, fp, vp]),
     "vt_smplh_backward_free": (ci, [vp, fp, ci, fp, fp, fp, fp, fp, ci, fp, fp, fp, vp]),
+    "vt_smplh_forward_verts": (ci, [vp, fp, fp, ci, fp, fp, fp, fp, vp]),
+    "vt_smplh_backward_gemms": (ci, [vp, ci, fp, fp, fp, fp, ci, vp]),
+    "vt_smplstep_close": (ci, [vp, fp, fp, fp, ci, fp, fp, fp, ci, fp, fp, fp, ci, fp,
+                               fp, fp, fp, cf, fp, cf, fp,
+                               fp, ci, fp, ci, fp, fp, ci, cf, fp, ci, fp, ci, fp, fp, ci, cf, fp, ci, fp, ci, fp, fp, ci, cf, ci, cf, cf, cf,
+                               fp, vp, ci, cf, ci, fp, fp, fp, ci, fp, ci, vp]),
     "vt_rodrigues_forward": (ci, [fp, ci, fp, vp]),
     "vt_rodrigues_backward": (ci, [fp, ci, fp, fp, vp]),
     "vt_landmarks_create": (ci, [C.POINTER(vp), vp, vp, vp, ci, ci, vp]),
diff --git a/vistracker_amd/csrc/smplh.hip b/vistracker_amd/csrc/smplh.hip
--- a/vistracker_amd/csrc/smplh.hip
+++ b/vistracker_amd/csrc/smplh.hip
@@ -1,4 +1,4 @@
-#include "common.h"
+#include "step_ops.h"
 #include <cstring>
 
 #define V_ VT_SMPL_V
@@ -108,15 +108,11 @@
     daa[3 * i] = d[0]; daa[3 * i + 1] = d[1]; daa[3 * i + 2] = d[2];
 }
 
-__global__ __launch_bounds__(64) void smplh_pose_kernel(const float *__restrict__ pose, const float *__restrict__ betas,
-                                                        const float *__restrict__ trans, const float *__restrict__ J_t,
-                                                        const float *__restrict__ J_s, SmplParents par,
-                                                        float *__restrict__ ws, float *__restrict__ jtr, int rod_lo, int rod_hi, int chain,
-                                                        const int *skip)
-{
-    VT_SKIP_RETURN(skip);
+__device__ __forceinline__ void smplh_pose_frame(const float *pose, const float *betas, const float *trans, const float *J_t, const float *J_s,
+                                                 const SmplParents &par, float *ws, float *jtr, int rod_lo, int rod_hi, int chain, int b)
+{
     __shared__ float sR[J_ * 9], sJ[J_ * 3], sG[J_ * 12];
-    const int b = blockIdx.x, j = threadIdx.x;
+    const int j = threadIdx.x;
     float *w = ws + (size_t)b * WS_FRAME;
     if (j < J_) {
         float R[9];
@@ -148,7 +144,7 @@
     if (j < J_) sPar[j] = par.p[j];
     __syncthreads();
     int lvl = 0, maxl = 0;
-    if (j < J_) { for (int q = j; q != 0; q = sPar[q]) lvl++; }
+    if ((j & 63) < J_) { for (int q = j & 63; q != 0; q = sPar[q]) lvl++; }
     maxl = lvl;
     for (int o = 32; o > 0; o >>= 1) maxl = max(maxl, __shfl_xor(maxl, o, 64));
     maxl = __builtin_amdgcn_readfirstlane(maxl);
@@ -182,6 +178,15 @@
             if (jtr) jtr[(b * J_ + j) * 3 + r] = gt + trans[3 * b + r];
         }
     }
+}
+__global__ __launch_bounds__(64) void smplh_pose_kernel(const float *__restrict__ pose, const float *__restrict__ betas,
+                                                        const float *__restrict__ trans, const float *__restrict__ J_t,
+                                                        const float *__restrict__ J_s, SmplParents par,
+                                                        float *__restrict__ ws, float *__restrict__ jtr, int rod_lo, int rod_hi, int chain,
+                                                        const int *skip)
+{
+    VT_SKIP_RETURN(skip);
+    smplh_pose_frame(pose, betas, trans, J_t, J_s, par, ws, jtr, rod_lo, rod_hi, chain, blockIdx.x);
 }
 
 #define FWD_FB 16
@@ -473,17 +478,13 @@
     }
 }
 
-__global__ __launch_bounds__(256) void smplh_bwd_frame_kernel(const float *__restrict__ pose, const float *__restrict__ J_s,
-                                                              SmplParents par, const float *__restrict__ ws,
-                                                              const float *__restrict__ part, const float *__restrict__ part3,
-                                                              const float *__restrict__ djtr, int B, int n_free, float *__restrict__ dpose,
-                                                              float *__restrict__ dbetas, float *__restrict__ dtrans, const int *skip)
-{
-    VT_SKIP_RETURN(skip);
+__device__ __forceinline__ void smplh_bwd_frame(const float *pose, const float *J_s, const SmplParents &par, const float *ws, const float *part,
+                                                const float *part3, const float *djtr, int B, int n_free, float *dpose, float *dbetas, float *dtrans, int b)
+{
     __shared__ float red[PT_N], red3[NQ_];
     __shared__ float sdG[J_ * 12], sdJ[J_ * 3], sdR[J_ * 9];
     __shared__ float sG[J_ * 12], sRm[J_ * 9], sJr[J_ * 3];
-    const int b = blockIdx.x, tid = threadIdx.x;
+    const int tid = threadIdx.x;
     const float *w = ws + (size_t)b * WS_FRAME;
     for (int i = tid; i < J_ * 12; i += 256) sG[i] = w[WS_G + i];
     for (int i = tid; i < J_ * 9; i += 256) sRm[i] = w[WS_R + i];
@@ -566,6 +567,33 @@
         dtrans[b * 3 + c] = s;
     }
 }
+__global__ __launch_bounds__(256) void smplh_bwd_frame_kernel(const float *__restrict__ pose, const float *__restrict__ J_s,
+                                                              SmplParents par, const float *__restrict__ ws,
+                                                              const float *__restrict__ part, const float *__restrict__ part3,
+                                                              const float *__restrict__ djtr, int B, int n_free, float *__restrict__ dpose,
+                                                              float *__restrict__ dbetas, float *__restrict__ dtrans, const int *skip)
+{
+    VT_SKIP_RETURN(skip);
+    smplh_bwd_frame(pose, J_s, par, ws, part, part3, djtr, B, n_free, dpose, dbetas, dtrans, blockIdx.x);
+}
+
+struct CloseSmplh { const float *J_t, *J_s, *part, *part3, *djtr; float *ws, *jtr; int n_free, rod_hi; };
+struct CloseTail { const float *pose_init, *mean, *prec; float gscale; double *term_prior; float w_pinit; double *term_pinit; float bc2s, beta1, beta2, eps; };
+__global__ __launch_bounds__(256) void smplstep_close_kernel(float *pose, float *betas, float *trans, float *dpose, float *dbetas, float *dtrans, SmplParents par,
+                                                             CloseSmplh m, CloseTail t, AdamSlice a0, AdamSlice a1, AdamSlice a2, StepEnd end, const int *skip)
+{
+    const int b = blockIdx.x, B = gridDim.x;
+    const bool stopped = end.stop_flag && *end.stop_flag;
+    const bool skipped = skip != nullptr && *(volatile const int *)skip != 0;
+    if (!skipped) smplh_bwd_frame(pose, m.J_s, par, m.ws, m.part, m.part3, m.djtr, B, m.n_free, dpose, dbetas, dtrans, b);
+    __syncthreads();
+    if (threadIdx.x >= 64) return;
+    smplstep_tail_frame<64>(pose, t.pose_init, dpose, t.mean, t.prec, t.gscale, t.term_prior, t.w_pinit, t.term_pinit, a0, a1, a2, t.bc2s, t.beta1, t.beta2, t.eps,
+                             b, B, stopped);
+    __syncthreads();
+    if (!stopped && !skipped) smplh_pose_frame(pose, betas, trans, m.J_t, m.J_s, par, m.ws, m.jtr, 0, m.rod_hi, 1, b);
+    step_end(end, B, stopped);
+}
 
 extern "C" int vt_smplh_create(vt_smplh **out, const float *v_template, const float *shapedirs, const float *posedirs,
                                const float *J_regressor, const float *weights, const int *parents, void *stream)
@@ -659,12 +687,14 @@
 
 #define FWD_LDS_FLOATS(w_) (FWD_R0 + FWD_FB * 64 * 3 + (w_) + FWD_FB * 3)
 static int smplh_forward_launch(int mode, const vt_smplh *h, const float *pose, const float *betas, const float *trans, int B, float *verts, float *jtr,
-                                float *v_posed, float *ws, float *prefix, hipStream_t st)
+                                float *v_posed, float *ws, float *prefix, hipStream_t st, bool pose_launch = true)
 {
     const int *skip = mode == 1 ? nullptr : vt_skip_flag_of(st);
-    hipLaunchKernelGGL(smplh_pose_kernel, dim3(B), dim3(64), 0, st, pose, betas, trans, h->J_t, h->J_s, h->par, ws, jtr, mode == 1 ? J_LIVE_ : 0,
-                       mode == 2 ? J_LIVE_ : J_, mode == 1 ? 0 : 1, skip);
-    VT_LAUNCH_CHECK();
+    if (pose_launch) {
+        hipLaunchKernelGGL(smplh_pose_kernel, dim3(B), dim3(64), 0, st, pose, betas, trans, h->J_t, h->J_s, h->par, ws, jtr, mode == 1 ? J_LIVE_ : 0,
+                           mode == 2 ? J_LIVE_ : J_, mode == 1 ? 0 : 1, skip);
+        VT_LAUNCH_CHECK();
+    }
     const size_t lds_f = sizeof(float) * FWD_LDS_FLOATS(h->nnz > 0 ? 2 * SP_K * 64 : J_ * 64), lds_max = sizeof(float) * FWD_LDS_FLOATS(J_ * 64);
     const dim3 grid(VP_ / 64, (B + FWD_FB - 1) / FWD_FB);
     if (mode == 0) {
@@ -703,7 +733,7 @@
 }
 
 static int smplh_backward_launch(const vt_smplh *h, const float *pose, int B, const float *dverts, const float *djtr, const float *v_posed, const float *ws,
-                                 float *scratch, int n_free, float *dpose, float *dbetas, float *dtrans, hipStream_t st)
+                                 float *scratch, int n_free, float *dpose, float *dbetas, float *dtrans, hipStream_t st, bool frame_launch = true)
 {
     const int *skip = vt_skip_flag_of(st);
     const size_t lds = sizeof(float) * (256 * 13 + BWD_FB * 624);
@@ -715,6 +745,7 @@
     hipLaunchKernelGGL(smplh_bwd_blend_kernel, dim3(NKS_, (ntiles + 4 * BL_NW - 1) / (4 * BL_NW), (B + BL_M - 1) / BL_M), dim3(256), 0, st, h->Q_t, dvp_g, B, ntiles,
                        part3, skip);
     VT_LAUNCH_CHECK();
+    if (!frame_launch) return VT_OK;
     hipLaunchKernelGGL(smplh_bwd_frame_kernel, dim3(B), dim3(256), 0, st, pose, h->J_s, h->par, ws, scratch, part3, djtr, B, n_free, dpose, dbetas, dtrans, skip);
     VT_LAUNCH_CHECK();
     return VT_OK;
@@ -739,6 +770,54 @@
     return smplh_backward_launch(h, pose, B, dverts, djtr, v_posed, ws, scratch, n_free_pose_cols, dpose, dbetas, dtrans, vt_stream(stream));
 }
 
+static bool n_free_ok(int n) { return n == NP_NUM_ || (n > 0 && n <= 3 * J_LIVE_ && n % 3 == 0); }
+
+extern "C" int vt_smplh_forward_verts(const vt_smplh *h, const float *betas, const float *trans, int B, const float *prefix, float *verts, float *v_posed,
+                                      const float *ws, void *stream)
+{
+    VT_REQUIRE(h && betas && trans && verts && v_posed && ws && B > 0, "vt_smplh_forward_verts: null argument or B <= 0");
+    return smplh_forward_launch(prefix ? 2 : 0, h, nullptr, betas, trans, B, verts, nullptr, v_posed, const_cast<float *>(ws), const_cast<float *>(prefix),
+                                vt_stream(stream), false);
+}
+
+extern "C" int vt_smplh_backward_gemms(const vt_smplh *h, int B, const float *dverts, const float *v_posed, const float *ws, float *scratch, int n_free_pose_cols,
+                                       void *stream)
+{
+    VT_REQUIRE(h && dverts && v_posed && ws && scratch && B > 0, "vt_smplh_backward_gemms: null argument or B <= 0");
+    VT_REQUIRE(n_free_ok(n_free_pose_cols), "vt_smplh_backward_gemms: n_free_pose_cols=%d must be 156 or a multiple of 3 in (0, %d]", n_free_pose_cols, 3 * J_LIVE_);
+    return smplh_backward_launch(h, nullptr, B, dverts, nullptr, v_posed, ws, scratch, n_free_pose_cols, nullptr, nullptr, nullptr, vt_stream(stream), false);
+}
+
+extern "C" int vt_smplstep_close(const vt_smplh *h, float *pose, float *betas, float *trans, int B, const float *djtr, float *ws, const float *scratch,
+                                 int n_free_pose_cols, float *dpose, float *dbetas, float *dtrans, int prefixed, float *jtr,
+                                 const float *pose_init, const float *prior_mean, const float *prior_prec, float gscale_prior, double *term_prior, float w_pinit,
+                                 double *term_pinit,
+                                 float *p0, int ps0, const float *g0, int gs0, float *m0, float *v0, int n0, float lr0,
+                                 float *p1, int ps1, const float *g1, int gs1, float *m1, float *v1, int n1, float lr1,
+                                 float *p2, int ps2, const float *g2, int gs2, float *m2, float *v2, int n2, float lr2,
+                                 int adam_step, float beta1, float beta2, float eps,
+                                 double *terms, const float *w, int nterms, float tol, int armed, float *state, int *stop_flag, float *history, int slot, int *ticket, int nzero,
+                                 void *stream)
+{
+    VT_REQUIRE(h && pose && betas && trans && ws && scratch && dpose && dbetas && dtrans && B > 0, "vt_smplstep_close: null argument or B <= 0");
+    VT_REQUIRE(n_free_ok(n_free_pose_cols), "vt_smplstep_close: n_free_pose_cols=%d must be 156 or a multiple of 3 in (0, %d]", n_free_pose_cols, 3 * J_LIVE_);
+    VT_REQUIRE(prefixed == 0 || prefixed == 1, "vt_smplstep_close: prefixed must be 0 or 1");
+    VT_REQUIRE(pose_init && prior_mean && prior_prec && term_prior && term_pinit && adam_step >= 1, "vt_smplstep_close: bad argument of the step's tail");
+    VT_REQUIRE(terms && w && state && ticket && nterms > 0 && nterms <= 16 && nzero >= 0 && nzero <= nterms, "vt_smplstep_close: bad loss arguments");
+    VT_REQUIRE((!p0 || (g0 && m0 && v0 && n0 > 0 && ps0 >= n0 && gs0 >= n0)) && (!p1 || (g1 && m1 && v1 && n1 > 0 && ps1 >= n1 && gs1 >= n1)) &&
+               (!p2 || (g2 && m2 && v2 && n2 > 0 && ps2 >= n2 && gs2 >= n2)), "vt_smplstep_close: a parameter group without its gradient / moments, or a stride below its column count");
+    hipStream_t st = vt_stream(stream);
+    double bc1; const float bc2s = adam_bias(beta1, beta2, adam_step, &bc1);
+    AdamSlice a0 = {p0, ps0, g0, gs0, m0, v0, n0, (float)(lr0 / bc1)}, a1 = {p1, ps1, g1, gs1, m1, v1, n1, (float)(lr1 / bc1)}, a2 = {p2, ps2, g2, gs2, m2, v2, n2, (float)(lr2 / bc1)};
+    const float *part3 = scratch + (size_t)NVT_ * B * PT_N + (size_t)B * KTOT_;
+    const CloseSmplh m = {h->J_t, h->J_s, scratch, part3, djtr, ws, jtr, n_free_pose_cols, prefixed ? J_LIVE_ : J_};
+    const CloseTail t = {pose_init, prior_mean, prior_prec, gscale_prior, term_prior, w_pinit, term_pinit, bc2s, beta1, beta2, eps};
+    hipLaunchKernelGGL(smplstep_close_kernel, dim3(B), dim3(256), 0, st, pose, betas, trans, dpose, dbetas, dtrans, h->par, m, t, a0, a1, a2,
+                       make_end(terms, w, nterms, tol, armed, state, stop_flag, history, slot, ticket, nzero), vt_skip_flag_of(st));
+    VT_LAUNCH_CHECK();
+    return VT_OK;
+}
+
 extern "C" int vt_rodrigues_forward(const float *aa, int n, float *R, void *stream)
 {
     VT_REQUIRE(aa && R && n > 0, "vt_rodrigues_forward: bad argument");
diff --git a/vistracker_amd/csrc/step.hip b/vistracker_amd/csrc/step.hip
--- a/vistracker_amd/csrc/step.hip
+++ b/vistracker_amd/csrc/step.hip
@@ -69,39 +69,6 @@
     hipLaunchKernelGGL(temporal2_kernel, dim3(min((B * D + 255) / 256, 512)), dim3(256), 0, vt_stream(stream), v, B, D, gs_a, term_accel, gs_v, term_velocity, dv, init_zero);
     VT_LAUNCH_CHECK();
     return VT_OK;
-}
-
-struct StepEnd {
-    const double *terms_r; double *terms_w; TermW tw; int nterms; float tol; int armed; float *state; int *stop_flag; float *history; int slot;
-    int *ticket; int nzero;
-};
-#ifndef STEP_END_FENCE
-#if defined(__HIP_DEVICE_COMPILE__) && !defined(__gfx942__) && !defined(__gfx950__)
-#define STEP_END_FENCE 1
-#else
-#define STEP_END_FENCE 0
-#endif
-#endif
-__device__ __forceinline__ void step_end(const StepEnd &e, int nblocks, bool stopped)
-{
-    __shared__ int last;
-#if STEP_END_FENCE
-    __threadfence();
-#else
-    asm volatile("s_waitcnt vmcnt(0) lgkmcnt(0)" ::: "memory");
-#endif
-    __syncthreads();
-    if (threadIdx.x == 0) last = (atomicAdd(e.ticket, 1) == nblocks - 1);
-    __syncthreads();
-    if (!last) return;
-#if STEP_END_FENCE
-    __threadfence();
-#endif
-    if (threadIdx.x == 0) {
-        *e.ticket = 0;
-        close_loss<true>(e.terms_r, e.tw, e.nterms, e.tol, e.armed, e.state, e.stop_flag, e.history, e.slot, stopped);
-        for (int k = 0; k < e.nzero; k++) e.terms_w[k] = 0.0;
-    }
 }
 
 struct TemporalIn { const float *X; float gs_a, gs_v; double *term_a, *term_v; int mode; };
@@ -197,13 +164,6 @@
     }
     step_end(end, B, stopped);
 }
-static StepEnd make_end(double *terms, const float *w, int nterms, float tol, int armed, float *state, int *stop_flag, float *history, int slot, int *ticket, int nzero)
-{
-    StepEnd e; e.terms_r = terms; e.terms_w = terms; e.nterms = nterms; e.tol = tol; e.armed = armed; e.state = state; e.stop_flag = stop_flag; e.history = history; e.slot = slot;
-    e.ticket = ticket; e.nzero = nzero;
-    for (int k = 0; k < 16; k++) e.tw.w[k] = k < nterms ? w[k] : 0.f;
-    return e;
-}
 static int objstep_tail_launch(const char *who, const TemporalIn &tin, const float *X0_verts, int NV, const float *dX_verts, const float *X0_points, int N, const float *dX_points,
                                const float *s, int B, const float *M0, const float *noise, const float *t, const float *t_init, float w_trans, double *term_trans,
                                float *dR, float *dt, float *dM,
@@ -252,28 +212,9 @@
                                                            float w_pinit, double *term_pinit, AdamSlice a0, AdamSlice a1, AdamSlice a2, float bc2s, float beta1,
                                                            float beta2, float eps, StepEnd end)
 {
-    __shared__ float d[64], t2[64];
-    const int b = blockIdx.x, B = gridDim.x, j = threadIdx.x, n = 63, off = 3, stride = 156;
+    const int b = blockIdx.x, B = gridDim.x;
     const bool stopped = end.stop_flag && *end.stop_flag;
-    const float val = mahalanobis_value(pose + (size_t)b * stride + off, n, mean, prec, d, t2);
-    __syncthreads();
-    mahalanobis_grad(t2, n, prec, dpose + (size_t)b * stride + off, gscale);
-    double acc = 0;
-    const float inv_denom = 1.f / (float)B;
-    for (int c = j; c < 69; c += 64) {
-        float g;
-        acc += (double)sqdiff_elem(pose[(size_t)b * stride + 3 + c], pose_init[(size_t)b * stride + 3 + c], inv_denom, w_pinit, g);
-        dpose[(size_t)b * stride + 3 + c] += g;
-    }
-    for (int o = 32; o > 0; o >>= 1) acc += __shfl_xor(acc, o, 64);
-    if (j == 0) { atomicAdd(term_pinit, acc * (double)inv_denom); atomicAdd(term_prior, (double)val / (double)B); }
-    __syncthreads();
-    if (!stopped) {
-        const AdamSlice *sl[3] = {&a0, &a1, &a2};
-#pragma unroll
-        for (int k = 0; k < 3; k++)
-            if (sl[k]->p) for (int c = j; c < sl[k]->ncols; c += 64) adam_one(*sl[k], b, c, bc2s, beta1, beta2, eps);
-    }
+    smplstep_tail_frame<64>(pose, pose_init, dpose, mean, prec, gscale, term_prior, w_pinit, term_pinit, a0, a1, a2, bc2s, beta1, beta2, eps, b, B, stopped);
     step_end(end, B, stopped);
 }
 extern "C" int vt_smplstep_tail(float *pose, const float *pose_init, float *dpose, int B, const float *prior_mean, const float *prior_prec, float gscale_prior,
diff --git a/vistracker_amd/csrc/step_ops.h b/vistracker_amd/csrc/step_ops.h
--- a/vistracker_amd/csrc/step_ops.h
+++ b/vistracker_amd/csrc/step_ops.h
@@ -241,6 +241,75 @@
     state[0] = loss; state[1] = loss;
 }
 
+struct StepEnd {
+    const double *terms_r; double *terms_w; TermW tw; int nterms; float tol; int armed; float *state; int *stop_flag; float *history; int slot;
+    int *ticket; int nzero;
+};
+#ifndef STEP_END_FENCE
+#if defined(__HIP_DEVICE_COMPILE__) && !defined(__gfx942__) && !defined(__gfx950__)
+#define STEP_END_FENCE 1
+#else
+#define STEP_END_FENCE 0
+#endif
+#endif
+__device__ __forceinline__ void step_end(const StepEnd &e, int nblocks, bool stopped)
+{
+    __shared__ int last;
+#if STEP_END_FENCE
+    __threadfence();
+#else
+    asm volatile("s_waitcnt vmcnt(0) lgkmcnt(0)" ::: "memory");
+#endif
+    __syncthreads();
+    if (threadIdx.x == 0) last = (atomicAdd(e.ticket, 1) == nblocks - 1);
+    __syncthreads();
+    if (!last) return;
+#if STEP_END_FENCE
+    __threadfence();
+#endif
+    if (threadIdx.x == 0) {
+        *e.ticket = 0;
+        close_loss<true>(e.terms_r, e.tw, e.nterms, e.tol, e.armed, e.state, e.stop_flag, e.history, e.slot, stopped);
+        for (int k = 0; k < e.nzero; k++) e.terms_w[k] = 0.0;
+    }
+}
+
+template <int NT>
+__device__ __forceinline__ void smplstep_tail_frame(float *pose, const float *pose_init, float *dpose, const float *mean, const float *prec, float gscale,
+                                                    double *term_prior, float w_pinit, double *term_pinit, const AdamSlice &a0, const AdamSlice &a1,
+                                                    const AdamSlice &a2, float bc2s, float beta1, float beta2, float eps, int b, int B, bool stopped)
+{
+    __shared__ float d[NT], t2[NT];
+    const int j = threadIdx.x, n = 63, off = 3, stride = 156;
+    const float val = mahalanobis_value(pose + (size_t)b * stride + off, n, mean, prec, d, t2);
+    __syncthreads();
+    mahalanobis_grad(t2, n, prec, dpose + (size_t)b * stride + off, gscale);
+    double acc = 0;
+    const float inv_denom = 1.f / (float)B;
+    if (j < 64)
+        for (int c = j; c < 69; c += 64) {
+            float g;
+            acc += (double)sqdiff_elem(pose[(size_t)b * stride + 3 + c], pose_init[(size_t)b * stride + 3 + c], inv_denom, w_pinit, g);
+            dpose[(size_t)b * stride + 3 + c] += g;
+        }
+    for (int o = 32; o > 0; o >>= 1) acc += __shfl_xor(acc, o, 64);
+    if (j == 0) { atomicAdd(term_pinit, acc * (double)inv_denom); atomicAdd(term_prior, (double)val / (double)B); }
+    __syncthreads();
+    if (!stopped && j < 64) {
+        const AdamSlice *sl[3] = {&a0, &a1, &a2};
+#pragma unroll
+        for (int k = 0; k < 3; k++)
+            if (sl[k]->p) for (int c = j; c < sl[k]->ncols; c += 64) adam_one(*sl[k], b, c, bc2s, beta1, beta2, eps);
+    }
+}
+
+static inline StepEnd make_end(double *terms, const float *w, int nterms, float tol, int armed, float *state, int *stop_flag, float *history, int slot, int *ticket, int nzero)
+{
+    StepEnd e; e.terms_r = terms; e.terms_w = terms; e.nterms = nterms; e.tol = tol; e.armed = armed; e.state = state; e.stop_flag = stop_flag; e.history = history; e.slot = slot;
+    e.ticket = ticket; e.nzero = nzero;
+    for (int k = 0; k < 16; k++) e.tw.w[k] = k < nterms ? w[k] : 0.f;
+    return e;
+}
 struct vt_landmarks { int K, V; int *indptr, *indices; float *data; int *colptr, *rowidx; float *cdata; };
 static inline float adam_bias(float beta1, float beta2, int step, double *bc1)
 {
diff --git a/vistracker_amd/fitting.py b/vistracker_amd/fitting.py
--- a/vistracker_amd/fitting.py
+++ b/vistracker_amd/fitting.py
@@ -227,6 +227,7 @@
             self.prefix = torch.empty(_lib().vt_smplh_prefix_floats(B), device=dev); self.n_free = 66
             _chk(_lib().vt_smplh_prefix(smpl.h, pose.data_ptr(), B, self.ws.data_ptr(), self.prefix.data_ptr(), L.stream_ptr()))
             self.dpose.zero_()
+        self.ws_ready = False
 
     @property
     def vert_order_ptr(self):
@@ -262,6 +263,7 @@
     fused_smpl_query = os.environ.get("VT_FUSED_SMPL_QUERY", "0") != "0"
     device_skip = os.environ.get("VT_DEVICE_SKIP", "1") != "0"
     frozen_hands = True
+    smpl_close = True
 
     def __init__(self, smpl_model, regressors, priors, decoders=None, part_labels=None, obj_verts=None, obj_faces=None, obj_points=None,
                  cam=ops.DEFAULT_CAM, device="cuda:0"):
@@ -425,11 +427,11 @@
             if it < iter_for_betas:
                 phase = "global"
                 if f.adam is None:
-                    f.adam = AdamState([(betas, 2, f.dbetas, 0.02), (trans, 3, f.dtrans, 0.02)], f.stop)
+                    f.adam = AdamState([(betas, 2, f.dbetas, 0.02), (trans, 3, f.dtrans, 0.02)], f.stop); f.ws_ready = False
             else:
                 phase = "kpts" if it >= iter_for_betas + iter_for_pose else "smpl all pose"
                 if f.adam is None or it == iter_for_betas:
-                    f.adam = AdamState([(trans, 3, f.dtrans, 0.006), (pose, 66, f.dpose, 0.006), (betas, 10, f.dbetas, 0.006)], f.stop)
+                    f.adam = AdamState([(trans, 3, f.dtrans, 0.006), (pose, 66, f.dpose, 0.006), (betas, 10, f.dbetas, 0.006)], f.stop); f.ws_ready = False
             return step, phase, f.terms.weights(FIT_WEIGHTS, 1 if phase != "kpts" else it / 3), int(early_stop and it > arm_after)
         return self._run_fit(f, start, end, check_every, outer, prof)
 
@@ -555,19 +557,18 @@
 
     def _smpl_step_fused(self, f, phase, k, w, armed):
         lib = _lib(); st = L.stream_ptr(); B = f.B
-        self.smpl_forward(f.pose, f.betas, f.trans, f.verts, f.jtr, f.vposed, f.ws, f.prefix)
+        self._smpl_step_forward(f)
         self._human_query(f, k, w)
         if phase == "kpts":
             _chk(lib.vt_kpts_step(self.b25.h, f.verts.data_ptr(), f.body_kpts.data_ptr(), f.crop_center.data_ptr(), B, 1, self.cam.ctypes.data, f.net_size,
                                   float(w[4]), f.terms.ptr("j2d"), f.J.data_ptr(), f.dverts.data_ptr(), 1, st))
         if B >= 4:
             _chk(lib.vt_accel_loss(f.verts.data_ptr(), B, 6890 * 3, None, float(w[5]), f.terms.ptr("stemp"), f.dverts.data_ptr(), st))
-        self.smpl_backward(f.pose, f.betas, f.dverts, f.vposed, f.ws, f.scratch, f.dpose, f.dbetas, f.dtrans, f.n_free)
-        self._smpl_tail(f, k, w, armed)
+        self._smpl_step_close(f, k, w, armed)
 
     def _smpl_step_fused_query(self, f, phase, k, w, armed):
         lib = _lib(); st = L.stream_ptr(); B = f.B
-        self.smpl_forward(f.pose, f.betas, f.trans, f.verts, f.jtr, f.vposed, f.ws, f.prefix)
+        self._smpl_step_forward(f)
         if phase == "kpts":
             _chk(lib.vt_kpts_step(self.b25.h, f.verts.data_ptr(), f.body_kpts.data_ptr(), f.crop_center.data_ptr(), B, 1, self.cam.ctypes.data, f.net_size,
                                   float(w[4]), f.terms.ptr("j2d"), f.J.data_ptr(), f.dverts.data_ptr(), 0, st))
@@ -576,8 +577,30 @@
                                      self.labels.data_ptr(), f.vert_order_ptr, float(w[0]), float(w[1]), int(phase == "kpts"), float(w[5]),
                                      f.terms.ptr("stemp") if B >= 4 else None, f.dverts.data_ptr(), f.terms.ptr("df_h"), st))
         _ev_end(f.lp, "human", ev, B, k)
-        self.smpl_backward(f.pose, f.betas, f.dverts, f.vposed, f.ws, f.scratch, f.dpose, f.dbetas, f.dtrans, f.n_free)
-        self._smpl_tail(f, k, w, armed)
+        self._smpl_step_close(f, k, w, armed)
+
+    def _smpl_step_forward(self, f):
+        if not f.ws_ready:
+            self.smpl_forward(f.pose, f.betas, f.trans, f.verts, f.jtr, f.vposed, f.ws, f.prefix)
+            return
+        _chk(_lib().vt_smplh_forward_verts(self.smpl.h, f.betas.data_ptr(), f.trans.data_ptr(), f.B, f.prefix.data_ptr() if f.prefix is not None else None,
+                                           f.verts.data_ptr(), f.vposed.data_ptr(), f.ws.data_ptr(), L.stream_ptr()))
+
+    def _smpl_step_close(self, f, k, w, armed):
+        if not self.smpl_close:
+            self.smpl_backward(f.pose, f.betas, f.dverts, f.vposed, f.ws, f.scratch, f.dpose, f.dbetas, f.dtrans, f.n_free)
+            self._smpl_tail(f, k, w, armed)
+            return
+        lib = _lib(); st = L.stream_ptr()
+        _chk(lib.vt_smplh_backward_gemms(self.smpl.h, f.B, f.dverts.data_ptr(), f.vposed.data_ptr(), f.ws.data_ptr(), f.scratch.data_ptr(), f.n_free, st))
+        _chk(lib.vt_smplstep_close(self.smpl.h, f.pose.data_ptr(), f.betas.data_ptr(), f.trans.data_ptr(), f.B, None, f.ws.data_ptr(), f.scratch.data_ptr(), f.n_free,
+                                   f.dpose.data_ptr(), f.dbetas.data_ptr(), f.dtrans.data_ptr(), int(f.prefix is not None), f.jtr.data_ptr(),
+                                   f.pose_init.data_ptr(), self.pri["body_mean"].data_ptr(), self.pri["body_prec"].data_ptr(), float(w[2]) / f.B,
+                                   f.terms.ptr("pose"), float(w[3]), f.terms.ptr("pinit"),
+                                   *f.adam.smpl_tail_groups, f.adam.tick(), 0.9, 0.999, 1e-8,
+                                   f.terms.buf.data_ptr(), w.ctypes.data, len(f.terms.names), 1e-3, armed, f.loss_state.data_ptr(), f.stop.data_ptr(),
+                                   f.hist.data_ptr(), k, f.ticket.data_ptr(), 6, st))
+        f.ws_ready = True
 
     def _smpl_tail(self, f, k, w, armed):
         _chk(_lib().vt_smplstep_tail(f.pose.data_ptr(), f.pose_init.data_ptr(), f.dpose.data_ptr(), f.B, self.pri["body_mean"].data_ptr(),
```

After: 150.4. 0.987x the previous value.
